# lkp411/cDLRM

Hardware: AMD Instinct MI355X
Metric: training samples/sec, Criteo-Terabyte-shape synthetic (cached data-parallel DLRM step; look-ahead refills that fall into the timed region included: see config.refills_in_timed_region) (higher is better)
Workload: dtype f32

## Files before the change

cdlrm_amd/_lib.py:

```python
from __future__ import annotations

import ctypes as C
import os
from typing import Optional

_HERE = os.path.dirname(os.path.abspath(__file__))
LIB_PATH = os.path.join(_HERE, "csrc", "libcdlrm_hip.so")

c_i32, c_i64, c_u64, c_f32 = C.c_int32, C.c_int64, C.c_uint64, C.c_float
vp = C.c_void_p


class CdlrmLibraryError(RuntimeError):
    pass


class CdlrmError(RuntimeError):
    def __init__(self, rc: int, msg: str):
        super().__init__("libcdlrm_hip: rc=%d: %s" % (rc, msg))
        self.rc = rc


class Geometry(C.Structure):
    _fields_ = [("num_tables", c_i32), ("dim", c_i32), ("num_ways", c_i32), ("aux_rows", c_i32),
                ("table_rows", C.POINTER(c_i64)), ("cache_sets", C.POINTER(c_i64)),
                ("device", c_i32), ("aux_phases", c_i32)]


class Plan(C.Structure):
    _fields_ = [("bitmap", vp), ("uniq", vp), ("uniq_off", vp), ("cap_uniq", c_i64),
                ("prot", vp), ("hit", vp), ("kept", vp), ("kept_off", vp), ("way", vp), ("flags", vp),
                ("winner", vp), ("win_claim", vp), ("win_idx", vp), ("win_row", vp), ("win_tag", vp),
                ("win_off", vp), ("cap_win", c_i64), ("stage", vp), ("ev_tag", vp)]


class Victims(C.Structure):
    _fields_ = [("pos", vp), ("idx", vp), ("off", vp), ("rows", vp), ("cap", c_i64)]


class GemmRoute(C.Structure):
    _fields_ = [("family", c_i32), ("tm", c_i32), ("tn", c_i32), ("mode", c_i32), ("aligned", c_i32), ("splits", c_i32),
                ("vec_a", c_i32), ("vec_b", c_i32), ("fast", c_i32)]


class EmbBwdRoute(C.Structure):
    _fields_ = [("sort_chunk", c_i32), ("sort_e", c_i32), ("sort_chunks", c_i32), ("merge_passes", c_i32), ("seg_meta", c_i32),
                ("keys_in_b", c_i32), ("apply", c_i32), ("arange", c_i32), ("lpr", c_i32), ("reserved", c_i32),
                ("apply_grid_x", c_i64), ("apply_grid_y", c_i64), ("long_grid", c_i64), ("keys_off", c_i64), ("meta_off", c_i64),
                ("once_off", c_i64), ("apply_keys_off", c_i64)]


PROTOTYPES = {
    "cdlrm_abi_version": (C.c_int, []),
    "cdlrm_debug_set": (C.c_int, [c_i32, c_i32]),
    "cdlrm_last_error": (C.c_char_p, []),
    "cdlrm_ctx_create": (C.c_int, [C.POINTER(Geometry), C.POINTER(vp)]),
    "cdlrm_ctx_destroy": (C.c_int, [vp]),
    "cdlrm_ctx_bind_cache": (C.c_int, [vp, vp, vp]),
    "cdlrm_ctx_bind_host_tables": (C.c_int, [vp, C.POINTER(vp)]),
    "cdlrm_host_register": (C.c_int, [vp, c_u64, C.POINTER(vp)]),
    "cdlrm_host_unregister": (C.c_int, [vp]),
    "cdlrm_ctx_check_sync": (C.c_int, [vp, vp]),
    "cdlrm_embbag_probe": (C.c_int, [vp, vp, c_i64, c_i64, vp, vp, vp, c_i32, vp]),
    "cdlrm_window_resolve": (C.c_int, [vp, vp, c_i64, c_i64, c_i64, c_i64, vp, vp, vp]),
    "cdlrm_embbag_take": (C.c_int, [vp, vp, c_i64, c_i64, vp, vp, c_i64, vp, c_i32, vp]),
    "cdlrm_victim_writeback_work_bytes": (c_u64, [c_i32, c_i64]),
    "cdlrm_victim_writeback": (C.c_int, [vp, vp, c_i64, c_i64, vp, vp, c_i64, c_i32, vp, vp]),
    "cdlrm_embbag_fwd": (C.c_int, [vp, vp, vp, c_i64, c_i64, c_i64, vp, c_i64, c_i64, vp]),
    "cdlrm_embbag_bwd_work_bytes": (c_u64, [c_i32, c_i64, c_i32]),
    "cdlrm_embbag_bwd_sgd": (C.c_int, [vp, vp, vp, c_i64, c_i64, c_i64, vp, c_i64, c_i64, c_f32, vp, vp, vp]),
    "cdlrm_embbag_bwd_prepare": (C.c_int, [vp, vp, c_i64, vp, vp]),
    "cdlrm_embbag_bwd_apply": (C.c_int, [vp, vp, c_i64, c_i64, c_i64, vp, c_i64, c_i64, c_f32, vp, vp, vp]),
    "cdlrm_embbag_bwd_apply_rest": (C.c_int, [vp, vp, c_i64, c_i64, c_i64, vp, c_i64, c_i64, c_f32, vp, vp, vp]),
    "cdlrm_embbag_bwd_once_flags": (C.c_int, [vp, vp, c_i64, vp]),
    "cdlrm_embbag_bwd_sorted_bytes": (C.c_uint64, [c_i32, c_i32, c_i64]),
    "cdlrm_embbag_bwd_prepare_window": (C.c_int, [vp, vp, c_i64, c_i64, c_i32, c_i64, c_i32, c_i32, vp, vp]),
    "cdlrm_embbag_bwd_sorted_views": (C.c_int, [vp, vp, c_i32, c_i64, c_i32, vp, vp, vp]),
    "cdlrm_embbag_bwd_apply_sorted": (C.c_int, [vp, c_i64, vp, c_i64, c_i64, c_f32, vp, vp, vp, c_i64, c_i32, c_i32, vp, vp]),
    "cdlrm_embbag_bwd_route": (C.c_int, [c_i32, c_i32, c_i64, c_i32, c_i32, c_i32, c_i32, c_i32, C.POINTER(EmbBwdRoute)]),
    "cdlrm_qr_embbag_fwd": (C.c_int, [vp, vp, c_i64, c_i64, vp, vp, c_i64, c_i32, c_i32, c_i32, vp, vp, vp, vp, vp]),
    "cdlrm_qr_embbag_bwd": (C.c_int, [vp, vp, c_i64, c_i64, vp, vp, vp, c_i64, c_i32, c_i32, c_i32, vp, vp, vp]),
    "cdlrm_bag_fwd": (C.c_int, [vp, vp, c_i64, c_i64, vp, c_i64, c_i32, vp, vp, vp]),
    "cdlrm_bag_bwd": (C.c_int, [vp, vp, c_i64, c_i64, vp, c_i64, c_i32, vp, vp]),
    "cdlrm_window_unique": (C.c_int, [vp, C.POINTER(Plan), vp, c_i64, c_i64, vp]),
    "cdlrm_window_unique_add": (C.c_int, [vp, C.POINTER(Plan), vp, c_i64, c_i64, vp]),
    "cdlrm_window_unique_finish": (C.c_int, [vp, C.POINTER(Plan), vp]),
    "cdlrm_plan_probe": (C.c_int, [vp, C.POINTER(Plan), vp]),
    "cdlrm_plan_offsets_sync": (C.c_int, [vp, C.POINTER(Plan), vp, vp, vp, vp]),
    "cdlrm_plan_assign": (C.c_int, [vp, C.POINTER(Plan), vp, c_u64, vp]),
    "cdlrm_plan_fetch": (C.c_int, [vp, C.POINTER(Plan), C.POINTER(vp), C.c_int, vp]),
    "cdlrm_plan_commit": (C.c_int, [vp, C.POINTER(Plan), vp]),
    "cdlrm_plan_writeback": (C.c_int, [vp, C.POINTER(Plan), C.POINTER(vp), C.c_int, vp]),
    "cdlrm_plan_victims": (C.c_int, [vp, C.POINTER(Plan), C.POINTER(Victims), vp]),
    "cdlrm_plan_victims_list": (C.c_int, [vp, C.POINTER(Plan), C.POINTER(Victims), vp]),
    "cdlrm_host_gather_rows": (C.c_int, [C.POINTER(vp), vp, vp, c_i32, c_i32, vp, c_i32]),
    "cdlrm_ctx_bind_victims": (C.c_int, [vp, C.POINTER(Victims)]),
    "cdlrm_gather_rows": (C.c_int, [vp, vp, c_i64, c_i32, vp, vp]),
    "cdlrm_agg_compact": (C.c_int, [vp, vp, c_i64, vp, c_i64, vp, vp]),
    "cdlrm_agg_gather": (C.c_int, [vp, vp, vp, c_f32, vp, c_i64, c_i64, vp]),
    "cdlrm_agg_scatter": (C.c_int, [vp, vp, vp, vp, c_i64, c_i64, vp]),
    "cdlrm_agg_mark_tier": (C.c_int, [vp, vp, c_i64, c_i64, c_i32, vp, vp]),
    "cdlrm_agg_split": (C.c_int, [vp, vp, c_i64, vp, c_i32, vp, vp, vp]),
    "cdlrm_interact_fwd": (C.c_int, [vp, c_i64, c_i32, c_i32, c_i32, vp, c_i64, vp]),
    "cdlrm_interact_bwd": (C.c_int, [vp, vp, c_i64, c_i64, c_i32, c_i32, c_i32, c_i32, vp, vp]),
    "cdlrm_gather_interact_supported": (C.c_int, [vp]),
    "cdlrm_gather_interact_fwd": (C.c_int, [vp, vp, c_i64, vp, c_i64, c_i64, c_i32, vp, c_i64, vp]),
    "cdlrm_gather_interact_bwd": (C.c_int, [vp, vp, c_i64, vp, c_i64, vp, c_i64, c_i64, c_i32, c_i32, vp, vp]),
    "cdlrm_gather_interact_bwd_sgd": (C.c_int, [vp, vp, c_i64, vp, c_i64, vp, c_i64, c_i64, c_i32, c_i32, vp, vp, c_i64, c_f32, vp]),
    "cdlrm_linear_fwd": (C.c_int, [vp, c_i64, vp, vp, vp, c_i64, c_i64, c_i32, c_i32, c_i32, vp]),
    "cdlrm_linear_bwd_work_bytes": (c_u64, [c_i64, c_i32, c_i32]),
    "cdlrm_linear_bwd": (C.c_int, [vp, c_i64, vp, vp, c_i64, vp, c_i64, vp, c_i64, vp, vp, c_i64, c_i32, c_i32,
                                   c_i32, c_i32, vp, vp]),
    "cdlrm_linear_fwd_route": (C.c_int, [vp, c_i64, vp, vp, vp, c_i64, c_i64, c_i32, c_i32, c_i32, vp, c_i32,
                                         C.POINTER(GemmRoute)]),
    "cdlrm_linear_bwd_route": (C.c_int, [vp, c_i64, vp, vp, c_i64, vp, c_i64, vp, c_i64, vp, vp, c_i64, c_i32, c_i32,
                                         c_i32, c_i32, vp, vp, c_i32, C.POINTER(GemmRoute)]),
    "cdlrm_mlp_wgrad_work_bytes": (c_u64, [c_i32, c_i64, vp, vp]),
    "cdlrm_mlp_wgrad": (C.c_int, [c_i32, vp, vp, vp, vp, vp, vp, c_i64, vp, vp, vp, vp]),
    "cdlrm_mlp_wgrad_sgd": (C.c_int, [c_i32, vp, vp, vp, vp, vp, vp, vp, vp, c_f32, c_i64, vp, vp, vp, vp]),
    "cdlrm_mlp_wgrad_work_bytes_ex": (c_u64, [c_i32, c_i64, vp, vp, c_i32]),
    "cdlrm_mlp_wgrad_ex": (C.c_int, [c_i32, vp, vp, vp, vp, vp, vp, c_i64, vp, vp, c_i32, vp, vp]),
    "cdlrm_mlp_wgrad_sgd_ex": (C.c_int, [c_i32, vp, vp, vp, vp, vp, vp, vp, vp, c_f32, c_i64, vp, vp, c_i32, vp, vp]),
    "cdlrm_mlp_wgrad_route": (C.c_int, [c_i32, vp, vp, vp, vp, vp, vp, c_i64, vp, vp, c_i32, c_i32, C.POINTER(GemmRoute)]),
    "cdlrm_bce_fwd_bwd": (C.c_int, [vp, vp, c_i64, vp, vp, c_i32, vp]),
    "cdlrm_loss_fwd_bwd": (C.c_int, [vp, vp, c_i64, c_i32, C.c_float, C.c_float, C.c_float, vp, vp, vp, c_i32, vp]),
    "cdlrm_head_scratch_floats": (c_i64, []),
    "cdlrm_head_fwd_bwd": (C.c_int, [vp, c_i64, vp, vp, vp, c_i64, c_i32, c_i32, C.c_float, C.c_float, C.c_float, c_i32,
                                     vp, vp, vp, vp, c_i64, vp, vp, c_i32, vp]),
    "cdlrm_head_finish": (C.c_int, [vp, c_i64, vp, vp, vp]),
    "cdlrm_sgd_step2": (C.c_int, [vp, vp, c_i64, c_i64, c_i64, c_i64, C.c_float, vp]),
    "cdlrm_act_bwd": (C.c_int, [vp, c_i64, vp, c_i64, c_i64, c_i32, c_i32, vp]),
    "cdlrm_sgd_step": (C.c_int, [vp, vp, c_i64, c_f32, vp]),
    "cdlrm_scale_div": (C.c_int, [vp, c_i64, c_f32, vp]),
    "cdlrm_scatter_rows": (C.c_int, [vp, vp, vp, c_i64, c_i32, C.c_int, vp]),
    "cdlrm_blend_rows": (C.c_int, [vp, vp, vp, c_i64, c_i32, vp, vp]),
    "cdlrm_mark_rows": (C.c_int, [vp, vp, c_i64, vp, vp]),
    "cdlrm_synth_indices": (C.c_int, [vp, c_i64, c_i64, c_i64, C.c_double, c_u64, vp]),
    "cdlrm_bags_window": (C.c_int, [vp, c_i64, vp, c_i32, c_i32, c_i64, vp, vp]),
    "cdlrm_bags_rank_slice": (C.c_int, [vp, c_i64, vp, c_i32, c_i32, c_i32, vp, c_i64, c_i64, c_i64, c_i64, vp, vp, vp]),
    "cdlrm_dayfile_window": (C.c_int, [vp, vp, vp, c_i64, c_i32, c_i32, c_i64, vp, vp, c_i64, c_i64, vp, vp]),
    "cdlrm_dayfile_tile": (C.c_int, []),
    "cdlrm_tape_create": (vp, [c_i32]),
    "cdlrm_tape_destroy": (None, [vp]),
    "cdlrm_tape_add": (C.c_int, [vp, vp, c_i32, vp, vp, c_i32, vp]),
    "cdlrm_tape_cells": (vp, [vp]),
    "cdlrm_tape_length": (c_i64, [vp]),
    "cdlrm_tape_stream_arg": (c_i32, [vp]),
    "cdlrm_tape_op_info": (C.c_char_p, [vp, c_i64, vp]),
    "cdlrm_tape_probe": (C.c_int, [c_f32, c_i64, c_f32, c_i32, vp, c_i64, c_f32, c_i32, c_i64, c_i64, vp, c_i32, c_f32, c_i64]),
    "cdlrm_tape_probe_log": (C.c_int, [c_i64, c_i64]),
    "cdlrm_tape_probe_log_take": (c_i64, [vp, c_i64]),
    "cdlrm_tape_replay": (C.c_int, [vp]),
    "cdlrm_tape_set_lanes": (C.c_int, [vp, vp, vp, c_i64]),
    "cdlrm_tape_selftest": (C.c_int, []),
    "cdlrm_event_record": (C.c_int, [vp, vp]),
    "cdlrm_stream_wait_event": (C.c_int, [vp, vp]),
    "cdlrm_event_attach_next": (C.c_int, [vp, vp]),
    "cdlrm_stream_create": (vp, [c_i32]),
    "cdlrm_stream_destroy": (C.c_int, [vp]),
    "cdlrm_event_create": (vp, [c_i32]),
    "cdlrm_event_destroy": (C.c_int, [vp]),
    "cdlrm_event_elapsed_us": (C.c_int, [vp, vp, vp]),
    "cdlrm_ctx_time_next_gather": (C.c_int, [vp, vp, vp]),
}

_lib: Optional[C.CDLL] = None
_proxy = None
import threading as _threading

_rec = _threading.local()


class _Recording:

    def __init__(self, cdll):
        self._cdll = cdll

    def __getattr__(self, name):
        fn = getattr(self._cdll, name)
        is_call = fn.restype is C.c_int

        def call(*args):
            tape = getattr(_rec, "tape", None)
            if tape is not None and is_call:
                tape.append((fn, args))
            return fn(*args)

        call.__name__ = name
        self.__dict__[name] = call
        return call


def start_recording(tape: list) -> None:
    _rec.tape = tape


def stop_recording() -> None:
    _rec.tape = None


def record(fn, *args):
    tape = getattr(_rec, "tape", None)
    if tape is not None:
        tape.append((fn, args))
    return fn(*args)


def raw():
    lib()
    return _lib


def lib():
    global _lib, _proxy
    if _lib is None:
        if not os.path.exists(LIB_PATH):
            raise CdlrmLibraryError(
                "%s not found: build it with `make -C cdlrm_amd/csrc` (or __graft_entry__.build()). "
                "cdlrm_amd has no CPU fallback for the cached training path." % LIB_PATH)
        import torch
        l = C.CDLL(LIB_PATH)
        for name, (res, args) in PROTOTYPES.items():
            fn = getattr(l, name)
            fn.restype = res
            fn.argtypes = args
        if l.cdlrm_abi_version() != 1:
            raise CdlrmLibraryError("ABI version mismatch")
        _lib = l
        _proxy = _Recording(l)
    return _proxy


def require_gpu(what: str = "cdlrm_amd") -> None:
    import torch
    if not torch.cuda.is_available():
        raise CdlrmLibraryError(
            "%s needs a HIP device (MI355X / gfx950) and found none: cdlrm_amd has no CPU fallback for the cached training "
            "path -- every compute entry point is a hand-written HIP kernel behind csrc/libcdlrm_hip.so" % what)


HW_QUEUES_PINNED = 2
HIP_DEFAULT_HW_QUEUES = 4


def hw_queues() -> int:
    try:
        return int(os.environ.get("GPU_MAX_HW_QUEUES", str(HIP_DEFAULT_HW_QUEUES)))
    except ValueError:
        return -1


_warned_queues = False


def warn_hw_queues() -> None:
    global _warned_queues
    if not _warned_queues and hw_queues() != HW_QUEUES_PINNED:
        _warned_queues = True
        import warnings
        warnings.warn("GPU_MAX_HW_QUEUES=%s: cdlrm_amd's entry points run with %d hardware queues per process (set "
                      "GPU_MAX_HW_QUEUES=%d before the first HIP call)"
                      % (os.environ.get("GPU_MAX_HW_QUEUES"), HW_QUEUES_PINNED, HW_QUEUES_PINNED), RuntimeWarning, stacklevel=3)


class TapeUnsupported(Exception):
# ... 188 lines not shown
```

cdlrm_amd/csrc/ctx.hip:

```cpp
#include <stdarg.h>
#include <sys/resource.h>
#include <sys/syscall.h>
#include <unistd.h>

#include <algorithm>
#include <thread>

#include "common.h"

static thread_local char g_err[512] = "";

void cdlrm_set_error(const char* fmt, ...) {
    va_list ap;
    va_start(ap, fmt);
    vsnprintf(g_err, sizeof(g_err), fmt, ap);
    va_end(ap);
}

int g_cdlrm_debug[8] = {0, 0, 0, 0, 0, 0, 0, 0};
extern "C" int cdlrm_debug_set(int32_t key, int32_t value) {
    CDLRM_REQUIRE(key >= 0 && key < 8, "key: 0 .. 7");
#ifndef CDLRM_DEV
    CDLRM_REQUIRE(!(key == 6 && (value & 3)), "work-skipping switches (key 6, bits 1 and 2) exist in -DCDLRM_DEV builds only");
#endif
    g_cdlrm_debug[key] = value;
    return 0;
}
extern "C" int cdlrm_abi_version(void) { return CDLRM_ABI_VERSION; }
extern "C" const char* cdlrm_last_error(void) { return g_err; }

extern "C" int cdlrm_ctx_create(const cdlrm_geometry* geo, cdlrm_ctx** out) {
    CDLRM_REQUIRE(geo && out, "null argument");
    CDLRM_REQUIRE(geo->num_tables >= 1 && geo->num_tables <= 1024, "1..1024 tables");
    CDLRM_REQUIRE(geo->dim >= 4 && geo->dim % 4 == 0, "dim must be a positive multiple of 4");
    CDLRM_REQUIRE(geo->num_ways >= 1 && geo->num_ways <= 64, "1..64 ways");
    CDLRM_REQUIRE(geo->aux_rows >= 0, "aux_rows >= 0");
    CDLRM_REQUIRE(geo->aux_phases >= 0 && geo->aux_phases <= 2, "aux_phases 0..2");
    CDLRM_HIP_CHECK(hipSetDevice(geo->device));
    cdlrm_ctx* c = new cdlrm_ctx();
    c->T = geo->num_tables; c->D = geo->dim; c->ways = geo->num_ways; c->aux = geo->aux_rows;
    c->device = geo->device;
    c->aux_phases = geo->aux_phases < 1 ? 1 : geo->aux_phases;
    int64_t tag = 0, row = 0, set = 0, bm = 0;
    for (int k = 0; k < c->T; ++k) {
        TableDesc d;
        d.n_rows = geo->table_rows[k];
        d.P = geo->cache_sets[k];
        if (d.n_rows < 1 || d.P < 1 || d.P > d.n_rows ||
            d.P * (int64_t)c->ways + (int64_t)c->aux * c->aux_phases >= ((int64_t)1 << 31)) {
            delete c;
            cdlrm_set_error("cdlrm_ctx_create: table %d has unsupported geometry (n=%lld P=%lld)", k,
                            (long long)geo->table_rows[k], (long long)geo->cache_sets[k]);
            return CDLRM_EINVAL;
        }
        d.tag_base = tag; d.row_base = row; d.set_base = set; d.bm_base = bm;
        d.bm_words = ((d.n_rows + 63) / 64 + BM_WPB - 1) / BM_WPB * BM_WPB;
        d.rows = d.P * c->ways + (int64_t)c->aux * c->aux_phases;
        tag += d.P * c->ways; row += d.rows; set += d.P; bm += d.bm_words;
        c->h_tab.push_back(d);
    }
    c->total_tags = tag; c->total_rows = row; c->total_sets = set; c->total_bm_words = bm;
    c->h_host_rows.assign(c->T, nullptr);
    CDLRM_HIP_CHECK(hipMalloc(&c->d_tab, sizeof(TableDesc) * c->T));
    CDLRM_HIP_CHECK(hipMemcpy(c->d_tab, c->h_tab.data(), sizeof(TableDesc) * c->T, hipMemcpyHostToDevice));
    CDLRM_HIP_CHECK(hipMalloc(&c->d_host_rows, sizeof(float*) * c->T));
    CDLRM_HIP_CHECK(hipMemset(c->d_host_rows, 0, sizeof(float*) * c->T));
    CDLRM_HIP_CHECK(hipMalloc(&c->d_ptr_fetch, sizeof(float*) * c->T));
    CDLRM_HIP_CHECK(hipMalloc(&c->d_ptr_wb, sizeof(float*) * c->T));
    CDLRM_HIP_CHECK(hipMalloc(&c->d_err, sizeof(int)));
    CDLRM_HIP_CHECK(hipMemset(c->d_err, 0, sizeof(int)));
    CDLRM_HIP_CHECK(hipMalloc(&c->d_small, sizeof(int64_t) * 256));
    CDLRM_HIP_CHECK(hipMemset(c->d_small, 0, sizeof(int64_t) * 256));
    CDLRM_HIP_CHECK(hipHostMalloc((void**)&c->h_pinned, sizeof(int64_t) * 4096, hipHostMallocDefault));
    int rc = cdlrm_scan_reserve(c, 1 << 16);
    if (rc) { delete c; return rc; }
    *out = c;
    return 0;
}

extern "C" int cdlrm_ctx_destroy(cdlrm_ctx* c) {
    if (!c) return 0;
    try {
        (void)hipDeviceSynchronize();
        if (c->d_tab) (void)hipFree(c->d_tab);
        if (c->d_host_rows) (void)hipFree(c->d_host_rows);
        if (c->d_ptr_fetch) (void)hipFree(c->d_ptr_fetch);
        if (c->d_ptr_wb) (void)hipFree(c->d_ptr_wb);
        if (c->d_err) (void)hipFree(c->d_err);
        if (c->d_small) (void)hipFree(c->d_small);
        if (c->d_scan) (void)hipFree(c->d_scan);
        if (c->d_scan_agg) (void)hipFree(c->d_scan_agg);
        if (c->h_pinned) (void)hipHostFree(c->h_pinned);
        (void)hipGetLastError();
    } catch (...) {
    }
    delete c;
    return 0;
}

extern "C" int cdlrm_ctx_bind_cache(cdlrm_ctx* c, int64_t* tags, float* weight) {
    CDLRM_REQUIRE(c && tags && weight, "null argument");
    CDLRM_REQUIRE(((uintptr_t)weight & 15) == 0 && ((uintptr_t)tags & 15) == 0, "16-byte aligned buffers");
    c->tags = tags;
    c->weight = weight;
    return 0;
}

extern "C" int cdlrm_ctx_bind_host_tables(cdlrm_ctx* c, float* const* host_rows) {
    CDLRM_REQUIRE(c && host_rows, "null argument");
    for (int k = 0; k < c->T; ++k) {
        CDLRM_REQUIRE(host_rows[k] != nullptr && ((uintptr_t)host_rows[k] & 15) == 0, "16-byte aligned host tables");
        c->h_host_rows[k] = host_rows[k];
    }
    CDLRM_HIP_CHECK(hipMemcpy(c->d_host_rows, c->h_host_rows.data(), sizeof(float*) * c->T, hipMemcpyHostToDevice));
    return 0;
}

extern "C" int cdlrm_host_register(void* host_ptr, uint64_t bytes, void** device_alias) {
    CDLRM_REQUIRE(host_ptr && bytes && device_alias, "null argument");
    CDLRM_HIP_CHECK(hipHostRegister(host_ptr, bytes, hipHostRegisterMapped | hipHostRegisterPortable));
    CDLRM_HIP_CHECK(hipHostGetDevicePointer(device_alias, host_ptr, 0));
    return 0;
}

extern "C" int cdlrm_host_unregister(void* host_ptr) {
    CDLRM_REQUIRE(host_ptr, "null argument");
    CDLRM_HIP_CHECK(hipHostUnregister(host_ptr));
    return 0;
}

static void host_gather_range(const float* const* tables, const int64_t* idx, const int64_t* off, int T, int D, float* dst,
                              int64_t a, int64_t b, int background) {
    if (background) (void)setpriority(PRIO_PROCESS, (id_t)syscall(SYS_gettid), 19);
    int t = 0;
    const size_t row_bytes = (size_t)D * sizeof(float);
    constexpr int AHEAD = 16;
    int ta = 0;
    for (int64_t j = a; j < b; ++j) {
        const int64_t jp = j + AHEAD;
        if (jp < b) {
            while (ta < T - 1 && jp >= off[ta + 1]) ++ta;
            const char* p = (const char*)(tables[ta] + idx[jp] * D);
            for (size_t o = 0; o < row_bytes; o += 64) __builtin_prefetch(p + o, 0, 0);
        }
        while (t < T - 1 && j >= off[t + 1]) ++t;
        memcpy(dst + j * D, tables[t] + idx[j] * D, row_bytes);
    }
}

extern "C" int cdlrm_host_gather_rows(const float* const* tables, const int64_t* idx, const int64_t* off, int32_t T,
                                      int32_t D, float* dst, int32_t nthreads) {
    CDLRM_REQUIRE(tables && idx && off && dst && T >= 1 && D >= 1, "bad argument");
    const int64_t n = off[T];
    if (n <= 0) return 0;
    for (int k = 0; k < T; ++k) CDLRM_REQUIRE(off[k] <= off[k + 1] && (off[k] == off[k + 1] || tables[k]), "bad offsets / table");
    int nt = nthreads < 1 ? 1 : nthreads;
    if ((int64_t)nt > (n + 4095) / 4096) nt = (int)((n + 4095) / 4096);
    if (nt <= 1) {
        host_gather_range(tables, idx, off, T, D, dst, 0, n, 0);
        return 0;
    }
    std::vector<std::thread> th;
    const int64_t per = (n + nt - 1) / nt;
    for (int i = 0; i < nt; ++i) {
        const int64_t a = i * per, b = std::min<int64_t>(n, a + per);
        if (a >= b) break;
        th.emplace_back(host_gather_range, tables, idx, off, (int)T, (int)D, dst, a, b, 1);
    }
    for (auto& x : th) x.join();
    return 0;
}

extern "C" int cdlrm_ctx_check_sync(cdlrm_ctx* c, void* stream) {
    CDLRM_REQUIRE(c, "null ctx");
    hipStream_t s = (hipStream_t)stream;
    int* h = (int*)(c->h_pinned + 4000);
// ... 11 lines not shown
```

cdlrm_amd/csrc/dense.hip:

```cpp
#include "gemm_wide.h"
#include "gemm_bf16.h"


#define SK_KMAX 32
__global__ void __launch_bounds__(256) k_linear_smallk(const float* __restrict__ X, int64_t ld_x, const float* __restrict__ W,
                                                       const float* __restrict__ bias, float* __restrict__ Y, int64_t ld_y,
                                                       int64_t M, int N, int K, int act) {
    __shared__ float Xs[32][SK_KMAX + 1];
    __shared__ __attribute__((aligned(16))) float Wt[SK_KMAX][128 + 4];
    const int64_t m0 = (int64_t)blockIdx.y * 32;
    const int n0 = blockIdx.x * 128;
    for (int e = threadIdx.x; e < 32 * K; e += 256) {
        const int r = e / K, k = e % K;
        Xs[r][k] = X[min(m0 + r, M - 1) * ld_x + k];
    }
    for (int e = threadIdx.x; e < 128 * K; e += 256) {
        const int n = e / K, k = e % K;
        Wt[k][n] = W[(int64_t)min(n0 + n, N - 1) * K + k];
    }
    __syncthreads();
    const int cg = threadIdx.x & 31, rg = threadIdx.x >> 5;
    float acc[4][4];
#pragma unroll
    for (int i = 0; i < 4; ++i)
// ... 102 lines not shown
        const int64_t blocks = cdiv(M, rpw) * (N >> 8);
        if (blocks <= 0x7fffffff) {
            if (rec) {
                gemm_record(rec, CDLRM_ROUTE_SMALLK_ROWS, 0, 0, 0, 0, 1, 0, 0, 0);
                return 0;
            }
            hipLaunchKernelGGL((k_linear_smallk_rows<13>), dim3((unsigned)blocks), dim3(256), 0, (hipStream_t)stream, X, ld_x, W,
                               bias, Y, ld_y, M, (int)N, rpw, (int)act);
            CDLRM_LAUNCH_CHECK();
            return 0;
        }
    }
    if (K <= SK_KMAX && N % 4 == 0 && ld_y % 4 == 0 && aligned16(Y) && cdiv(M, 32) <= 65535) {
        if (rec) {
            gemm_record(rec, CDLRM_ROUTE_SMALLK, 0, 0, 0, 0, 1, 0, 0, 0);
            return 0;
        }
        dim3 grid((unsigned)cdiv(N, 128), (unsigned)cdiv(M, 32));
        hipLaunchKernelGGL(k_linear_smallk, grid, dim3(256), 0, (hipStream_t)stream, X, ld_x, W, bias, Y, ld_y, M, (int)N,
                           (int)K, (int)act);
        CDLRM_LAUNCH_CHECK();
        return 0;
    }
    GemmArgs g = gemm_args();
    g.A = X; g.lda = ld_x; g.B = W; g.ldb = K; g.C = Y; g.ldc = ld_y; g.slab = 0;
    g.M = M; g.N = N; g.K = K; g.kchunk = K; g.bias = bias; g.act = act;
    g.vecA = aligned16(X) && ld_x % 4 == 0 && K % 4 == 0;
    g.vecB = aligned16(W) && K % 4 == 0;
    g.alone = alone;
    return launch_gemm<true, true>(g, 1, (hipStream_t)stream, rec);
}

extern "C" int cdlrm_linear_fwd(const float* X, int64_t ld_x, const float* W, const float* bias, float* Y, int64_t ld_y,
                                int64_t M, int32_t N, int32_t K, int32_t act, void* stream) {
    return linear_fwd(X, ld_x, W, bias, Y, ld_y, M, N, K, act, stream, nullptr);
}

extern "C" int cdlrm_linear_fwd_route(const float* X, int64_t ld_x, const float* W, const float* bias, float* Y, int64_t ld_y,
                                      int64_t M, int32_t N, int32_t K, int32_t act, void* stream, int32_t n_cu,
                                      cdlrm_gemm_route* out) {
    CDLRM_REQUIRE(out && n_cu >= 1, "bad argument");
    memset(out, 0, sizeof(*out));
    const GemmRec rec = {out, n_cu};
    return linear_fwd(X, ld_x, W, bias, Y, ld_y, M, N, K, act, stream, &rec);
}

__global__ void __launch_bounds__(256) k_act_grad(const float* __restrict__ Y, int64_t ld_y, float* __restrict__ dY,
                                                  int64_t ld_dy, int64_t M, int N, int act) {
    const int64_t total = M * N;
    for (int64_t e = (int64_t)blockIdx.x * blockDim.x + threadIdx.x; e < total; e += (int64_t)gridDim.x * blockDim.x) {
        const int64_t m = e / N;
        const int n = (int)(e % N);
        const float y = Y[m * ld_y + n];
        float d = dY[m * ld_dy + n];
        if (act == 1) d = y > 0.f ? d : 0.f;
        else if (act == 2) d = d * ((1.0f - y) * y);
        dY[m * ld_dy + n] = d;
    }
}

__device__ __forceinline__ void reduce_slabs_body(int bid, const float* __restrict__ partA, int64_t countA, int splitsA,
                                                  float* __restrict__ outA, int gxa, const float* __restrict__ partB,
                                                  int64_t countB, int splitsB, float* __restrict__ outB,
                                                  float (*red)[64], float* __restrict__ pA = nullptr,
                                                  float* __restrict__ pB = nullptr, float lr = 0.f, int novec = 0) {
    if (bid >= gxa) {
        const int c = threadIdx.x & 63, sub = threadIdx.x >> 6;
        const int64_t e = (int64_t)(bid - gxa) * 64 + c;
        float s = 0.f;
        if (e < countB)
            for (int z = sub; z < splitsB; z += 4) s += partB[(int64_t)z * countB + e];
        red[sub][c] = s;
        __syncthreads();
        if (sub == 0 && e < countB) {
            const float g = ((red[0][c] + red[1][c]) + red[2][c]) + red[3][c];
            outB[e] = g;
            if (pB) pB[e] = fmaf(-lr, g, pB[e]);
        }
        return;
    }
    if (!novec && (countA & 3) == 0 && ((((uintptr_t)partA | (uintptr_t)outA | (uintptr_t)pA) & 15) == 0)) {
        const int64_t n4 = countA >> 2;
        const float4* __restrict__ p4 = reinterpret_cast<const float4*>(partA);
        for (int64_t e = (int64_t)bid * blockDim.x + threadIdx.x; e < n4; e += (int64_t)gxa * blockDim.x) {
            float4 s = make_float4(0.f, 0.f, 0.f, 0.f);
            float4 q = make_float4(0.f, 0.f, 0.f, 0.f);
            if (pA) q = reinterpret_cast<const float4*>(pA)[e];
            __builtin_amdgcn_sched_barrier(0);
            int z = 0;
            for (; z + 8 <= splitsA; z += 8) {
                float4 v[8];
#pragma unroll
                for (int u = 0; u < 8; ++u) v[u] = p4[(int64_t)(z + u) * n4 + e];
#pragma unroll
                for (int u = 0; u < 8; ++u) { s.x += v[u].x; s.y += v[u].y; s.z += v[u].z; s.w += v[u].w; }
            }
            for (; z < splitsA; ++z) {
                const float4 v = p4[(int64_t)z * n4 + e];
                s.x += v.x; s.y += v.y; s.z += v.z; s.w += v.w;
            }
            reinterpret_cast<float4*>(outA)[e] = s;
            if (pA) {
                q.x = fmaf(-lr, s.x, q.x); q.y = fmaf(-lr, s.y, q.y); q.z = fmaf(-lr, s.z, q.z); q.w = fmaf(-lr, s.w, q.w);
                reinterpret_cast<float4*>(pA)[e] = q;
            }
        }
        return;
    }
    for (int64_t e = (int64_t)bid * blockDim.x + threadIdx.x; e < countA; e += (int64_t)gxa * blockDim.x) {
        float s = 0.f;
        int z = 0;
        for (; z + 4 <= splitsA; z += 4) {
            const float v0 = partA[(int64_t)z * countA + e], v1 = partA[(int64_t)(z + 1) * countA + e];
            const float v2 = partA[(int64_t)(z + 2) * countA + e], v3 = partA[(int64_t)(z + 3) * countA + e];
            s += v0; s += v1; s += v2; s += v3;
        }
        for (; z < splitsA; ++z) s += partA[(int64_t)z * countA + e];
        outA[e] = s;
        if (pA) pA[e] = fmaf(-lr, s, pA[e]);
    }
}

__global__ void __launch_bounds__(256) k_reduce_slabs(const float* __restrict__ partA, int64_t countA, int splitsA,
                                                      float* __restrict__ outA, int gxa,
                                                      const float* __restrict__ partB, int64_t countB, int splitsB,
                                                      float* __restrict__ outB) {
    __shared__ float red[4][64];
    reduce_slabs_body((int)blockIdx.x, partA, countA, splitsA, outA, gxa, partB, countB, splitsB, outB, red);
}

struct ReduceJob {
    const float* partA; int64_t countA; float* outA; int gxa;
    const float* partB; int64_t countB; float* outB;
    int splits;
    float* pA; float* pB; float lr;
    int novec;
};
struct ReduceGroup {
    int n;
    unsigned first[GEMM_GROUP_MAX + 1];
    ReduceJob j[GEMM_GROUP_MAX];
};
__global__ void __launch_bounds__(256) k_reduce_group(ReduceGroup grp) {
    __shared__ float red[4][64];
    int p = 0;
#pragma unroll
    for (int q = 1; q < GEMM_GROUP_MAX; ++q)
        if (q < grp.n && blockIdx.x >= grp.first[q]) p = q;
    const ReduceJob& r = grp.j[p];
    reduce_slabs_body((int)(blockIdx.x - grp.first[p]), r.partA, r.countA, r.splits, r.outA, r.gxa, r.partB, r.countB,
                      r.splits, r.outB, red, r.pA, r.pB, r.lr, r.novec);
}

#define WGRAD_DIRECT_MAX_M 2048
static int wgrad_splits(int64_t M, int N, int K) {
    if (M <= WGRAD_DIRECT_MAX_M) return 1;
    const int64_t tiles = cdiv(N, 64) * cdiv(K, 64);
    const int64_t target = 1024;
    int64_t s = cdiv(target, tiles);
    const int64_t smax = cdiv(M, 8 * GBK);
    if (s > smax) s = smax;
    if (s < 1) s = 1;
    return (int)s;
}

extern "C" uint64_t cdlrm_linear_bwd_work_bytes(int64_t M, int32_t N, int32_t K) {
    const uint64_t splits = (uint64_t)wgrad_splits(M, N, K);
    const uint64_t slabs = splits * N * K * 4;
    const uint64_t cs = splits * N * 4;
    return ((slabs + 255) & ~(uint64_t)255) + ((cs + 255) & ~(uint64_t)255) + 256;
}

extern "C" uint64_t cdlrm_mlp_wgrad_work_bytes(int32_t n_layers, int64_t M, const int32_t* N, const int32_t* K) {
    uint64_t total = 256, largest = 0;
    if (!N || !K) return 0;
    if (M <= WGRAD_DIRECT_MAX_M) {
        const uint64_t zs = (uint64_t)cdiv(M, 4 * GBK) + 1;
        for (int i = 0; i < n_layers; ++i)
            total += ((zs * N[i] * K[i] * 4 + 255) & ~(uint64_t)255) + ((zs * N[i] * 4 + 255) & ~(uint64_t)255);
        return total;
    }
    (void)largest;
    for (int i = 0; i < n_layers; ++i) total += cdlrm_linear_bwd_work_bytes(M, N[i], K[i]);
    return total;
}

static int linear_bwd(const float* X, int64_t ld_x, const float* W, const float* Y, int64_t ld_y, float* dY, int64_t ld_dy,
                      float* dX, int64_t ld_dx, float* dW, float* db, int64_t M, int32_t N, int32_t K, int32_t act,
                      int32_t x_act, void* work, void* stream, const GemmRec* rec) {
    const int alone = (act & CDLRM_GEMM_ALONE) != 0;
    const int bf16 = (act & CDLRM_GEMM_BF16) != 0 && bf16_layer_ok(N, K);
    act &= ~(CDLRM_GEMM_ALONE | CDLRM_GEMM_BF16);
    CDLRM_REQUIRE(X && W && dY && work && M >= 1 && N >= 1 && K >= 1, "bad argument");
    CDLRM_REQUIRE(dW || !db, "db without dW (the bias gradient is a by-product of the weight-gradient GEMM)");
    CDLRM_REQUIRE(act == 0 || Y, "activation backward needs Y");
    CDLRM_REQUIRE(act >= 0 && act <= 2 && x_act >= 0 && x_act <= 2, "bad activation code");
    CDLRM_REQUIRE(((uintptr_t)work & 255) == 0, "work must be 256-byte aligned");
    hipStream_t s = (hipStream_t)stream;
    const int splits = wgrad_splits(M, N, K);
    float* slabs = (float*)work;
    float* cs = (float*)((char*)work + ((((uint64_t)splits * N * K * 4) + 255) & ~(uint64_t)255));
    if (act != 0 && !rec) {
        const int64_t nb = cdiv(M * N, 256), blocks = nb < 2048 ? nb : 2048;
        hipLaunchKernelGGL(k_act_grad, dim3((unsigned)blocks), dim3(256), 0, s, Y, ld_y, dY, ld_dy, M, N, act);
    }
    if (dX) {
        GemmArgs g = gemm_args();
        g.A = dY; g.lda = ld_dy; g.B = W; g.ldb = K; g.C = dX; g.ldc = ld_dx; g.slab = 0;
        g.M = M; g.N = K; g.K = N; g.kchunk = N; g.bias = nullptr; g.act = 0;
        g.vecA = aligned16(dY) && ld_dy % 4 == 0 && N % 4 == 0;
        g.vecB = aligned16(W) && K % 4 == 0;
        g.mask = X; g.ldmask = ld_x; g.mask_act = x_act;
        g.alone = alone;
        int rc = bf16 ? launch_gemm_bf16<true, false>(g, s, rec) : launch_gemm<true, false>(g, 1, s, rec);
        if (rc) return rc;
    }
    if (dW && bf16) {
        GemmArgs g = gemm_args();
        g.A = dY; g.lda = ld_dy; g.B = X; g.ldb = ld_x; g.ldc = K;
        g.slab = (int64_t)N * K;
        g.M = N; g.N = K; g.K = M; g.kchunk = bf16_wgrad_kchunk(M, cdiv(N, 64) * cdiv(K, 64), splits);
        const int va = bf16_vec<false>(dY, ld_dy, N, M), vb = bf16_vec<false>(X, ld_x, K, M);
        g.vecA = va; g.vecB = vb;
        const int zs = (int)cdiv(M, g.kchunk);
        g.C = zs > 1 ? slabs : dW;
        g.colsum = db ? (zs > 1 ? cs : db) : nullptr;
        if (rec) {
            gemm_record(rec + 1, CDLRM_ROUTE_BF16, 1, 1, 0, 0, zs, va, vb, 0);
            return 0;
        }
        int rc = launch_wgrad_bf16(&g, 1, va, vb, s);
        if (rc) return rc;
        if (zs > 1) {
            int64_t gxa = cdiv((int64_t)N * K, 256);
            if (gxa > 2048) gxa = 2048;
            const int64_t gxb = db ? cdiv(N, 64) : 0;
            hipLaunchKernelGGL(k_reduce_slabs, dim3((unsigned)(gxa + gxb)), dim3(256), 0, s, slabs, (int64_t)N * K, zs, dW,
                               (int)gxa, cs, (int64_t)N, zs, db);
        }
    } else if (dW) {
        GemmArgs g = gemm_args();
        g.A = dY; g.lda = ld_dy; g.B = X; g.ldb = ld_x; g.ldc = K;
        g.slab = (int64_t)N * K;
        g.M = N; g.N = K; g.K = M; g.kchunk = cdiv(cdiv(M, splits), GBK) * GBK; g.bias = nullptr; g.act = 0;
        g.vecA = aligned16(dY) && ld_dy % 4 == 0 && N % 4 == 0;
        g.vecB = aligned16(X) && ld_x % 4 == 0 && K % 4 == 0;
        const int zs = (int)cdiv(M, g.kchunk);
        g.C = zs > 1 ? slabs : dW;
        g.colsum = db ? (zs > 1 ? cs : db) : nullptr;
        int rc = launch_gemm<false, false>(g, zs, s, rec ? rec + 1 : nullptr);
        if (rc) return rc;
        if (zs > 1 && !rec) {
            int64_t gxa = cdiv((int64_t)N * K, 256);
            if (gxa > 2048) gxa = 2048;
            const int64_t gxb = db ? cdiv(N, 64) : 0;
            hipLaunchKernelGGL(k_reduce_slabs, dim3((unsigned)(gxa + gxb)), dim3(256), 0, s, slabs, (int64_t)N * K, zs, dW,
                               (int)gxa, cs, (int64_t)N, zs, db);
        }
    }
    if (!rec) CDLRM_LAUNCH_CHECK();
    return 0;
}

extern "C" int cdlrm_linear_bwd(const float* X, int64_t ld_x, const float* W, const float* Y, int64_t ld_y, float* dY,
                                int64_t ld_dy, float* dX, int64_t ld_dx, float* dW, float* db, int64_t M, int32_t N,
                                int32_t K, int32_t act, int32_t x_act, void* work, void* stream) {
    CdlrmStopScope stop_scope;
    if ((act & ~(CDLRM_GEMM_ALONE | CDLRM_GEMM_BF16)) != 0 || dW || !dX) stop_scope.hold((hipStream_t)stream);
    return linear_bwd(X, ld_x, W, Y, ld_y, dY, ld_dy, dX, ld_dx, dW, db, M, N, K, act, x_act, work, stream, nullptr);
}

extern "C" int cdlrm_linear_bwd_route(const float* X, int64_t ld_x, const float* W, const float* Y, int64_t ld_y, float* dY,
                                      int64_t ld_dy, float* dX, int64_t ld_dx, float* dW, float* db, int64_t M, int32_t N,
                                      int32_t K, int32_t act, int32_t x_act, void* work, void* stream, int32_t n_cu,
                                      cdlrm_gemm_route* out) {
    CDLRM_REQUIRE(out && n_cu >= 1, "bad argument");
    memset(out, 0, 2 * sizeof(*out));
    const GemmRec rec[2] = {{out, n_cu}, {out + 1, n_cu}};
    return linear_bwd(X, ld_x, W, Y, ld_y, dY, ld_dy, dX, ld_dx, dW, db, M, N, K, act, x_act, work, stream, rec);
}

__global__ void __launch_bounds__(256) k_sgd(float* __restrict__ p, const float* __restrict__ g, int64_t n, float lr);

static void launch_reduce_jobs(const std::vector<ReduceJob>& jobs, hipStream_t s) {
    for (size_t q0 = 0; q0 < jobs.size(); q0 += GEMM_GROUP_MAX) {
        ReduceGroup red;
        memset(&red, 0, sizeof(red));
        unsigned rblocks = 0;
        for (size_t q = q0; q < jobs.size() && q < q0 + GEMM_GROUP_MAX; ++q) {
            red.first[red.n] = rblocks;
            red.j[red.n] = jobs[q];
            rblocks += (unsigned)(jobs[q].gxa + cdiv(jobs[q].countB, 64));
            red.n++;
        }
        red.first[red.n] = rblocks;
        hipLaunchKernelGGL(k_reduce_group, dim3(rblocks), dim3(256), 0, s, red);
    }
}

static int sgd_layers(const std::vector<int>& layers, float* const* dW, float* const* db, float* const* P_w, float* const* P_b,
                      const int32_t* N, const int32_t* K, float lr, hipStream_t s) {
    for (int i : layers) {
        const int64_t cnt = (int64_t)N[i] * K[i];
        int64_t gx = cdiv(cnt, 256);
        if (gx > 2048) gx = 2048;
        hipLaunchKernelGGL(k_sgd, dim3((unsigned)gx), dim3(256), 0, s, P_w[i], (const float*)dW[i], cnt, lr);
        if (db[i] && P_b && P_b[i])
            hipLaunchKernelGGL(k_sgd, dim3((unsigned)cdiv(N[i], 256)), dim3(256), 0, s, P_b[i], (const float*)db[i], (int64_t)N[i], lr);
    }
    CDLRM_LAUNCH_CHECK();
    return 0;
}

static inline void route_set(cdlrm_gemm_route* out, int family, int tm, int tn, int mode, int aligned, int splits, int va, int vb,
                             int fast) {
    const GemmRec rec = {out, 0};
    gemm_record(&rec, family, tm, tn, mode, aligned, splits, va, vb, fast);
}

static int mlp_wgrad_impl(int32_t n_layers, const float* const* X, const int64_t* ld_x, const float* const* dZ,
                          const int64_t* ld_dz, float* const* dW, float* const* db, int64_t M, const int32_t* N,
                          const int32_t* K, void* work, void* stream, float* const* P_w, float* const* P_b, float lr,
                          cdlrm_gemm_route* rout = nullptr, int n_cu = 0, int64_t extra_tiles = 0) {
    CDLRM_REQUIRE(n_layers >= 0 && (n_layers == 0 || (X && ld_x && dZ && ld_dz && dW && db && N && K)) && M >= 1,
                  "bad argument");
    hipStream_t s = (hipStream_t)stream;
    std::vector<char> stepped((size_t)(n_layers > 0 ? n_layers : 0), 0);
    auto step_rest = [&]() -> int {
        if (!P_w) return 0;
        std::vector<int> rest;
        for (int i = 0; i < n_layers; ++i)
            if (!stepped[i]) rest.push_back(i);
        return sgd_layers(rest, dW, db, P_w, P_b, N, K, lr, s);
    };
    if (M <= WGRAD_DIRECT_MAX_M) {
        const int use_tiled = 1;
        std::vector<GemmArgs> direct, tiled;
        std::vector<int> direct_layer, tiled_layer;
        int64_t tiles = 0;
        for (int i = 0; i < n_layers; ++i) {
            CDLRM_REQUIRE(X[i] && dZ[i] && dW[i] && N[i] >= 1 && K[i] >= 1 && ld_x[i] >= K[i] && ld_dz[i] >= N[i],
                          "bad layer argument");
            GemmArgs g = gemm_args();
            g.A = dZ[i]; g.lda = ld_dz[i]; g.B = X[i]; g.ldb = ld_x[i]; g.C = dW[i]; g.ldc = K[i];
            g.M = N[i]; g.N = K[i]; g.K = M; g.kchunk = M; g.colsum = db[i];
            g.vecA = aligned16(dZ[i]) && ld_dz[i] % 4 == 0 && N[i] % 4 == 0;
            g.vecB = aligned16(X[i]) && ld_x[i] % 4 == 0 && K[i] % 4 == 0;
            if (use_tiled && g.vecA && g.vecB && M >= 256) {
                tiled.push_back(g);
                tiled_layer.push_back(i);
                tiles += cdiv(N[i], 64) * cdiv(K[i], 64);
            } else {
                direct.push_back(g);
                direct_layer.push_back(i);
            }
        }
        int64_t kchunk = M;
        int zs = 1;
        tiles += extra_tiles;
        if (tiles > 0) {
            const int64_t target_wgs = M <= 1024 ? 768 : 640;
            int64_t splits = cdiv(target_wgs, tiles);
            const int64_t smax = cdiv(M, 4 * GBK);
            if (splits > smax) splits = smax;
            if (splits < 1) splits = 1;
            kchunk = cdiv(cdiv(M, splits), GBK) * GBK;
            zs = (int)cdiv(M, kchunk);
        }
        if (rout) {
            for (size_t q = 0; q < tiled.size(); ++q)
                route_set(&rout[tiled_layer[q]], CDLRM_ROUTE_GEMM, 1, 1, 0, 0, zs, 1, 1, 0);
            for (size_t q = 0; q < direct.size(); ++q)
                route_set(&rout[direct_layer[q]], CDLRM_ROUTE_DIRECT, 0, 0, 0, 0, zs, direct[q].vecA, direct[q].vecB, 0);
            return 0;
        }
        CDLRM_REQUIRE(zs == 1 || (work && ((uintptr_t)work & 255) == 0), "work must be 256-byte aligned");
        char* wp = (char*)work;
        std::vector<ReduceJob> jobs;
        auto slabbed = [&](GemmArgs& g, int li) {
            const int64_t cnt = (int64_t)N[li] * K[li];
            g.kchunk = kchunk;
            g.slab = cnt;
            if (zs == 1) return;
            float* slabs = (float*)wp;
            wp += (((uint64_t)zs * cnt * 4) + 255) & ~(uint64_t)255;
            float* cs = (float*)wp;
            wp += (((uint64_t)zs * N[li] * 4) + 255) & ~(uint64_t)255;
            g.C = slabs;
            g.colsum = db[li] ? cs : nullptr;
            ReduceJob r;
            r.partA = slabs; r.countA = cnt; r.outA = dW[li];
            int64_t gxa = cdiv(cnt, 1024);
            if (gxa > 256) gxa = 256;
            r.gxa = (int)gxa;
            r.partB = cs; r.countB = db[li] ? N[li] : 0; r.outB = db[li];
            r.splits = zs;
            r.novec = g_cdlrm_debug[2];
            r.pA = P_w ? P_w[li] : nullptr; r.pB = (P_w && P_b && db[li]) ? P_b[li] : nullptr; r.lr = lr;
            if (P_w) stepped[li] = 1;
            jobs.push_back(r);
        };
        for (size_t q = 0; q < direct.size(); ++q) slabbed(direct[q], direct_layer[q]);
        for (size_t q = 0; q < tiled.size(); ++q) slabbed(tiled[q], tiled_layer[q]);
        bool direct_done = direct.empty();
        for (size_t q0 = 0; q0 < tiled.size(); q0 += GEMM_GROUP_MAX) {
            GemmGroup grp;
            memset(&grp, 0, sizeof(grp));
            unsigned blocks = 0;
            for (size_t q = q0; q < tiled.size() && q < q0 + GEMM_GROUP_MAX; ++q) {
                grp.first[grp.n] = blocks;
                grp.g[grp.n] = tiled[q];
                blocks += (unsigned)(cdiv(tiled[q].M, 64) * cdiv(tiled[q].N, 64) * zs);
                grp.n++;
            }
            grp.first[grp.n] = blocks;
            if (!direct_done && launch_wgrad_mixed(direct.data(), (int)direct.size(), grp, blocks, s)) {
                direct_done = true;
                continue;
            }
            hipLaunchKernelGGL((k_gemm_group<false, false, true, true>), dim3(blocks), dim3(256), 0, s, grp);
        }
        if (!direct_done) {
            int rc = launch_wgrad_group(direct.data(), (int)direct.size(), s);
            if (rc) return rc;
        }
        launch_reduce_jobs(jobs, s);
        CDLRM_LAUNCH_CHECK();
        return step_rest();
    }
    CDLRM_REQUIRE(rout || (work && ((uintptr_t)work & 255) == 0), "work must be 256-byte aligned");
    char* wp = (char*)work;
    std::vector<ReduceJob> jobs;
    for (int i = 0; i < n_layers; ++i) {
        CDLRM_REQUIRE(X[i] && dZ[i] && dW[i] && N[i] >= 1 && K[i] >= 1 && ld_x[i] >= K[i] && ld_dz[i] >= N[i],
                      "bad layer argument");
        const int splits = wgrad_splits(M, N[i], K[i]);
        const int64_t cnt = (int64_t)N[i] * K[i];
        GemmArgs g = gemm_args();
        g.A = dZ[i]; g.lda = ld_dz[i]; g.B = X[i]; g.ldb = ld_x[i]; g.ldc = K[i];
        g.slab = cnt;
        g.M = N[i]; g.N = K[i]; g.K = M; g.kchunk = cdiv(cdiv(M, splits), GBK) * GBK;
        g.vecA = aligned16(dZ[i]) && ld_dz[i] % 4 == 0 && N[i] % 4 == 0;
        g.vecB = aligned16(X[i]) && ld_x[i] % 4 == 0 && K[i] % 4 == 0;
        const int zs = (int)cdiv(M, g.kchunk);
        g.C = dW[i];
        g.colsum = db[i];
        if (rout) {
            const GemmRec rec = {&rout[i], n_cu};
            (void)launch_gemm<false, false>(g, zs, s, &rec);
            continue;
        }
        if (zs > 1) {
            float* slabs = (float*)wp;
            wp += (((uint64_t)zs * cnt * 4) + 255) & ~(uint64_t)255;
            float* cs = (float*)wp;
            wp += (((uint64_t)zs * N[i] * 4) + 255) & ~(uint64_t)255;
            g.C = slabs;
            g.colsum = db[i] ? cs : nullptr;
            ReduceJob r;
            r.partA = slabs; r.countA = cnt; r.outA = dW[i];
            int64_t gxa = cdiv(cnt, 256);
            if (gxa > 1024) gxa = 1024;
            r.gxa = (int)gxa;
            r.partB = cs; r.countB = db[i] ? N[i] : 0; r.outB = db[i];
            r.splits = zs;
            r.novec = g_cdlrm_debug[2];
            r.pA = P_w ? P_w[i] : nullptr; r.pB = (P_w && P_b && db[i]) ? P_b[i] : nullptr; r.lr = lr;
            if (P_w) stepped[i] = 1;
            jobs.push_back(r);
        }
        int rc = launch_gemm<false, false>(g, zs, s);
        if (rc) return rc;
    }
    if (rout) return 0;
    launch_reduce_jobs(jobs, s);
    CDLRM_LAUNCH_CHECK();
    return step_rest();
}

extern "C" int cdlrm_mlp_wgrad(int32_t n_layers, const float* const* X, const int64_t* ld_x, const float* const* dZ,
                               const int64_t* ld_dz, float* const* dW, float* const* db, int64_t M, const int32_t* N,
                               const int32_t* K, void* work, void* stream) {
    return mlp_wgrad_impl(n_layers, X, ld_x, dZ, ld_dz, dW, db, M, N, K, work, stream, nullptr, nullptr, 0.f);
}

extern "C" int cdlrm_mlp_wgrad_sgd(int32_t n_layers, const float* const* X, const int64_t* ld_x, const float* const* dZ,
                                   const int64_t* ld_dz, float* const* dW, float* const* db, float* const* W,
                                   float* const* b, float lr, int64_t M, const int32_t* N, const int32_t* K, void* work,
                                   void* stream) {
    CDLRM_REQUIRE(n_layers == 0 || (W && b), "parameters missing");
    return mlp_wgrad_impl(n_layers, X, ld_x, dZ, ld_dz, dW, db, M, N, K, work, stream, W, b, lr);
}

struct Bf16Wgrad {
    std::vector<int> fp, bf;
    int64_t kchunk = 0;
    int zs = 1;
    uint64_t fp_bytes = 0;
};

static void bf16_wgrad_plan(int32_t n_layers, int64_t M, const int32_t* N, const int32_t* K, Bf16Wgrad& p) {
    int64_t tiles = 0;
    for (int i = 0; i < n_layers; ++i) {
        if (bf16_layer_ok(N[i], K[i])) {
            p.bf.push_back(i);
            tiles += cdiv(N[i], 64) * cdiv(K[i], 64);
        } else {
            p.fp.push_back(i);
        }
    }
    p.kchunk = bf16_wgrad_kchunk(M, tiles, INT64_MAX);
    p.zs = (int)cdiv(M, p.kchunk);
    if (!p.fp.empty()) {
        std::vector<int32_t> n, k;
        for (int i : p.fp) { n.push_back(N[i]); k.push_back(K[i]); }
        p.fp_bytes = cdlrm_mlp_wgrad_work_bytes((int32_t)p.fp.size(), M, n.data(), k.data());
    }
}

extern "C" uint64_t cdlrm_mlp_wgrad_work_bytes_ex(int32_t n_layers, int64_t M, const int32_t* N, const int32_t* K,
                                                  int32_t flags) {
    if (!(flags & CDLRM_GEMM_BF16)) return cdlrm_mlp_wgrad_work_bytes(n_layers, M, N, K);
    if (!N || !K) return 0;
    Bf16Wgrad p;
    bf16_wgrad_plan(n_layers, M, N, K, p);
    uint64_t total = p.fp_bytes + 256;
    if (p.zs > 1)
        for (int i : p.bf)
            total += (((uint64_t)p.zs * N[i] * K[i] * 4 + 255) & ~(uint64_t)255) + (((uint64_t)p.zs * N[i] * 4 + 255) & ~(uint64_t)255);
    return total;
}

static int mlp_wgrad_ex_impl(int32_t n_layers, const float* const* X, const int64_t* ld_x, const float* const* dZ,
                             const int64_t* ld_dz, float* const* dW, float* const* db, int64_t M, const int32_t* N,
                             const int32_t* K, int32_t flags, void* work, void* stream, float* const* P_w, float* const* P_b,
                             float lr, cdlrm_gemm_route* rout, int n_cu) {
    CDLRM_REQUIRE((flags & ~CDLRM_GEMM_BF16) == 0, "bad flags");
    if (!(flags & CDLRM_GEMM_BF16))
        return mlp_wgrad_impl(n_layers, X, ld_x, dZ, ld_dz, dW, db, M, N, K, work, stream, P_w, P_b, lr, rout, n_cu);
    CDLRM_REQUIRE(n_layers >= 0 && (n_layers == 0 || (X && ld_x && dZ && ld_dz && dW && db && N && K)) && M >= 1,
                  "bad argument");
    CDLRM_REQUIRE(rout || (work && ((uintptr_t)work & 255) == 0), "work must be 256-byte aligned");
    for (int i = 0; i < n_layers; ++i)
        CDLRM_REQUIRE(X[i] && dZ[i] && dW[i] && N[i] >= 1 && K[i] >= 1 && ld_x[i] >= K[i] && ld_dz[i] >= N[i],
                      "bad layer argument");
    hipStream_t s = (hipStream_t)stream;
    Bf16Wgrad p;
    bf16_wgrad_plan(n_layers, M, N, K, p);
    if (!p.fp.empty()) {
        int64_t extra_tiles = 0;
        for (int i : p.bf) {
            const bool va = aligned16(dZ[i]) && ld_dz[i] % 4 == 0 && N[i] % 4 == 0;
            const bool vb = aligned16(X[i]) && ld_x[i] % 4 == 0 && K[i] % 4 == 0;
            if (va && vb && M >= 256) extra_tiles += cdiv(N[i], 64) * cdiv(K[i], 64);
        }
        const size_t nf = p.fp.size();
        std::vector<const float*> fx(nf), fdz(nf);
        std::vector<float*> fdw(nf), fdb(nf), fpw(nf), fpb(nf);
        std::vector<int64_t> fldx(nf), flddz(nf);
        std::vector<int32_t> fn(nf), fk(nf);
        std::vector<cdlrm_gemm_route> fr(nf);
        for (size_t q = 0; q < nf; ++q) {
            const int i = p.fp[q];
            fx[q] = X[i]; fdz[q] = dZ[i]; fdw[q] = dW[i]; fdb[q] = db[i]; fldx[q] = ld_x[i]; flddz[q] = ld_dz[i];
            fn[q] = N[i]; fk[q] = K[i];
            fpw[q] = P_w ? P_w[i] : nullptr; fpb[q] = (P_w && P_b) ? P_b[i] : nullptr;
        }
        memset(fr.data(), 0, nf * sizeof(cdlrm_gemm_route));
        int rc = mlp_wgrad_impl((int32_t)nf, fx.data(), fldx.data(), fdz.data(), flddz.data(), fdw.data(), fdb.data(), M, fn.data(),
                                fk.data(), work, stream, P_w ? fpw.data() : nullptr, P_w ? fpb.data() : nullptr, lr,
                                rout ? fr.data() : nullptr, n_cu, extra_tiles);
        if (rc) return rc;
        if (rout)
            for (size_t q = 0; q < nf; ++q) rout[p.fp[q]] = fr[q];
    }
    if (p.bf.empty()) return 0;
    std::vector<GemmArgs> probs;
    std::vector<ReduceJob> jobs;
    char* wp = (char*)work + p.fp_bytes;
    int va = 1, vb = 1;
    for (int i : p.bf) {
        const int64_t cnt = (int64_t)N[i] * K[i];
        GemmArgs g = gemm_args();
        g.A = dZ[i]; g.lda = ld_dz[i]; g.B = X[i]; g.ldb = ld_x[i]; g.ldc = K[i];
        g.slab = cnt;
        g.M = N[i]; g.N = K[i]; g.K = M; g.kchunk = p.kchunk;
        g.vecA = bf16_vec<false>(dZ[i], ld_dz[i], N[i], M);
        g.vecB = bf16_vec<false>(X[i], ld_x[i], K[i], M);
// ... 1413 lines not shown
```

cdlrm_amd/csrc/gemm_glds.h:

```cpp
#pragma once
#include "gemm.h"

#define G2_BK 32
#ifndef G2_PRIO
#define G2_PRIO 0
#endif
#ifndef G2_ABL
#define G2_ABL 0
#endif

typedef __attribute__((address_space(3))) void* g2_lds_ptr;

__device__ __forceinline__ void g2_dma16(const float* src, unsigned lds_wave_base) {
    unsigned keep;
    asm volatile("s_mov_b32 %0, m0\n\ts_mov_b32 m0, %2\n\ts_nop 0\n\tglobal_load_lds_dwordx4 %1, off\n\ts_mov_b32 m0, %0"
                 : "=&s"(keep)
                 : "v"(src), "s"(lds_wave_base)
                 : "memory");
}
__device__ __forceinline__ void g2_dma_wait() { asm volatile("s_waitcnt vmcnt(0)" ::: "memory"); }
__device__ __forceinline__ unsigned g2_lds_addr(const float* p) {
    return (unsigned)(uintptr_t)(g2_lds_ptr)(p);
}

template <bool KC, int ROWS>
struct G2Stage {
    static constexpr int NP = ROWS / 32;
    const float* src[NP];
    int64_t step;
    __device__ __forceinline__ void init(const float* P, int64_t ld, int64_t r0, int64_t rmax, int64_t kbeg) {
        const int tid = threadIdx.x;
#pragma unroll
        for (int i = 0; i < NP; ++i) {
            if (KC) {
                const int row = i * 32 + (tid >> 3);
                const int c = (tid & 7) ^ ((row >> 1) & 7);
                src[i] = P + min(r0 + row, rmax - 1) * ld + kbeg + 4 * c;
            } else {
                constexpr int CPR = ROWS / 4;
                const int q = i * 256 + tid;
                const int kk = q / CPR, rc = (q % CPR) * 4;
                src[i] = P + (kbeg + kk) * ld + min(r0 + rc, rmax - 4);
            }
        }
        step = KC ? G2_BK : G2_BK * ld;
    }
    __device__ __forceinline__ void piece(int i, unsigned base) {
        g2_dma16(src[i], base + i * 4096u);
        src[i] += step;
    }
};

template <bool A_KC, bool B_KC, int TM, int TN>
__device__ __forceinline__ void g2_frags(const float* Ab, const float* Bb, int kg, int ra, int rb, int lk, int sw,
                                         float4 (&a)[TM], float4 (&b)[TN]) {
    constexpr int BM = 64 * TM, BN = 64 * TN;
#pragma unroll
    for (int i = 0; i < TM; ++i) {
        const int r = ra + i * 32;
        if (A_KC) {
            a[i] = *reinterpret_cast<const float4*>(Ab + r * G2_BK + 4 * ((kg * 2 + lk) ^ sw));
        } else {
            const float* q = Ab + (kg * 8 + 4 * lk) * BM + r;
            a[i] = make_float4(q[0], q[BM], q[2 * BM], q[3 * BM]);
        }
    }
#pragma unroll
    for (int j = 0; j < TN; ++j) {
        const int c = rb + j * 32;
        if (B_KC) {
            b[j] = *reinterpret_cast<const float4*>(Bb + c * G2_BK + 4 * ((kg * 2 + lk) ^ sw));
        } else {
            const float* q = Bb + (kg * 8 + 4 * lk) * BN + c;
            b[j] = make_float4(q[0], q[BN], q[2 * BN], q[3 * BN]);
        }
    }
}

template <int TM, int TN>
__device__ __forceinline__ void g2_epilogue(const GemmArgs& g, f32x16 (&acc)[TM][TN], int64_t m0, int64_t n0, unsigned bz,
                                            int wm, int wn, int lane) {
    float* C = g.C + (int64_t)bz * g.slab;
    const bool vbias = g.bias != nullptr && (((uintptr_t)g.bias) & 15) == 0;
    const bool vmask = g.mask_act != 0 && (((uintptr_t)g.mask) & 15) == 0 && (g.ldmask & 3) == 0;
#pragma unroll
    for (int i = 0; i < TM; ++i) {
        const int64_t row = m0 + wm * (32 * TM) + i * 32 + (lane & 31);
#pragma unroll
        for (int j = 0; j < TN; ++j) {
#pragma unroll
            for (int q = 0; q < 4; ++q) {
                const int64_t col = n0 + wn * (32 * TN) + j * 32 + 8 * q + 4 * (lane >> 5);
                if (row >= g.M || col >= g.N) continue;
                float4 v = make_float4(acc[i][j][4 * q], acc[i][j][4 * q + 1], acc[i][j][4 * q + 2], acc[i][j][4 * q + 3]);
                if (g.bias) {
                    float4 bv;
                    if (vbias) bv = *reinterpret_cast<const float4*>(g.bias + col);
                    else bv = make_float4(g.bias[col], g.bias[col + 1], g.bias[col + 2], g.bias[col + 3]);
                    v.x += bv.x; v.y += bv.y; v.z += bv.z; v.w += bv.w;
                }
                if (g.act == 1) {
                    v.x = v.x > 0.f ? v.x : 0.f; v.y = v.y > 0.f ? v.y : 0.f;
                    v.z = v.z > 0.f ? v.z : 0.f; v.w = v.w > 0.f ? v.w : 0.f;
                } else if (g.act == 2) {
                    v.x = 1.0f / (1.0f + expf(-v.x)); v.y = 1.0f / (1.0f + expf(-v.y));
                    v.z = 1.0f / (1.0f + expf(-v.z)); v.w = 1.0f / (1.0f + expf(-v.w));
                }
                if (g.mask_act) {
                    float4 x;
                    const float* mp = g.mask + row * g.ldmask + col;
                    if (vmask) x = *reinterpret_cast<const float4*>(mp);
                    else x = make_float4(mp[0], mp[1], mp[2], mp[3]);
                    if (g.mask_act == 1) {
                        v.x = x.x > 0.f ? v.x : 0.f; v.y = x.y > 0.f ? v.y : 0.f;
                        v.z = x.z > 0.f ? v.z : 0.f; v.w = x.w > 0.f ? v.w : 0.f;
                    } else {
                        v.x *= (1.0f - x.x) * x.x; v.y *= (1.0f - x.y) * x.y;
                        v.z *= (1.0f - x.z) * x.z; v.w *= (1.0f - x.w) * x.w;
                    }
                }
                *reinterpret_cast<float4*>(C + row * g.ldc + col) = v;
            }
        }
    }
}

template <int TM, int TN, bool B_KC, int ACT>
__device__ __forceinline__ void g2_epilogue_full(const GemmArgs& g, f32x16 (&acc)[TM][TN], int64_t m0, int64_t n0, int wm, int wn,
                                                 int lane) {
    float4 bv[TN][4];
    float4 mv[B_KC ? 1 : TM][B_KC ? 1 : TN][4];
    const int64_t row0 = m0 + wm * (32 * TM) + (lane & 31);
    const int64_t col0 = n0 + wn * (32 * TN) + 4 * (lane >> 5);
    if (B_KC) {
        if (g.bias) {
#pragma unroll
            for (int j = 0; j < TN; ++j)
#pragma unroll
                for (int q = 0; q < 4; ++q) bv[j][q] = *reinterpret_cast<const float4*>(g.bias + col0 + j * 32 + 8 * q);
        } else {
#pragma unroll
            for (int j = 0; j < TN; ++j)
#pragma unroll
                for (int q = 0; q < 4; ++q) bv[j][q] = make_float4(0.f, 0.f, 0.f, 0.f);
        }
    } else if (ACT != 0) {
#pragma unroll
        for (int i = 0; i < TM; ++i)
#pragma unroll
            for (int j = 0; j < TN; ++j)
#pragma unroll
                for (int q = 0; q < 4; ++q)
                    mv[i][j][q] = *reinterpret_cast<const float4*>(g.mask + (row0 + i * 32) * g.ldmask + col0 + j * 32 + 8 * q);
    }
    const bool has_bias = g.bias != nullptr;
    __builtin_amdgcn_sched_barrier(0);
#pragma unroll
    for (int i = 0; i < TM; ++i)
#pragma unroll
        for (int j = 0; j < TN; ++j)
#pragma unroll
            for (int q = 0; q < 4; ++q) {
                float4 v = make_float4(acc[i][j][4 * q], acc[i][j][4 * q + 1], acc[i][j][4 * q + 2], acc[i][j][4 * q + 3]);
                if (B_KC) {
                    const float4 b = bv[j][q];
                    if (has_bias) { v.x += b.x; v.y += b.y; v.z += b.z; v.w += b.w; }
                    if (ACT == 1) {
                        v.x = v.x > 0.f ? v.x : 0.f; v.y = v.y > 0.f ? v.y : 0.f;
                        v.z = v.z > 0.f ? v.z : 0.f; v.w = v.w > 0.f ? v.w : 0.f;
                    } else if (ACT == 2) {
                        v.x = 1.0f / (1.0f + expf(-v.x)); v.y = 1.0f / (1.0f + expf(-v.y));
                        v.z = 1.0f / (1.0f + expf(-v.z)); v.w = 1.0f / (1.0f + expf(-v.w));
                    }
                } else if (ACT != 0) {
                    const float4 x = mv[i][j][q];
                    if (ACT == 1) {
                        v.x = x.x > 0.f ? v.x : 0.f; v.y = x.y > 0.f ? v.y : 0.f;
                        v.z = x.z > 0.f ? v.z : 0.f; v.w = x.w > 0.f ? v.w : 0.f;
                    } else if (ACT == 2) {
                        v.x *= (1.0f - x.x) * x.x; v.y *= (1.0f - x.y) * x.y;
                        v.z *= (1.0f - x.z) * x.z; v.w *= (1.0f - x.w) * x.w;
                    }
                }
                *reinterpret_cast<float4*>(g.C + (row0 + i * 32) * g.ldc + col0 + j * 32 + 8 * q) = v;
            }
}

template <bool B_KC>
__host__ __device__ __forceinline__ bool g2_full_ok(const GemmArgs& g) {
    if (!g.fastep) return false;
    if (B_KC) return g.mask_act == 0 && (g.bias == nullptr || (((uintptr_t)g.bias) & 15) == 0);
    return g.bias == nullptr && g.act == 0 && (g.mask_act == 0 || ((((uintptr_t)g.mask) & 15) == 0 && (g.ldmask & 3) == 0));
}

#ifdef GEMM2_STAMP
__device__ unsigned long long g2_stamps[8 * 4096];
#define G2_STAMP(slot)                                                                            \
    if (threadIdx.x == 0 && g2_wg < 4096) {                                                         \
        g2_stamps[g2_wg * 8 + (slot)] = __builtin_amdgcn_s_memtime();                                \
        if ((slot) == 0 || (slot) == 3) g2_stamps[g2_wg * 8 + 4 + ((slot) ? 1 : 0)] = __builtin_amdgcn_s_memrealtime(); \
        if ((slot) == 0) g2_stamps[g2_wg * 8 + 6] = ((unsigned long long)__builtin_amdgcn_s_getreg((31 << 11) | 20) << 32) | \
                                                    (unsigned)__builtin_amdgcn_s_getreg((31 << 11) | 4);               \
    }
#else
#define G2_STAMP(slot)
#endif

template <bool A_KC, bool B_KC, int TM, int TN>
__device__ __forceinline__ void gemm2_tile_body(const GemmArgs& g, unsigned bx, unsigned by, unsigned bz, float* lds) {
#ifdef GEMM2_STAMP
    const unsigned g2_wg = (blockIdx.z * gridDim.y + blockIdx.y) * gridDim.x + blockIdx.x;
#endif
    G2_STAMP(0)
    constexpr int BM = 64 * TM, BN = 64 * TN;
    constexpr int A_ST = BM * G2_BK, B_ST = BN * G2_BK;
    float* As = lds;
    float* Bs = lds + 2 * A_ST;
    const int lane = threadIdx.x & 63, wave = threadIdx.x >> 6;
    const int wm = wave >> 1, wn = wave & 1;
    const int lr = lane & 31, lk = lane >> 5;
    const int64_t m0 = (int64_t)by * BM;
    const int64_t n0 = (int64_t)bx * BN;
    const int64_t kbeg = (int64_t)bz * g.kchunk;
    const int64_t kend = min(g.K, kbeg + g.kchunk);
    const int nt = (int)((kend - kbeg) / G2_BK);
    f32x16 acc[TM][TN];
#pragma unroll
    for (int i = 0; i < TM; ++i)
#pragma unroll
        for (int j = 0; j < TN; ++j)
#pragma unroll
            for (int r = 0; r < 16; ++r) acc[i][j][r] = 0.f;
    const bool do_colsum = !A_KC && g.colsum != nullptr && bx == 0 && wn == 0;
    float csum[TM];
#pragma unroll
    for (int i = 0; i < TM; ++i) csum[i] = 0.f;

    G2Stage<A_KC, BM> sa;
    G2Stage<B_KC, BN> sb;
    constexpr int NPA = G2Stage<A_KC, BM>::NP, NPB = G2Stage<B_KC, BN>::NP, NPIECE = NPA + NPB;
    sa.init(g.A, g.lda, m0, g.M, kbeg);
    sb.init(g.B, g.ldb, n0, g.N, kbeg);
    const unsigned a_dst = __builtin_amdgcn_readfirstlane(g2_lds_addr(As) + wave * 1024u);
    const unsigned b_dst = __builtin_amdgcn_readfirstlane(g2_lds_addr(Bs) + wave * 1024u);
    const int ra = wm * (32 * TM) + lr, rb = wn * (32 * TN) + lr;
    const int sw = (lr >> 1) & 7;

    float4 fa[2][TM], fb[2][TN];
#pragma unroll
    for (int i = 0; i < NPA; ++i) sa.piece(i, a_dst);
#pragma unroll
    for (int i = 0; i < NPB; ++i) sb.piece(i, b_dst);
    g2_dma_wait();
    __syncthreads();
    if (nt > 1) {
#pragma unroll
        for (int i = 0; i < NPA; ++i) sa.piece(i, a_dst + A_ST * 4u);
#pragma unroll
        for (int i = 0; i < NPB; ++i) sb.piece(i, b_dst + B_ST * 4u);
    }
    g2_frags<A_KC, B_KC, TM, TN>(As, Bs, 0, ra, rb, lk, sw, fa[0], fb[0]);
    G2_STAMP(1)

    auto mfma_group = [&](const float4 (&a)[TM], const float4 (&b)[TN]) {
        if (!A_KC && do_colsum) {
#pragma unroll
            for (int i = 0; i < TM; ++i) csum[i] += (a[i].x + a[i].y) + (a[i].z + a[i].w);
        }
#pragma unroll
        for (int i = 0; i < TM; ++i)
#pragma unroll
            for (int j = 0; j < TN; ++j) {
                acc[i][j] = __builtin_amdgcn_mfma_f32_32x32x2f32(b[j].x, a[i].x, acc[i][j], 0, 0, 0);
                acc[i][j] = __builtin_amdgcn_mfma_f32_32x32x2f32(b[j].y, a[i].y, acc[i][j], 0, 0, 0);
                acc[i][j] = __builtin_amdgcn_mfma_f32_32x32x2f32(b[j].z, a[i].z, acc[i][j], 0, 0, 0);
                acc[i][j] = __builtin_amdgcn_mfma_f32_32x32x2f32(b[j].w, a[i].w, acc[i][j], 0, 0, 0);
            }
    };

    for (int t = 0; t < nt; ++t) {
        const int cur = t & 1;
        const float* Ab = As + cur * A_ST;
        const float* Bb = Bs + cur * B_ST;
        g2_frags<A_KC, B_KC, TM, TN>(Ab, Bb, 1, ra, rb, lk, sw, fa[1], fb[1]);
        mfma_group(fa[0], fb[0]);
        __builtin_amdgcn_sched_barrier(0);
        g2_frags<A_KC, B_KC, TM, TN>(Ab, Bb, 2, ra, rb, lk, sw, fa[0], fb[0]);
        mfma_group(fa[1], fb[1]);
        __builtin_amdgcn_sched_barrier(0);
        g2_frags<A_KC, B_KC, TM, TN>(Ab, Bb, 3, ra, rb, lk, sw, fa[1], fb[1]);
        mfma_group(fa[0], fb[0]);
        __builtin_amdgcn_sched_barrier(0);
        const bool more = t + 1 < nt, more2 = t + 2 < nt;
        if (more) {
            g2_dma_wait();
            if (!(G2_ABL & 2))
            __syncthreads();
            g2_frags<A_KC, B_KC, TM, TN>(As + (cur ^ 1) * A_ST, Bs + (cur ^ 1) * B_ST, 0, ra, rb, lk, sw, fa[0], fb[0]);
        }
        __builtin_amdgcn_sched_barrier(0);
        if (!A_KC && do_colsum) {
#pragma unroll
            for (int i = 0; i < TM; ++i) csum[i] += (fa[1][i].x + fa[1][i].y) + (fa[1][i].z + fa[1][i].w);
        }
        const unsigned a_st = a_dst + cur * (A_ST * 4u), b_st = b_dst + cur * (B_ST * 4u);
#pragma unroll
        for (int m = 0; m < 4 * TM * TN; ++m) {
            const int i = (m >> 2) / TN, j = (m >> 2) % TN, comp = m & 3;
            const float av = comp == 0 ? fa[1][i].x : comp == 1 ? fa[1][i].y : comp == 2 ? fa[1][i].z : fa[1][i].w;
            const float bv = comp == 0 ? fb[1][j].x : comp == 1 ? fb[1][j].y : comp == 2 ? fb[1][j].z : fb[1][j].w;
            acc[i][j] = __builtin_amdgcn_mfma_f32_32x32x2f32(bv, av, acc[i][j], 0, 0, 0);
            constexpr int PSTEP = (G2_ABL & 4) ? 2 : 1;
            if (!(G2_ABL & 1) && (m % PSTEP) == 0 && m / PSTEP < NPIECE && more2) {
                if (m / PSTEP < NPA) sa.piece(m / PSTEP, a_st);
                else sb.piece(m / PSTEP - NPA, b_st);
            }
            __builtin_amdgcn_sched_barrier(0);
        }
    }
    G2_STAMP(2)
    if (!A_KC && g.colsum != nullptr && bx == 0) {
        if (wn == 0) {
#pragma unroll
            for (int i = 0; i < TM; ++i) {
                const float other = __shfl_xor(csum[i], 32, 64);
                const float s = lk == 0 ? csum[i] + other : other + csum[i];
                const int64_t row = m0 + wm * (32 * TM) + i * 32 + lr;
                if (lk == 0 && row < g.M) g.colsum[(int64_t)bz * g.M + row] = s;
            }
        }
    }
    bool fast = A_KC && gridDim.z == 1 && m0 + BM <= g.M && n0 + BN <= (int64_t)g.N && g2_full_ok<B_KC>(g);
    if (fast) {
        const int actk = B_KC ? g.act : g.mask_act;
        if (actk == 1) g2_epilogue_full<TM, TN, B_KC, 1>(g, acc, m0, n0, wm, wn, lane);
        else if (actk == 2) g2_epilogue_full<TM, TN, B_KC, 2>(g, acc, m0, n0, wm, wn, lane);
        else g2_epilogue_full<TM, TN, B_KC, 0>(g, acc, m0, n0, wm, wn, lane);
    } else {
        g2_epilogue<TM, TN>(g, acc, m0, n0, bz, wm, wn, lane);
    }
    G2_STAMP(3)
}

template <bool A_KC, bool B_KC, int TM, int TN>
__global__ void __launch_bounds__(256) k_gemm2(GemmArgs g) {
    __shared__ __attribute__((aligned(1024))) float lds[2 * 64 * (TM + TN) * G2_BK];
    const unsigned nwg = gridDim.x * gridDim.y * gridDim.z;
    const unsigned orig = (blockIdx.z * gridDim.y + blockIdx.y) * gridDim.x + blockIdx.x;
    const unsigned wgid = xcd_remap(orig, nwg);
#if G2_PRIO
    if (orig < (nwg >> 1)) __builtin_amdgcn_s_setprio(G2_PRIO);
#endif
    gemm2_tile_body<A_KC, B_KC, TM, TN>(g, wgid % gridDim.x, (wgid / gridDim.x) % gridDim.y,
                                        wgid / (gridDim.x * gridDim.y), lds);
}


template <bool A_KC, bool B_KC>
static inline bool gemm2_applies(const GemmArgs& g) {
    if (!g.vecA || !g.vecB) return false;
    const int64_t kc = g.kchunk < g.K ? g.kchunk : g.K;
    if (g.K < G2_BK || g.K % G2_BK != 0 || kc % G2_BK != 0) return false;
    if (!A_KC && g.M < 4) return false;
    if (!B_KC && g.N < 4) return false;
    if (g.N % 4 != 0 || g.ldc % 4 != 0 || g.slab % 4 != 0 || (((uintptr_t)g.C) & 15) != 0) return false;
    return true;
}

#ifndef G2_EXTRA_LDS
#define G2_EXTRA_LDS(tm, tn) 0
#endif
template <bool A_KC, bool B_KC>
static void launch_gemm2(const GemmArgs& g, int tm, int tn, int splits, hipStream_t s) {
    dim3 grid((unsigned)cdiv(g.N, 64 * tn), (unsigned)cdiv(g.M, 64 * tm), (unsigned)splits);
    const size_t dyn = (size_t)G2_EXTRA_LDS(tm, tn);
    if (tm == 2 && tn == 2) CDLRM_LAUNCH_EV((k_gemm2<A_KC, B_KC, 2, 2>), grid, dim3(256), dyn, s, g);
    else if (tm == 2 && tn == 1) CDLRM_LAUNCH_EV((k_gemm2<A_KC, B_KC, 2, 1>), grid, dim3(256), dyn, s, g);
    else if (tm == 1 && tn == 2) CDLRM_LAUNCH_EV((k_gemm2<A_KC, B_KC, 1, 2>), grid, dim3(256), dyn, s, g);
    else CDLRM_LAUNCH_EV((k_gemm2<A_KC, B_KC, 1, 1>), grid, dim3(256), dyn, s, g);
}

template <bool A_KC, bool B_KC>
static bool gemm3_try(const GemmArgs& g, int splits, hipStream_t s, const GemmRec* rec);

template <bool A_KC, bool B_KC>
static int launch_gemm(GemmArgs g, int splits, hipStream_t s, const GemmRec* rec = nullptr) {
    if (g.K < 4) g.vecA = g.vecB = 0;
    if constexpr (A_KC || !B_KC) {
        if (gemm3_try<A_KC, B_KC>(g, splits, s, rec)) {
            if (!rec) CDLRM_LAUNCH_CHECK();
            return 0;
        }
    }
    const bool long_narrow = (g.M >= 4096 || g.K >= 4096) && cdiv(g.M, 64) * cdiv(g.N, 64) * splits >= 256 &&
                             gemm2_applies<A_KC, B_KC>(g);
    if (gemm_use_direct(g.M, g.N, splits) && !long_narrow) {
        launch_gemm_direct<A_KC, B_KC>(g, splits, s, rec);
        if (!rec) CDLRM_LAUNCH_CHECK();
        return 0;
    }
    if (gemm2_applies<A_KC, B_KC>(g)) {
        int tm2 = 2, tn2 = 1;
        if (g.M <= 64 || cdiv(g.M, 128) * cdiv(g.N, 64) * splits <= 256) tm2 = 1;
        if (splits == 1 && g.K <= 256) tm2 = 1;
        if (!(g_cdlrm_debug[6] & 16) && A_KC && splits == 1 && tm2 == 2 && cdiv(g.M, 128) * cdiv(g.N, 128) >= 1024) tn2 = 2;
        if (rec) {
            gemm_record(rec, CDLRM_ROUTE_GEMM2, tm2, tn2, 0, 0, splits, 1, 1, A_KC && splits == 1 && g2_full_ok<B_KC>(g));
            return 0;
        }
        launch_gemm2<A_KC, B_KC>(g, tm2, tn2, splits, s);
        CDLRM_LAUNCH_CHECK();
        return 0;
    }
    if (g.N <= 32 || g.M <= 32) {
        launch_gemm_direct<A_KC, B_KC>(g, splits, s, rec);
        if (!rec) CDLRM_LAUNCH_CHECK();
        return 0;
    }
    int tm, tn;
    gemm_pick_tile(g.M, g.N, splits, &tm, &tn);
    if (g.N <= 32) tn = 1;
    if (g.M <= 32) tm = 1;
    if (tm == 2 && tn == 1) { tm = 1; tn = g.N <= 64 ? 1 : 2; }
    if (g.K < 4) g.vecA = g.vecB = 0;
    if (!A_KC && g.M < 4) g.vecA = 0;
    if (!B_KC && g.N < 4) g.vecB = 0;
    if (rec) {
        gemm_record(rec, CDLRM_ROUTE_GEMM, tm, tn, 0, 0, splits, g.vecA, g.vecB, 0);
        return 0;
    }
    dim3 grid((unsigned)cdiv(g.N, 64 * tn), (unsigned)cdiv(g.M, 64 * tm), (unsigned)splits);
    if (tm == 2 && tn == 2) launch_gemm_v<A_KC, B_KC, 2, 2>(g, grid, s);
    else if (tm == 1 && tn == 2) launch_gemm_v<A_KC, B_KC, 1, 2>(g, grid, s);
    else launch_gemm_v<A_KC, B_KC, 1, 1>(g, grid, s);
    CDLRM_LAUNCH_CHECK();
    return 0;
}
```

cdlrm_amd/csrc/tape.hip:

```cpp
#include <hip/hip_runtime.h>

#include <atomic>
#include <chrono>
#include <climits>
#include <condition_variable>
#include <mutex>
#include <new>
#include <thread>
#include <tuple>
#include <type_traits>
#include <utility>
#include <vector>

#include "common.h"

#define TAPE_MAX_INT 24
#define TAPE_MAX_FLT 8
#define TAPE_MAX_LANES 4

typedef int (*tape_invoke_fn)(void* fn, const int64_t* ia, const float* fa);

template <typename T>
static inline T tape_take(const int64_t*& ia, const float*& fa) {
    if constexpr (std::is_floating_point<T>::value) {
        return (T)*fa++;
    } else if constexpr (std::is_pointer<T>::value) {
        return reinterpret_cast<T>((intptr_t)*ia++);
    } else {
        static_assert(std::is_integral<T>::value, "tape entry points take pointers, integers and floats only");
        return static_cast<T>(*ia++);
    }
}

template <typename R, typename... A>
static int tape_invoke(void* fn, const int64_t* ia, const float* fa) {
    std::tuple<A...> args{tape_take<A>(ia, fa)...};
    return (int)std::apply(reinterpret_cast<R (*)(A...)>(fn), args);
}

struct TapeEntry {
    void* fn;
    tape_invoke_fn invoke;
    int32_t n_int, n_flt;
    const char* name;
    int32_t stream_arg;
};

template <typename R, typename... A>
static TapeEntry tape_entry(R (*f)(A...), const char* name) {
    static_assert(std::is_same<R, int>::value, "tape entry points return int");
    constexpr int n_flt = (0 + ... + (std::is_floating_point<A>::value ? 1 : 0));
    constexpr int n_int = (int)sizeof...(A) - n_flt;
    static_assert(n_int <= TAPE_MAX_INT && n_flt <= TAPE_MAX_FLT, "too many arguments for a tape call");
    return TapeEntry{reinterpret_cast<void*>(f), &tape_invoke<R, A...>, n_int, n_flt, name, -1};
}
template <typename... A> struct tape_last_is_ptr : std::false_type {};
template <typename A0> struct tape_last_is_ptr<A0> : std::is_same<A0, void*> {};
template <typename A0, typename... A> struct tape_last_is_ptr<A0, A...> : tape_last_is_ptr<A...> {};
template <typename R, typename... A>
static TapeEntry tape_entry_s(R (*f)(A...), const char* name) {
    static_assert(tape_last_is_ptr<A...>::value, "a launching entry point ends on its stream (void*)");
    TapeEntry e = tape_entry(f, name);
    e.stream_arg = (int32_t)sizeof...(A) - 1;
    return e;
}
template <typename R, typename... A>
static TapeEntry tape_entry_at(R (*f)(A...), const char* name, int32_t stream_arg) {
    TapeEntry e = tape_entry(f, name);
    e.stream_arg = stream_arg;
    return e;
}

extern "C" int cdlrm_tape_probe(float f0, int64_t a0, float f1, int32_t a1, void* a2, int64_t a3, float f2, int32_t a4,
                                int64_t a5, int64_t a6, void* a7, int32_t a8, float f3, int64_t a9);
extern "C" int cdlrm_tape_probe_log(int64_t tag, int64_t spin);

#define TAPE_FN(f) tape_entry_s(&f, #f)
#define TAPE_FN_AT(f, pos) tape_entry_at(&f, #f, pos)
static const std::vector<TapeEntry>& tape_registry() {
    static const std::vector<TapeEntry> reg = {
        TAPE_FN(cdlrm_embbag_probe), TAPE_FN(cdlrm_embbag_take), TAPE_FN(cdlrm_embbag_fwd), TAPE_FN(cdlrm_embbag_bwd_sgd),
        TAPE_FN(cdlrm_embbag_bwd_prepare), TAPE_FN(cdlrm_embbag_bwd_apply), TAPE_FN(cdlrm_embbag_bwd_apply_rest),
        TAPE_FN(cdlrm_gather_interact_bwd_sgd), TAPE_FN(cdlrm_embbag_bwd_prepare_window), TAPE_FN(cdlrm_embbag_bwd_apply_sorted),
        TAPE_FN(cdlrm_window_resolve),
        TAPE_FN(cdlrm_mark_rows), TAPE_FN(cdlrm_interact_fwd), TAPE_FN(cdlrm_interact_bwd), TAPE_FN(cdlrm_gather_interact_fwd),
        TAPE_FN(cdlrm_gather_interact_bwd), TAPE_FN(cdlrm_linear_fwd),
        TAPE_FN(cdlrm_linear_bwd), TAPE_FN(cdlrm_mlp_wgrad), TAPE_FN(cdlrm_mlp_wgrad_sgd), TAPE_FN(cdlrm_mlp_wgrad_ex),
        TAPE_FN(cdlrm_mlp_wgrad_sgd_ex), TAPE_FN(cdlrm_bce_fwd_bwd),
        TAPE_FN(cdlrm_loss_fwd_bwd), TAPE_FN(cdlrm_head_fwd_bwd), TAPE_FN(cdlrm_head_finish), TAPE_FN(cdlrm_act_bwd),
        TAPE_FN(cdlrm_sgd_step), TAPE_FN(cdlrm_sgd_step2), TAPE_FN(cdlrm_scale_div),
        TAPE_FN_AT(cdlrm_ctx_time_next_gather, -1),
        TAPE_FN_AT(cdlrm_event_record, 1), TAPE_FN_AT(cdlrm_stream_wait_event, 0), TAPE_FN_AT(cdlrm_event_attach_next, 1),
        TAPE_FN(cdlrm_agg_compact), TAPE_FN(cdlrm_agg_gather), TAPE_FN(cdlrm_agg_scatter),
        TAPE_FN_AT(cdlrm_tape_probe, -1), TAPE_FN_AT(cdlrm_tape_probe_log, -1),
    };
    return reg;
}
#undef TAPE_FN_AT
#undef TAPE_FN

struct TapeOp {
    void* fn;
    tape_invoke_fn invoke;
    int32_t n_int, n_flt;
    int64_t iargs[TAPE_MAX_INT];
    int32_t cell[TAPE_MAX_INT];
    float fargs[TAPE_MAX_FLT];
    int32_t lane = 0;
    int32_t dep = -1;
    const char* name = "";
    int64_t call_ns = 0, wait_ns = 0, calls = 0, max_ns = 0;
};

struct cdlrm_tape {
    std::vector<TapeOp> ops;
    std::vector<int64_t> cells;
    int lanes = 1;
    int device = 0;
    std::atomic<int> done[TAPE_MAX_LANES];
    std::atomic<int> finished[TAPE_MAX_LANES];
    int rc[TAPE_MAX_LANES];
    char err[TAPE_MAX_LANES][256];
};

static inline int tape_call(const TapeOp& o, const int64_t* a) { return o.invoke(o.fn, a, o.fargs); }

extern "C" cdlrm_tape* cdlrm_tape_create(int32_t n_cells) {
    if (n_cells < 0 || n_cells > 64) { cdlrm_set_error("cdlrm_tape_create: 0..64 cells"); return nullptr; }
    cdlrm_tape* t = new (std::nothrow) cdlrm_tape();
    if (!t) { cdlrm_set_error("cdlrm_tape_create: out of memory"); return nullptr; }
    t->cells.assign((size_t)n_cells, 0);
    return t;
}

extern "C" void cdlrm_tape_destroy(cdlrm_tape* t) { delete t; }

extern "C" int cdlrm_tape_add(cdlrm_tape* t, void* fn, int32_t n_int, const int64_t* iargs, const int32_t* cell,
                              int32_t n_flt, const float* fargs) {
    CDLRM_REQUIRE(t && fn, "null argument");
    CDLRM_REQUIRE(n_int >= 0 && n_int <= TAPE_MAX_INT && n_flt >= 0 && n_flt <= TAPE_MAX_FLT, "too many arguments for a tape call");
    const TapeEntry* e = nullptr;
    for (const TapeEntry& r : tape_registry())
        if (r.fn == fn) { e = &r; break; }
    CDLRM_REQUIRE(e, "not a registered tape entry point (csrc/tape.hip: tape_registry)");
    if (e->n_int != n_int || e->n_flt != n_flt) {
        cdlrm_set_error("cdlrm_tape_add: %s takes %d integer-class + %d float arguments, got %d + %d", e->name, e->n_int,
                        e->n_flt, n_int, n_flt);
        return CDLRM_EINVAL;
    }
    TapeOp o;
    o.fn = fn;
    o.invoke = e->invoke;
    o.name = e->name;
    o.n_int = n_int; o.n_flt = n_flt;
    for (int i = 0; i < TAPE_MAX_INT; ++i) {
        o.iargs[i] = i < n_int ? iargs[i] : 0;
        o.cell[i] = i < n_int ? cell[i] : -1;
        CDLRM_REQUIRE(o.cell[i] >= -1 && o.cell[i] < (int)t->cells.size(), "cell index outside the tape's cells");
    }
    for (int i = 0; i < TAPE_MAX_FLT; ++i) o.fargs[i] = i < n_flt ? fargs[i] : 0.f;
    t->ops.push_back(o);
    return 0;
}

extern "C" int64_t* cdlrm_tape_cells(cdlrm_tape* t) { return t ? t->cells.data() : nullptr; }

extern "C" int64_t cdlrm_tape_length(cdlrm_tape* t) { return t ? (int64_t)t->ops.size() : -1; }

extern "C" const char* cdlrm_tape_op_info(cdlrm_tape* t, int64_t k, int64_t* out) {
    if (!t || !out || k < 0 || k >= (int64_t)t->ops.size()) return nullptr;
    const TapeOp& o = t->ops[(size_t)k];
    out[0] = o.lane; out[1] = o.calls; out[2] = o.call_ns; out[3] = o.wait_ns; out[4] = o.max_ns;
    return o.name;
}

extern "C" int32_t cdlrm_tape_stream_arg(void* fn) {
    for (const TapeEntry& e : tape_registry())
        if (e.fn == fn) return e.stream_arg;
    return -2;
}

static inline void tape_pause() { __builtin_ia32_pause(); }

static inline int64_t tape_now_ns() {
    return std::chrono::duration_cast<std::chrono::nanoseconds>(std::chrono::steady_clock::now().time_since_epoch()).count();
}

static int tape_run_lane(cdlrm_tape* t, int lane) {
    const int64_t* cells = t->cells.data();
    const int n = (int)t->ops.size();
    const bool timed = g_cdlrm_debug[3] != 0;
    int rc = 0;
    for (int k = 0; k < n; ++k) {
        TapeOp& o = t->ops[k];
        if (o.lane != lane) continue;
        const int64_t t0 = timed ? tape_now_ns() : 0;
        if (o.dep >= 0) {
            const std::atomic<int>& other = t->done[t->ops[o.dep].lane];
            while (other.load(std::memory_order_acquire) < o.dep) tape_pause();
        }
        const int64_t t1 = timed ? tape_now_ns() : 0;
        int64_t a[TAPE_MAX_INT];
        for (int i = 0; i < TAPE_MAX_INT; ++i) a[i] = o.cell[i] >= 0 ? cells[o.cell[i]] : o.iargs[i];
        rc = tape_call(o, a);
        if (timed) { const int64_t d = tape_now_ns() - t1; o.wait_ns += t1 - t0; o.call_ns += d; ++o.calls; if (d > o.max_ns) o.max_ns = d; }
        if (rc) break;
        t->done[lane].store(k, std::memory_order_release);
    }
    t->done[lane].store(INT_MAX, std::memory_order_release);
    return rc;
}

struct TapeHelper {
    int lane = 1;
    std::atomic<cdlrm_tape*> job{nullptr};
    std::atomic<int> sleeping{0};
    std::mutex m;
    std::condition_variable cv;
    void loop() {
        int idle = 0;
        int device = -1;
        for (;;) {
            cdlrm_tape* t = job.exchange(nullptr, std::memory_order_acquire);
            if (!t) {
                if (++idle < (1 << 16)) { tape_pause(); continue; }
                std::unique_lock<std::mutex> lk(m);
                sleeping.store(1, std::memory_order_seq_cst);
                while (!job.load(std::memory_order_seq_cst)) cv.wait_for(lk, std::chrono::milliseconds(5));
                sleeping.store(0, std::memory_order_seq_cst);
                idle = 0;
                continue;
            }
            idle = 0;
            if (t->device >= 0 && t->device != device) { (void)hipSetDevice(t->device); device = t->device; }
            if (t->device >= 0) (void)hipGetLastError();
            t->rc[lane] = tape_run_lane(t, lane);
            if (t->rc[lane]) snprintf(t->err[lane], sizeof(t->err[lane]), "%s", cdlrm_last_error());
            t->finished[lane].store(1, std::memory_order_release);
        }
    }
// ... 186 lines not shown
```

cdlrm_amd/engine.py:

```python
from __future__ import annotations

import itertools
import math
import os
from typing import List, Optional

import torch
import torch.distributed as dist

from . import _lib
from . import _streams as S
from . import ops
from ._lib import record as rec
from .model_no_ddp import DLRM_Net, Embedding_Table_Cache_Group, Embedding_Table_Group, _linears


_SORT_SERIAL = itertools.count(1)


def square_bags(lS_o, lS_i, device=None, multiple: int = 256):
    if isinstance(lS_i, torch.Tensor) and lS_i.dim() == 2:
        off = lS_o if isinstance(lS_o, torch.Tensor) or lS_o is None else torch.stack(list(lS_o))
        return (None if off is None else off.to(device) if device is not None else off,
                lS_i.to(device) if device is not None else lS_i)
# ... 510 lines not shown
                eng.flush_pending_resolve()
        nchunks = -(-self.nb // self.CH)
        want = min(nchunks, -(-min(int(upto_batch), self.nb) // self.CH))
        while self.done < want and self._armed is None:
            c = self.done
            if c >= self.RING and self.maxj < (c - 2) * self.CH + 1:
                break
            self.done += 1
            pr = self._prepare(c)
            if not urgent and c > 0 and self._started and self._long_batch() and eng._pending_resolve is None:
                eng._pending_resolve, eng.mark_next = pr, True
                self._armed = c
                break
            if hasattr(eng, "_issue_resolve"):
                eng._issue_resolve(pr, lambda fn, *a: fn(*a), S.current_stream(eng.dev), placed=False)
            else:
                ops.window_resolve(self.ctx, pr["cols"], self.lbs, pr["ws"], pr["wsrc"], stream=eng.pref, batch_len=self.B)
        if not urgent:
            self.ensure_sorted(int(upto_batch) - self.CH - 2 + 3)

    def _chunk_nb(self, c: int) -> int:
        return min(self.nb, (c + 1) * self.CH) - c * self.CH

    def ensure_sorted(self, upto_batch: int):
        if not self.sort_chunks:
            return
        eng = self.eng
        upto = min(int(upto_batch), self.nb)
        while self.sorted_upto < upto:
            b0 = self.sorted_upto
            c = b0 // self.CH
            if c >= self.done or c not in self.chunks:
                break
            if self._armed is not None and c >= self._armed and getattr(eng, "_pending_resolve", None) is not None:
                break
            ws, _, ev = self.chunks[c]
            nbc = self._chunk_nb(c)
            j0 = b0 - c * self.CH
            cnt = min(self.SL, nbc - j0)
            if getattr(eng, "sort_chunks", True):
                st = getattr(eng, "sort_st", eng.pref)
                st.wait_event(ev)
                if eng._emb_done is not None:
                    st.wait_event(eng._emb_done)
                if getattr(eng, "sort_delay", 0):
                    with torch.cuda.stream(st):
                        torch.cuda._sleep(int(eng.sort_delay))
                ops.embbag_bwd_prepare_window(self.ctx, ws[:, self.col0:], self.B, nbc, self.width,
                                              self._sorted_ring[c % self.RING], stream=st, j0=j0, count=cnt)
                sev = self._sorted_ev[c % self.RING][j0 // self.SL]
                sev.record(st)
                eng._last_sort_ev = sev
                self._sorted_at[b0] = (cnt, next(_SORT_SERIAL))
            self.sorted_upto = b0 + cnt
            self._sorted_at.pop(b0 - self.RING * self.CH, None)

    def sorted_views(self, j: int):
        if not self.sort_chunks or j >= self.sorted_upto:
            return None
        c = j // self.CH
        nbc = self._chunk_nb(c)
        jl = j - c * self.CH
        at = self._sorted_at.get(j - jl % self.SL)
        if at is None:
            return None
        k, m, o = ops.embbag_bwd_sorted_views(self.ctx, self._sorted_ring[c % self.RING], nbc, self.width, jl)
        return k, m, o, nbc * self.width, self._sorted_ev[c % self.RING][jl // self.SL], at[1]

    def batch(self, j: int):
        c = j // self.CH
        self.maxj = max(self.maxj, j)
        self.ensure(j + 1, urgent=True)
        ws, wsrc, ev = self.chunks[c]
        col = (j - c * self.CH) * self.B + self.col0
        if c >= 2 and (c - 2) in self.chunks:
            del self.chunks[c - 2]
        return ws[:, col:col + self.width], wsrc[:, col:col + self.width], ev, (self, j)

    def lookahead(self, j: int, kmax: int):
        out = []
        eng = self.eng
        for k in range(1, int(kmax) + 1):
            b = j + k
            if b >= self.nb:
                break
            c = b // self.CH
            if c >= self.done or c not in self.chunks:
                break
            if self._armed is not None and c >= self._armed and getattr(eng, "_pending_resolve", None) is not None:
                break
            ws, _, ev = self.chunks[c]
            col = (b - c * self.CH) * self.B
            out.append((k, ws[:, col:col + self.B], ev))
        return out


class TrainEngine:
    def __init__(self, cache_group: Embedding_Table_Cache_Group, dlrm: DLRM_Net, host_tables: Embedding_Table_Group,
                 *, lr: float, lr_embeds: float, world_size: int = 1, rank: int = 0, table_agg_freq: int = 1,
                 table_agg_op: str = "mean", process_group=None, loss: str = "bce", loss_weights=(1.0, 1.0),
                 defer_top_update: bool = False, force_collectives: bool = False, matmul_precision: str = "fp32"):
        self.cg, self.dlrm, self.host = cache_group, dlrm, host_tables
        self.ctx = cache_group.ctx
        self.dev = cache_group.weight.device
        self.lr, self.lr_embeds = float(lr), float(lr_embeds)
        self.world, self.rank = int(world_size), int(rank)
        self.multi = self.world > 1 or bool(force_collectives)
        self.agg_freq, self.agg_op = int(table_agg_freq), table_agg_op
        self.pg = process_group
        self.T, self.D = self.ctx.T, self.ctx.D
        self.F = self.T + 1
        self.itself = bool(dlrm.arch_interaction_itself)
        assert dlrm.arch_interaction_op in ("dot", "cat"), "--arch-interaction-op: dot or cat (model_no_ddp.py:272-304)"
        self.cat = dlrm.arch_interaction_op == "cat"
        self.loss_kind = ops.LOSS[loss]
        self.loss_weights = (float(loss_weights[0]), float(loss_weights[1]))
        thr = float(getattr(dlrm, "loss_threshold", 0.0) or 0.0)
        self.loss_threshold = thr if 0.0 < thr < 1.0 else 0.0
        self.defer_top = bool(defer_top_update)
        self.matmul_precision = matmul_precision
        self.bot = dlrm._acts(dlrm.bot_l, dlrm.sigmoid_bot)
        self.top = dlrm._acts(dlrm.top_l, dlrm.sigmoid_top)
        self._flatten_params()
        self.ctx.bind_host_tables(host_tables.device_pointers())
        self._bufs = {}
        self.iter = 0
        self.comm = S.new_stream(self.dev) if self.multi else None
        self.side = S.new_stream(self.dev)
        self.pref = S.new_stream(self.dev)
        self.agg_rows = None
        self.agg_chunk_rows = 1 << 16
        self.lazy_merge = True
        self.merge_budget_rows = 1 << 16
        self.merge_budget_auto = True
        self._pump = None
        self._pref = None
        self._phase = 0
        self._emb_done = None
        ne = lambda: S.new_event(self.dev)
        self._events = dict(probed={k: ne() for k in range(4)}, probed_inline=ne(), gathered=ne(), interacted=ne(),
                            emb_done=ne(), wgrad_done=ne(), top_dz=ne(), top_updated=ne(), fwd_mark=ne(), res_slot=ne(),
                            tier_marked=ne())
        if S.is_hip(self.dev):
            cur = S.current_stream(self.dev)
            for e in list(self._events["probed"].values()) + [v for k, v in self._events.items() if k != "probed"]:
                e.record(cur)
        self._head_scratch = ops.head_scratch(self.dev)
        self.stat_acc = torch.zeros(2, dtype=torch.float64, device=self.dev)
        self.loss_sync = True
        l_last, a_last = self.top[-1]
        self.fused_head = l_last.out_features == 1 and a_last == 2
        self.wst = self.pref
        self.split_wgrad_min = 2049
        self.gather_alone_min = 16384
        self.wide_gemm = True
        self.fuse_once = True
        self.sort_chunks = True
        self.sort_slice = 2
        self.sort_st = self.pref
        self._cur_sorted = self._next_sorted = None
        self._next_waited = self._cur_waited = 0
        self.slice_wait = True
        self._last_sort_ev = None
        self.evict_victim = False
        self._vwb_work = {}
        self._gslot = None
        self._res = self._next_res = None
        self._tapes = {}
        self.tape_fallbacks = []
        self.use_tape = S.is_hip(self.dev)
        self.native_tape = True
        self.tape_lanes = 3
        self.tape_lanes_below = 4096
        self.attach_events = True
        self.fuse_gather = True
        self.place_resolve_min = 8192
        self.mark_next = False
        self._mark_this = False
        self._fwd_marked = False
        self._pending_resolve = None

    def _flatten_params(self):
        lin = _linears(self.dlrm.bot_l) + _linears(self.dlrm.top_l)
        top0 = _linears(self.dlrm.top_l)[0]
        kp = {l: ((l.in_features + 3) // 4 * 4 if l is top0 else l.in_features) for l in lin}
        nw = sum(l.out_features * kp[l] for l in lin)
        nb = sum(l.bias.numel() for l in lin)
        self.param_flat = torch.zeros(nw + nb, dtype=torch.float32, device=self.dev)
        self.grad_flat = torch.zeros(nw + nb, dtype=torch.float32, device=self.dev)
        self.n_weight = nw
        nbot = len(_linears(self.dlrm.bot_l))
        nw_bot = sum(l.out_features * kp[l] for l in lin[:nbot])
        nb_bot = sum(l.bias.numel() for l in lin[:nbot])
        self.rng_bot = (0, nw_bot, nw, nb_bot)
        self.rng_top = (nw_bot, nw - nw_bot, nw + nb_bot, nb - nb_bot)
        self._grad_views = (self.grad_flat[nw_bot:nw], self.grad_flat[0:nw_bot])
        off_w, off_b = 0, nw
        self.W, self.gW, self.gb = {}, {}, {}
        for l in lin:
            n = l.out_features * kp[l]
            Wp = self.param_flat[off_w:off_w + n].view(l.out_features, kp[l])
            Wp[:, :l.in_features].copy_(l.weight.data)
            self.W[l] = Wp
            l.weight.data = Wp[:, :l.in_features]
            self.gW[l] = self.grad_flat[off_w:off_w + n].view(l.out_features, kp[l])
            l.weight.grad = self.gW[l][:, :l.in_features]
            off_w += n
            m = l.bias.numel()
            self.param_flat[off_b:off_b + m].copy_(l.bias.data)
            l.bias.data = self.param_flat[off_b:off_b + m]
            self.gb[l] = self.grad_flat[off_b:off_b + m]
            l.bias.grad = self.gb[l]
            off_b += m
        self.r_width = kp[top0]

    def _issue_resolve(self, pr, rec, main, placed: bool):
        pst, ev = self.pref, self._events
        if placed:
            if not self._fwd_marked:
                rec(ev["fwd_mark"].record, main)
            rec(pst.wait_event, ev["fwd_mark"])
        elif pr["first"]:
            pst.wait_stream(main)
        rec(ev["res_slot"].record, self.side)
        rec(pst.wait_event, ev["res_slot"])
        if self.multi:
            rec(pst.wait_event, ev["tier_marked"])
        ops.window_resolve(self.ctx, pr["cols"], pr["lbs"], pr["ws"], pr["wsrc"], stream=pst, batch_len=pr["B"])
        if S.is_hip(self.dev):
            ops.event_record(pr["ev"], pst)
        else:
            pr["ev"].record(pst)

    def flush_pending_resolve(self):
        pr, self._pending_resolve = self._pending_resolve, None
        self.mark_next = False
        if pr is not None:
            self._issue_resolve(pr, lambda fn, *a: fn(*a), S.current_stream(self.dev), placed=False)

    def _fused_gather(self, lS_o) -> bool:
        return bool(self.fuse_gather and lS_o is None and not self.cat and S.is_hip(self.dev)
                    and ops.gather_interact_supported(self.ctx))

    def _side_gather(self, B: int) -> bool:
        return B < self.gather_alone_min and not (self.defer_top and self.cat)

    def _chain(self, B: int, next_idx, lS_o) -> bool:
        return not self._side_gather(B) and next_idx is not None and self._next_res is not None and lS_o is None

    def _take(self, idx, res, phase: int, which, st):
        out = self._probe_bufs(idx.shape[1], which)
        if res is None:
            return ops.embbag_probe(self.ctx, idx, stream=st, aux_phase=phase, out=out)
        ops.embbag_take(self.ctx, idx, res[0], res[1], out[0], aux_phase=phase, stream=st)
        return out

    def _wait_slices(self, cur, nxt, B: int, next_idx):
        if not self.slice_wait:
            return
        if nxt is not None and nxt[5] != self._next_waited:
            (self.pref if self.ctx.aux_phases >= 2 and not self._chain(B, next_idx, None) else self.side).wait_event(nxt[4])
            self._next_waited = nxt[5]
        if cur is not None and cur[5] != self._cur_waited:
            self.side.wait_event(cur[4])
            self._cur_waited = cur[5]

    def _reduce_avg(self) -> bool:
        r = getattr(self, "_avg_ok", None)
        if r is None:
            W = self.world
            r = (W & (W - 1)) == 0 and dist.get_backend(self.pg) == "nccl"
            self._avg_ok = r
        return r

    def _mm(self, l) -> dict:
        if self.matmul_precision == "fp32":
            return {}
        assert self.matmul_precision == "bf16", "matmul_precision: 'fp32' or 'bf16', not %r" % (self.matmul_precision,)
        return {"bf16": True} if ops.bf16_eligible(l.out_features, self.W[l].shape[1]) else {}

    def _wplans(self, buf):
        if self.matmul_precision == "fp32":
            return buf["wgrad"], buf["wgrad_split"]
        self._mm(self.bot[0][0])
        if "wgrad_bf16" not in buf:
            xs, dzs, layers, B, dev = buf["wgrad_args"]
            gw = [self.gW[l] for l in layers]
            gb = [self.gb[l] for l in layers]
            wk = lambda ls: ops.mlp_wgrad_work(B, [l.out_features for l in ls], [self.W[l].shape[1] for l in ls], dev,
                                               precision="bf16")
            whole, split = None, None
            if buf["wgrad_split"] is None:
                whole = ops.WgradPlan(xs, dzs, gw, gb, wk(layers), precision="bf16")
            else:
                nb = len(self.bot)
                split = (ops.WgradPlan(xs[:nb], dzs[:nb], gw[:nb], gb[:nb], wk(layers[:nb]), precision="bf16"),
                         ops.WgradPlan(xs[nb:], dzs[nb:], gw[nb:], gb[nb:], wk(layers[nb:]), precision="bf16"))
                split[0].set_params([self.W[l] for l in layers[:nb]], [l.bias.data for l in layers[:nb]])
                split[1].set_params([self.W[l] for l in layers[nb:]], [l.bias.data for l in layers[nb:]])
            buf["wgrad_bf16"] = (whole, split)
        return buf["wgrad_bf16"]

    def _buffers(self, B):
        if B in self._bufs:
            return self._bufs[B]
        dev, D, F = self.dev, self.D, self.F
        f32 = torch.float32
        npairs = F * (F + 1) // 2 if self.itself else F * (F - 1) // 2
        b = dict()
        if self.cat:
            assert self.r_width >= F * D
            b["R"] = torch.zeros(B + 1, self.r_width, dtype=f32, device=dev)[:B]
            b["dR"] = torch.zeros(B + 1, self.r_width, dtype=f32, device=dev)[:B]
            b["feat"] = b["R"].as_strided((B, F, D), (self.r_width, D, 1))
            b["dfeat"] = b["dR"].as_strided((B, F, D), (self.r_width, D, 1))
        else:
            b["feat"] = torch.zeros(B + 1, F, D, dtype=f32, device=dev)[:B]
            b["dfeat"] = torch.zeros(B + 1, F, D, dtype=f32, device=dev)[:B]
            assert self.r_width >= D + npairs
            b["R"] = torch.zeros(B, self.r_width, dtype=f32, device=dev)
            b["dR"] = torch.zeros(B, self.r_width, dtype=f32, device=dev)
        b["Zc"] = torch.empty(B, 1, dtype=f32, device=dev) if self.loss_threshold > 0.0 else None
        b["bot_y"] = [torch.empty(B, l.out_features, dtype=f32, device=dev) for l, _ in self.bot[:-1]]
        b["bot_dy"] = [torch.empty(B, l.out_features, dtype=f32, device=dev) for l, _ in self.bot[:-1]]
        b["top_y"] = [torch.empty(B, l.out_features, dtype=f32, device=dev) for l, _ in self.top]
        b["top_dy"] = [torch.empty(B, l.out_features, dtype=f32, device=dev) for l, _ in self.top]
        b["loss"] = torch.zeros(65, dtype=f32, device=dev)
        work = 0
        for l, _ in self.bot + self.top:
            work = max(work, ops.linear_bwd_work(B, l.out_features, self.W[l].shape[1], dev).numel())
        work = max(work, ops.mlp_wgrad_work(B, [l.out_features for l, _ in self.bot + self.top],
                                            [self.W[l].shape[1] for l, _ in self.bot + self.top], dev).numel())
        b["lin_work"] = torch.empty(work, dtype=torch.uint8, device=dev)
        layers = [l for l, _ in self.bot + self.top]
        x0 = torch.empty(B, self.W[layers[0]].shape[1], dtype=f32, device=dev)
        xs = [x0] + b["bot_y"] + [b["R"]] + b["top_y"][:-1]
        dzs = b["bot_dy"] + [b["dfeat"][:, 0, :]] + b["top_dy"]
        b["wgrad"] = ops.WgradPlan(xs, dzs, [self.gW[l] for l in layers], [self.gb[l] for l in layers], b["lin_work"])
        b["wgrad_args"] = (xs, dzs, layers, B, dev)
        b["wgrad_split"] = None
        if self.defer_top or (S.is_hip(dev) and B >= self.split_wgrad_min):
            nb = len(self.bot)
            gw = [self.gW[l] for l in layers]
            gb = [self.gb[l] for l in layers]
            wk = lambda ls: ops.mlp_wgrad_work(B, [l.out_features for l in ls], [self.W[l].shape[1] for l in ls], dev)
            b["wgrad_split"] = (ops.WgradPlan(xs[:nb], dzs[:nb], gw[:nb], gb[:nb], wk(layers[:nb])),
                                ops.WgradPlan(xs[nb:], dzs[nb:], gw[nb:], gb[nb:], wk(layers[nb:])))
            b["wgrad_split"][0].set_params([self.W[l] for l in layers[:nb]], [l.bias.data for l in layers[:nb]])
            b["wgrad_split"][1].set_params([self.W[l] for l in layers[nb:]], [l.bias.data for l in layers[nb:]])
        self._bufs[B] = b
        return b

    def _probe_bufs(self, n, which):
        key = ("probe", n, which)
        if key not in self._bufs:
            i32 = torch.int32
            self._bufs[key] = (torch.empty(self.T, n, dtype=i32, device=self.dev),
                               torch.empty(self.T, n, dtype=i32, device=self.dev),
                               torch.empty(self.T, dtype=i32, device=self.dev))
        return self._bufs[key]

    def _emb_work(self, n):
        key = ("emb", n)
        if key not in self._bufs:
            self._bufs[key] = ops.embbag_bwd_work(self.ctx, n, self.dev)
        return self._bufs[key]

    def sync_touched_to_rank0(self):
        if not self.multi:
            return
        ctx = self.ctx
        self._pump_finish()
        self._agg_alloc()
        self._agg_flags.copy_(self.cg.touched)
        dist.all_reduce(self._agg_flags, op=dist.ReduceOp.MAX, group=self.pg)
        U = self._agg_list(self._agg_flags)
        if U == 0:
            return
        buf = self._agg_buffer(U)
        ops.agg_gather(ctx, self.agg_rows, self.agg_count, 1.0, buf, U)
        dist.broadcast(buf, src=0, group=self.pg)
        ops.agg_scatter(ctx, self.agg_rows, self.agg_count, buf, U)

    def _agg_alloc(self):
        if self.agg_rows is None:
            self.agg_rows = torch.empty(self.ctx.total_rows, dtype=torch.int64, device=self.dev)
            self.agg_count = torch.zeros(1, dtype=torch.int64, device=self.dev)
            self.agg_count_host = S.pinned(torch.zeros(1, dtype=torch.int64), self.dev)
            self._agg_flags = torch.zeros(self.ctx.total_rows, dtype=torch.uint8, device=self.dev)
            self._agg_counted = S.new_event(self.dev)
            self._agg_buf = None

    def _agg_list(self, flags) -> int:
        ops.agg_compact(self.ctx, flags, self.agg_rows, self.agg_count)
        self.agg_count_host.copy_(self.agg_count, non_blocking=True)
        self._agg_counted.record(S.current_stream(self.dev))
        self._agg_counted.synchronize()
        return int(self.agg_count_host[0])

    def _agg_buffer(self, U: int) -> torch.Tensor:
        if self._agg_buf is None or self._agg_buf.shape[0] < U:
            cap = 1 << max(12, (U - 1).bit_length())
            self._agg_buf = torch.empty(min(cap, self.ctx.total_rows), self.D, dtype=torch.float32, device=self.dev)
        return self._agg_buf[:U]

    def step(self, X: torch.Tensor, lS_i: torch.Tensor, T: torch.Tensor, lS_o: Optional[torch.Tensor] = None,
             j: Optional[int] = None, gather_events: Optional[list] = None, next_idx: Optional[torch.Tensor] = None,
             res=None, next_res=None, loss_sync: bool = True):
        B, n = X.shape[0], lS_i.shape[1]
        if self.evict_victim:
            assert not self.multi, "--evict-victim-cache is defined for one rank (every rank would write its own misses' rows)"
            next_idx = next_res = None
        self.loss_sync = bool(loss_sync) or not self.fused_head
        self._mark_this = bool(self.mark_next and self._pending_resolve is not None and lS_o is None)
        self.mark_next = False
        self._res, self._next_res = res, (next_res if next_idx is not None else None)
        if lS_o is not None:
            assert lS_o.shape[1] in (B, B + 1)
        if j is None:
            j = self.iter
        sgd_done = False
        if gather_events is None:
            self._gslot = None
        elif isinstance(gather_events, tuple):
            self._gslot = gather_events
        else:
            self._gslot = (ops.TimingEvent(), ops.TimingEvent())
            gather_events.append(self._gslot)
        if self._pump is not None:
            p, pos = self._pump, (res[3] if (res is not None and len(res) > 3) else None)
            if pos is None or pos[0] is not p["rs"] or pos[1] != p["j0"] + (self.iter - p["step0"]):
                self._pump_finish()
        if self._pump is not None:
            self._pump_wait()
        self._cur_sorted = self._next_sorted = None
        if lS_o is None and not self.evict_victim:
            if res is not None and len(res) > 3:
                self._cur_sorted = res[3][0].sorted_views(res[3][1])
            if self._next_res is not None and len(next_res) > 3:
                self._next_sorted = next_res[3][0].sorted_views(next_res[3][1])
            pf = self._pref
            if (self._cur_sorted is not None and pf is not None and pf["ptr"] == lS_i.data_ptr()
                    and pf["shape"] == tuple(lS_i.shape) and not pf.get("sorted_ok")):
                self._cur_sorted = None
            self._wait_slices(self._cur_sorted, self._next_sorted, B, next_idx)
        if res is not None:
            self.side.wait_event(res[2])
        if self._next_res is not None and next_res[2] is not (res[2] if res is not None else None):
            self.side.wait_event(next_res[2])
        if self.use_tape and lS_o is None and not self.evict_victim:
            sgd_done = self._step_taped(X, lS_i, T, next_idx)
        else:
            sgd_done = self._fwd_bwd(X, lS_i, T, lS_o, gather_events, next_idx)
        if self.evict_victim:
            if n not in self._vwb_work:
                self._vwb_work[n] = ops.victim_writeback_work(self.ctx, n)
            ops.victim_writeback(self.ctx, lS_i, self._last_slots, res[1] if (res is not None and lS_o is None) else None,
                                 self._last_phase, self._vwb_work[n], stream=self.side)
        if self._mark_this:
            self._pending_resolve = None
        if self.multi and self.defer_top:
            wst, W = self.wst, float(self.world)
            gt, gb = self._grad_views
            avg = self._reduce_avg()
            with S.on_stream(wst):
                if avg:
                    dist.all_reduce(gt, op=dist.ReduceOp.AVG, group=self.pg)
                else:
                    ops.scale_div(gt, W, stream=wst)
                    dist.all_reduce(gt, op=dist.ReduceOp.SUM, group=self.pg)
                ops.sgd_step2(self.param_flat, self.grad_flat, *self.rng_top, self.lr, stream=wst)
                self._events["top_updated"].record(wst)
            if avg:
                dist.all_reduce(gb, op=dist.ReduceOp.AVG, group=self.pg)
            else:
                ops.scale_div(gb, W)
                dist.all_reduce(gb, op=dist.ReduceOp.SUM, group=self.pg)
            if next_idx is None or not (self._side_gather(B) and self.ctx.aux_phases >= 2):
                S.current_stream(self.dev).wait_event(self._events["emb_done"])
            ops.sgd_step2(self.param_flat, self.grad_flat, *self.rng_bot, self.lr)
            sgd_done = True
        elif self.multi:
            gw = self.grad_flat[:self.n_weight]
            if self._reduce_avg():
                dist.all_reduce(gw, op=dist.ReduceOp.AVG, group=self.pg)
            else:
                ops.scale_div(gw, float(self.world))
                dist.all_reduce(gw, op=dist.ReduceOp.SUM, group=self.pg)
            S.current_stream(self.dev).wait_event(self._events["emb_done"])
        if not sgd_done:
            ops.sgd_step(self.param_flat, self.grad_flat, self.lr)
        if j is None:
            j = self.iter
        if self.multi and j > 0 and j % self.agg_freq == 0:
            if self._emb_done is not None:
                S.current_stream(self.dev).wait_event(self._emb_done)
            self.table_aggregate()
            self.side.wait_stream(S.current_stream(self.dev))
        elif self._pump is not None:
            self._pump_advance()
        self.iter += 1
        return self._buffers(B)["loss"]
# ... 37 lines not shown
            if self._gslot is not None:
                ops.time_next_gather(ctx, self._gslot[0], self._gslot[1])
            ops.embbag_fwd(ctx, slots, lS_o, feat[:, 1:, :], feat.stride(0), D, n_bags=n_bags, stream=st)

        side_gather = self._side_gather(B)
        if side_gather:
            rec(side.wait_event, probed)
            if self.defer_top and not self.cat and not top_waited:
                rec(side.wait_event, ev["top_updated"])
                top_waited = True
            gather(side)
            rec(ev["gathered"].record, side)
        cur = X
        bot_acts = [X]
        for i, (l, act) in enumerate(self.bot):
            y = feat[:, 0, :] if i == len(self.bot) - 1 else buf["bot_y"][i]
            ops.linear_fwd(cur, self.W[l], l.bias.data, y, act, alone=self.wide_gemm, **self._mm(l))
            bot_acts.append(y)
            cur = y
        if side_gather:
            rec(main.wait_event, ev["gathered"])
        else:
            rec(main.wait_event, probed)
            gather(main)
        if next_idx is not None and two_phase:
            pst = self.pref
            if B >= self.gather_alone_min:
                ev_g = ev["gathered"]
                rec(ev_g.record, main)
                rec(pst.wait_event, ev_g)
            if self._emb_done is not None:
                rec(pst.wait_event, self._emb_done)
            ph = 1 - self._phase
            res = self._take(next_idx, self._next_res, ph, ph, pst)
            evp = ev["probed"][ph]
            rec(evp.record, pst)
            self._pref = dict(ptr=next_idx.data_ptr(), shape=tuple(next_idx.shape), phase=ph,
                              res=(res[0], res[1], res[2], evp), sorted_ok=self._next_sorted is not None)
        emb_work = self._emb_work(n)
        if not side_gather:
            rec(side.wait_event, probed)
        attach = self.attach_events and S.is_hip(self.dev)
        sv = self._cur_sorted if (lS_o is None and n == B) else None
        once = bool(self.fuse_once and fused and sv is not None)
        if sv is None and not prepared:
            ops.embbag_bwd_prepare(ctx, slots, emb_work, stream=side)
        if self.defer_top and not self.cat and not top_waited:
            rec(main.wait_event, ev["top_updated"])
        self._fwd_marked = False
        if fused:
            if self._gslot is not None:
                ops.time_next_gather(ctx, self._gslot[0], self._gslot[1])
            if attach and self._mark_this:
                ops.event_attach_next(ev["fwd_mark"], main)
                self._fwd_marked = True
            ops.gather_interact_fwd(ctx, slots, feat[:, 0, :], self.itself, R)
        elif not self.cat:
            ops.interact_fwd(feat, self.itself, R)
        if self._mark_this:
            self._issue_resolve(self._pending_resolve, rec, main, placed=True)
        cur = R
        top_acts = [R]
        fused_head = self.fused_head
        for i, (l, act) in enumerate(self.top):
            y = buf["top_y"][i]
            if not (fused_head and i == len(self.top) - 1):
                ops.linear_fwd(cur, self.W[l], l.bias.data, y, act, alone=self.wide_gemm, **self._mm(l))
            top_acts.append(y)
            cur = y
        Z = cur
        last_act = self.top[-1][1]
        whole_plan, split = self._wplans(buf)
        wst = self.wst
        sgd_in_wgrad = self.defer_top and not self.multi

        n_top = len(self.top)
        if fused_head:
            l = self.top[-1][0]
            dX = dR if n_top == 1 else buf["top_dy"][-2]
            ops.head_fwd_bwd(top_acts[-2][:, :l.in_features], self.W[l], l.bias.data, T, Z, buf["top_dy"][-1],
                             dX[:, :l.in_features], buf["loss"], self._head_scratch,
                             x_act=(self.top[-2][1] if n_top > 1 else 0), kind=self.loss_kind,
                             weights=self.loss_weights, threshold=self.loss_threshold, Zc=buf["Zc"], finish=False)
            if self.loss_sync:
                ops.head_finish(self._head_scratch, B, buf["loss"], acc=self.stat_acc)
            dY = dX
        else:
            ops.loss_fwd_bwd(Z, T, buf["loss"], buf["top_dy"][-1], kind=self.loss_kind, weights=self.loss_weights,
                             threshold=self.loss_threshold, Zc=buf["Zc"], sigmoid_bwd=(last_act == 2))
            rec(self.stat_acc.add_, buf["loss"][1:3])
            dY = buf["top_dy"][-1]
        for i in reversed(range(n_top - 1 if fused_head else n_top)):
            l, act = self.top[i]
            if i == len(self.top) - 1 and act == 2:
                act = 0
            elif i < len(self.top) - 1:
                act = 0
            dX = dR if i == 0 else buf["top_dy"][i - 1]
            if i == 0 and attach and split is not None:
                ops.event_attach_next(ev["top_dz"], main)
            ops.linear_bwd(top_acts[i], self.W[l], top_acts[i + 1], dY, dX, None, None, act,
                           buf["lin_work"], x_act=(self.top[i - 1][1] if i > 0 else 0), alone=self.wide_gemm, **self._mm(l))
            dY = dX
        if split is not None:
            if not (attach and n_top - (1 if fused_head else 0) > 0):
                rec(ev["top_dz"].record, main)
            rec(wst.wait_event, ev["top_dz"])
            ops.mlp_wgrad(split[1], stream=wst, lr=self.lr if sgd_in_wgrad else None)
            if not self.defer_top:
                rec(ev["wgrad_done"].record, wst)
            elif not self.multi:
                rec(ev["top_updated"].record, wst)
        if self.cat:
            ops.act_bwd(dfeat[:, 0, :], feat[:, 0, :], self.bot[-1][1])
        else:
            if attach:
                ops.event_attach_next(ev["interacted"], main)
            if once:
                ops.gather_interact_bwd_sgd(ctx, slots, feat[:, 0, :], dR, self.itself, dfeat, sv[2], sv[3], self.lr_embeds,
                                            x_act=self.bot[-1][1])
            elif fused:
                ops.gather_interact_bwd(ctx, slots, feat[:, 0, :], dR, self.itself, dfeat, x_act=self.bot[-1][1])
            else:
                ops.interact_bwd(feat, dR, self.itself, dfeat, x_act=self.bot[-1][1])
        if not attach or self.cat:
            rec(ev["interacted"].record, main)
        rec(side.wait_event, ev["interacted"])
        if fused_head and not self.loss_sync:
            ops.head_finish(self._head_scratch, B, buf["loss"], stream=side, acc=self.stat_acc)
        if sv is not None:
            ops.embbag_bwd_apply_sorted(ctx, n, dfeat[:, 1:, :], dfeat.stride(0), D, self.lr_embeds, emb_work, sv[0], sv[1], sv[3],
                                        self._phase, once, cg.touched if self.multi else None, stream=side)
        else:
            ops.embbag_bwd_apply(ctx, n, lS_o, dfeat[:, 1:, :], dfeat.stride(0), D, self.lr_embeds, emb_work,
                                 cg.touched if self.multi else None, stream=side)
        emb_done = ev["emb_done"]
        rec(emb_done.record, side)
        self._emb_done = emb_done
        if next_idx is not None and not two_phase:
            which = 2 + (self.iter & 1)
            res = self._take(next_idx, self._next_res, 0, which, side)
            chain_sort = chain and self._next_sorted is None
            if chain_sort:
                ops.embbag_bwd_prepare(ctx, res[0], emb_work, stream=side)
            chained_top = chain and sgd_in_wgrad and split is not None
            if chained_top:
                rec(side.wait_event, ev["top_updated"])
            evp = ev["probed"][which]
            rec(evp.record, side)
            self._pref = dict(ptr=next_idx.data_ptr(), shape=tuple(next_idx.shape), phase=0,
                              res=(res[0], res[1], res[2], evp), chained_top=chained_top, prepared=chain_sort,
                              sorted_ok=self._next_sorted is not None)
        dY = dfeat[:, 0, :]
        for i in reversed(range(1, len(self.bot))):
            l, act = self.bot[i]
            dX = buf["bot_dy"][i - 1]
            ops.linear_bwd(bot_acts[i], self.W[l], bot_acts[i + 1], dY, dX, None, None, 0,
                           buf["lin_work"], x_act=self.bot[i - 1][1], **self._mm(l))
            dY = dX
        if split is not None:
            split[0].set_x(0, X)
            ops.mlp_wgrad(split[0], lr=self.lr if sgd_in_wgrad else None)
            if not self.defer_top:
                rec(main.wait_event, ev["wgrad_done"])
        else:
            plan = whole_plan
            plan.set_x(0, X)
            ops.mlp_wgrad(plan)
        if self.multi:
            return False
        if next_idx is None:
            rec(main.wait_stream, side)
        elif chain:
            pass
        elif not (side_gather and two_phase):
            rec(main.wait_event, emb_done)
        return split is not None and sgd_in_wgrad

    def evaluate(self, X: torch.Tensor, lS_i: torch.Tensor, lS_o: Optional[torch.Tensor] = None) -> torch.Tensor:
        ctx = self.ctx
        B, n = X.shape[0], lS_i.shape[1]
        assert n <= ctx.aux, "test batch larger than the aux table (test_mini_batch_size <= aux_table_size)"
        if self._pump is not None:
            raise RuntimeError("evaluate(): a row merge is still draining; every rank has to call drain_merge() first")
        self.finish()
        pend = self._pref
        if pend is not None and pend["phase"] == self._phase:
            S.current_stream(self.dev).wait_event(pend["res"][3])
            self._pref = None
        buf = self._buffers(B)
        feat, R = buf["feat"], buf["R"]
        F, D = self.F, self.D
        slots, _, _ = ops.embbag_probe(ctx, lS_i, aux_phase=self._phase, out=self._probe_bufs(n, "eval"))
        cur = X
        for i, (l, act) in enumerate(self.bot):
            y = feat[:, 0, :] if i == len(self.bot) - 1 else buf["bot_y"][i]
            ops.linear_fwd(cur, self.W[l], l.bias.data, y, act, **self._mm(l))
            cur = y
        if self._fused_gather(lS_o):
            ops.gather_interact_fwd(ctx, slots, feat[:, 0, :], self.itself, R)
        else:
            ops.embbag_fwd(ctx, slots, lS_o, feat[:, 1:, :], feat.stride(0), D, n_bags=(B if lS_o is None else lS_o.shape[1]))
            if not self.cat:
                ops.interact_fwd(feat, self.itself, R)
        cur = R
        for i, (l, act) in enumerate(self.top):
            y = buf["top_y"][i]
            ops.linear_fwd(cur, self.W[l], l.bias.data, y, act, alone=self.wide_gemm, **self._mm(l))
            cur = y
        if self.loss_threshold > 0.0:
            cur = torch.clamp(cur, min=self.loss_threshold, max=1.0 - self.loss_threshold)
        return cur

    def drain_merge(self):
        self._pump_finish()

    def finish(self):
        if self.defer_top:
            S.current_stream(self.dev).wait_event(self._events["top_updated"])
        if self._emb_done is not None:
            S.current_stream(self.dev).wait_event(self._emb_done)
        self._pump_finish()

    def prediction(self, B: int) -> torch.Tensor:
        buf = self._buffers(B)
        return buf["Zc"] if buf["Zc"] is not None else buf["top_y"][-1]

    def _step_taped(self, X, lS_i, T, next_idx):
        import ctypes as C
        B, n = X.shape[0], lS_i.shape[1]
        main = S.current_stream(self.dev)
        pref = self._pref
        hit = pref is not None and pref["ptr"] == lS_i.data_ptr() and pref["shape"] == tuple(lS_i.shape)
        phase = pref["phase"] if hit else self._phase
        nxt = next_idx is not None
        key = (B, n, main.cuda_stream, hit, phase, nxt, self._emb_done is not None, X.stride(0), lS_i.stride(0),
               next_idx.stride(0) if nxt else 0,
               (self.iter & 1) if (self.ctx.aux_phases < 2 or self._chain(B, next_idx, None)) else 0,
               bool(hit and pref.get("chained_top")), bool(hit and pref.get("prepared")),
               self._gslot is not None, self.loss_sync,
               (int(self._pending_resolve["cols"].shape[1]), self._pending_resolve["cols"].stride(0)) if self._mark_this else None,
               self.tape_lanes, self.tape_lanes_below, self.attach_events, self.fuse_gather, self.wide_gemm, self.fuse_once,
               self.matmul_precision,
               None if self._cur_sorted is None else self._cur_sorted[3], self._next_sorted is not None,
               self._res[0].stride(0) if (self._res is not None and not hit) else 0,
               self._next_res[0].stride(0) if self._next_res is not None else 0)
        tape = self._tapes.get(key)
        if tape is None:
            calls = []
            _lib.start_recording(calls)
            try:
                included = self._fwd_bwd(X, lS_i, T, None, None, next_idx)
                if not self.multi and not included:
                    ops.sgd_step(self.param_flat, self.grad_flat, self.lr)
            finally:
                _lib.stop_recording()
            cells = {k: C.c_void_p(v) for k, v in self._tape_ptrs(X, T, lS_i, next_idx, hit).items()}
            by_value = {c.value: c for c in cells.values()}
            if len(by_value) != len(cells):
                return not self.multi
            prog = []
            for fn, args in calls:
                if getattr(fn, "argtypes", None) is not None:
                    args = tuple(by_value.get(a, a) if isinstance(a, int) and not isinstance(a, bool) else a for a in args)
                    prog.append((fn, args, True))
                else:
                    prog.append((fn, args, False))
            post = self._pref
            native = None
            if self.native_tape and _lib.native_tape_ok():
                try:
                    lanes = self.tape_lanes if B < self.tape_lanes_below else 1
                    native = _lib.NativeTape(prog, cells, main_stream=main.cuda_stream if lanes > 1 else None, max_lanes=lanes)
                except _lib.TapeUnsupported as e:
                    native = None
                    self.tape_fallbacks.append(str(e))
            self._tapes[key] = dict(prog=prog, cells=cells, phase=self._phase, native=native,
                                    pref=None if post is None else (post["phase"], post["res"], post.get("chained_top", False),
                                                                    post.get("prepared", False)))
            return not self.multi
        cells = tape["cells"]
        for k, v in self._tape_ptrs(X, T, lS_i, next_idx, hit).items():
            cells[k].value = v
        bufs = self._buffers(B)
        whole_plan, split = self._wplans(bufs)
        (split[0] if split is not None else whole_plan).set_x(0, X)
        if tape["native"] is not None:
            rc = tape["native"].replay()
            if rc:
                _lib.check(rc)
        else:
            for fn, args, is_lib in tape["prog"]:
                rc = fn(*args)
                if is_lib and rc:
                    _lib.check(rc)
        self._phase = tape["phase"]
        self._emb_done = self._events["emb_done"]
        self._pref = None
        if tape["pref"] is not None:
            self._pref = dict(ptr=next_idx.data_ptr(), shape=tuple(next_idx.shape), phase=tape["pref"][0], res=tape["pref"][1],
                              chained_top=tape["pref"][2], prepared=tape["pref"][3], sorted_ok=self._next_sorted is not None)
        return not self.multi

    def _tape_ptrs(self, X, T, lS_i, next_idx, hit: bool) -> dict:
        p = {"X": X.data_ptr(), "T": T.data_ptr(), "idx": lS_i.data_ptr()}
        if next_idx is not None:
            p["next"] = next_idx.data_ptr()
        if self._res is not None and not hit:
            p["ws"], p["wsrc"] = self._res[0].data_ptr(), self._res[1].data_ptr()
        if self._next_res is not None:
            p["nws"], p["nwsrc"] = self._next_res[0].data_ptr(), self._next_res[1].data_ptr()
        if self._cur_sorted is not None:
            p["skeys"], p["smeta"], p["sonce"] = self._cur_sorted[:3]
        if self._gslot is not None:
            p["g0"], p["g1"] = self._gslot[0].handle, self._gslot[1].handle
        if self._mark_this:
            pr = self._pending_resolve
            p["rcols"], p["rws"] = pr["cols"].data_ptr(), pr["ws"].data_ptr()
            p["rwsrc"], p["rev"] = pr["wsrc"].data_ptr(), int(pr["ev"].cuda_event)
        return p

    MERGE_CLASS_FIRST = (1, 2, 3, 5, 9, 17, 33)
    MERGE_LOOKAHEAD = 64

    def _pump_start(self, U, buf, scale, rop) -> bool:
        pos = self._res[3] if (self._res is not None and len(self._res) > 3) else None
        if pos is None:
            return False
        rs, j = pos
        la = rs.lookahead(j, self.MERGE_LOOKAHEAD)
        if not la:
            return False
        ctx, main = self.ctx, S.current_stream(self.dev)
        first = self.MERGE_CLASS_FIRST
        C = len(first) + 1
        K = la[-1][0]
        if ("agg_tier",) not in self._bufs:
            self._bufs[("agg_tier",)] = (torch.empty(ctx.total_rows, dtype=torch.uint8, device=self.dev),
                                         torch.empty(ctx.total_rows, dtype=torch.int64, device=self.dev),
                                         torch.zeros(C + 1, dtype=torch.int64, device=self.dev),
                                         S.pinned(torch.zeros(C + 1, dtype=torch.int64), self.dev))
        tier, rows_sorted, off_dev, off_host = self._bufs[("agg_tier",)]
        tier.fill_(C - 1)
        seen = set()
        for k, ws, ev in la:
            if id(ev) not in seen:
                main.wait_event(ev)
                seen.add(id(ev))
        for c in reversed(range(C - 1)):
            hi = first[c + 1] if c + 1 < len(first) else self.MERGE_LOOKAHEAD + 1
            for k, ws, ev in la:
                if first[c] <= k < hi:
                    ops.agg_mark_tier(ctx, ws, c, tier)
        ops.agg_split(ctx, self.agg_rows, U, tier, C, rows_sorted, off_dev)
        self._events["tier_marked"].record(main)
        off_host.copy_(off_dev, non_blocking=True)
        self._agg_counted.record(main)
        self._agg_counted.synchronize()
        off = [int(x) for x in off_host.tolist()]
        ready = S.new_event(self.dev)
        ready.record(main)
        budget = int(self.merge_budget_rows)
        if self.merge_budget_auto:
            budget = max(budget, int(rs.lbs) * self.T)
        self._pump = dict(rows=rows_sorted, U=U, buf=buf, scale=scale, rop=rop, off=off, K=K, step0=self.iter, issued=0,
                          waited=0, chunks=[], ready=ready, budget=budget, rs=rs, j0=j)
        self._pump_advance()
        return True

    def _pump_need(self, d: int) -> int:
        p = self._pump
        if d > p["K"]:
            return p["U"]
        need = 0
        for c, f in enumerate(self.MERGE_CLASS_FIRST):
            if f <= d:
                need = p["off"][c + 1]
        return need

    def _pump_issue(self, lo: int, hi: int):
        p, ctx, comm = self._pump, self.ctx, self.comm
        with S.on_stream(comm):
            if not p["chunks"]:
                comm.wait_event(p["ready"])
            ops.agg_gather(ctx, p["rows"][lo:], self.agg_count, p["scale"], p["buf"][lo:hi], hi - lo, first=lo)
            dist.all_reduce(p["buf"][lo:hi], op=p["rop"], group=self.pg)
            ops.agg_scatter(ctx, p["rows"][lo:], self.agg_count, p["buf"][lo:hi], hi - lo, first=lo)
            ev = S.new_event(self.dev)
            ev.record(comm)
        p["chunks"].append((hi, ev))
        p["issued"] = hi

    def _pump_advance(self, everything: bool = False):
        p = self._pump
        if p is None:
            return
# ... 87 lines not shown
```

cdlrm_amd/ops.py:

```python
from __future__ import annotations

import ctypes as C
from typing import List, Optional, Sequence

import torch

from . import _lib
from ._lib import Geometry, Plan, check, ptr, stream_ptr
from ._lib import Victims as _VictimsStruct


def _require_cuda(t: torch.Tensor, name: str):
    if not t.is_cuda:
        raise RuntimeError("cdlrm_amd: %s must live on the MI355X (got %s); there is no CPU path" % (name, t.device))


class CacheCtx:

    def __init__(self, table_rows: Sequence[int], cache_sets: Sequence[int], dim: int, num_ways: int,
                 aux_rows: int, device: torch.device, aux_phases: int = 1):
        self.T = len(table_rows)
        self.D, self.ways, self.aux = int(dim), int(num_ways), int(aux_rows)
        self.aux_phases = max(1, int(aux_phases))
        self.table_rows = [int(x) for x in table_rows]
# ... 341 lines not shown
    def writeback(self, dst_ptrs: Sequence[int], average: bool, stream=None):
        arr = (C.c_void_p * self.ctx.T)(*[int(p) for p in dst_ptrs])
        check(_lib.lib().cdlrm_plan_writeback(self.ctx.handle, C.byref(self.c), arr, 1 if average else 0,
                                              stream_ptr(stream)))


class Victims:

    def __init__(self, ctx: CacheCtx, cap: int):
        dev = ctx.device
        self.cap = max(1, int(cap))
        self.pos = torch.empty(self.cap, dtype=torch.int32, device=dev)
        self.idx = torch.zeros(self.cap, dtype=torch.int64, device=dev)
        self.off = torch.zeros(ctx.T + 2, dtype=torch.int64, device=dev)
        self.rows = torch.empty((self.cap, ctx.D), dtype=torch.float32, device=dev)
        self.c = _VictimsStruct(self.pos.data_ptr(), self.idx.data_ptr(), self.off.data_ptr(), self.rows.data_ptr(),
                                self.cap)


def host_gather_rows(table_ptrs: Sequence[int], idx: torch.Tensor, off: Sequence[int], dim: int, dst: torch.Tensor,
                     threads: int = 16):
    T = len(table_ptrs)
    assert idx.device.type == "cpu" and idx.dtype == torch.int64 and idx.is_contiguous()
    assert dst.device.type == "cpu" and dst.dtype == torch.float32 and dst.is_contiguous() and dst.shape[1] == dim
    assert len(off) == T + 1 and off[-1] <= idx.numel() and off[-1] <= dst.shape[0]
    tp = (C.c_void_p * T)(*[int(p) for p in table_ptrs])
    oa = (C.c_int64 * (T + 1))(*[int(o) for o in off])
    check(_lib.lib().cdlrm_host_gather_rows(tp, idx.data_ptr(), oa, T, int(dim), dst.data_ptr(), int(threads)))


def gather_rows(src_ptr: int, index: torch.Tensor, dim: int, stream=None) -> torch.Tensor:
    _require_cuda(index, "index")
    out = torch.empty((index.numel(), dim), dtype=torch.float32, device=index.device)
    check(_lib.lib().cdlrm_gather_rows(int(src_ptr), index.data_ptr(), index.numel(), dim, out.data_ptr(),
                                       stream_ptr(stream)))
    return out



def agg_compact(ctx: CacheCtx, touched: torch.Tensor, rows_out: torch.Tensor, count_out: torch.Tensor, stream=None):
    check(_lib.lib().cdlrm_agg_compact(ctx.handle, touched.data_ptr(), touched.numel(), rows_out.data_ptr(),
                                       rows_out.numel(), count_out.data_ptr(), stream_ptr(stream)))


def agg_gather(ctx: CacheCtx, rows: torch.Tensor, count: torch.Tensor, scale: float, buf: torch.Tensor, cap: int,
               stream=None, first: int = 0):
    check(_lib.lib().cdlrm_agg_gather(ctx.handle, rows.data_ptr(), count.data_ptr(), float(scale), buf.data_ptr(),
                                      int(cap), int(first), stream_ptr(stream)))


def agg_scatter(ctx: CacheCtx, rows: torch.Tensor, count: torch.Tensor, buf: torch.Tensor, cap: int, stream=None,
                first: int = 0):
    check(_lib.lib().cdlrm_agg_scatter(ctx.handle, rows.data_ptr(), count.data_ptr(), buf.data_ptr(), int(cap),
                                       int(first), stream_ptr(stream)))


def agg_mark_tier(ctx: CacheCtx, slots: torch.Tensor, value: int, tier: torch.Tensor, stream=None):
    assert slots.dtype == torch.int32 and slots.dim() == 2 and slots.shape[0] == ctx.T and slots.stride(1) == 1
    assert tier.dtype == torch.uint8 and tier.numel() == ctx.total_rows
    check(_lib.lib().cdlrm_agg_mark_tier(ctx.handle, slots.data_ptr(), slots.shape[1], slots.stride(0), int(value),
                                         tier.data_ptr(), stream_ptr(stream)))


def agg_split(ctx: CacheCtx, rows: torch.Tensor, count: int, tier: torch.Tensor, n_classes: int, rows_out: torch.Tensor,
              class_off: torch.Tensor, stream=None):
    assert rows.dtype == torch.int64 and rows_out.dtype == torch.int64 and rows_out.numel() >= count
    assert class_off.dtype == torch.int64 and class_off.numel() >= n_classes + 1
    check(_lib.lib().cdlrm_agg_split(ctx.handle, rows.data_ptr(), int(count), tier.data_ptr(), int(n_classes), rows_out.data_ptr(),
                                     class_off.data_ptr(), stream_ptr(stream)))



def interact_fwd(feat: torch.Tensor, itself: bool, R: torch.Tensor, stream=None):
    B, F, D = feat.shape
    check(_lib.lib().cdlrm_interact_fwd(feat.data_ptr(), B, F, D, int(bool(itself)), R.data_ptr(), R.stride(0),
                                        stream_ptr(stream)))


def interact_bwd(feat: torch.Tensor, dR: torch.Tensor, itself: bool, dfeat: torch.Tensor, stream=None, x_act: int = 0):
    B, F, D = feat.shape
    check(_lib.lib().cdlrm_interact_bwd(feat.data_ptr(), dR.data_ptr(), dR.stride(0), B, F, D, int(bool(itself)),
                                        int(x_act), dfeat.data_ptr(), stream_ptr(stream)))


def gather_interact_supported(ctx: CacheCtx) -> bool:
    return bool(_lib.raw().cdlrm_gather_interact_supported(ctx.handle))


def gather_interact_fwd(ctx: CacheCtx, slots: torch.Tensor, x: torch.Tensor, itself: bool, R: torch.Tensor, stream=None):
    B = x.shape[0]
    assert slots.dtype == torch.int32 and slots.stride(1) == 1 and x.stride(1) == 1
    check(_lib.lib().cdlrm_gather_interact_fwd(ctx.handle, slots.data_ptr(), slots.stride(0), x.data_ptr(), x.stride(0), B,
                                               int(bool(itself)), R.data_ptr(), R.stride(0), stream_ptr(stream)))


def gather_interact_bwd(ctx: CacheCtx, slots: torch.Tensor, x: torch.Tensor, dR: torch.Tensor, itself: bool,
                        dfeat: torch.Tensor, stream=None, x_act: int = 0):
    B = x.shape[0]
    assert slots.dtype == torch.int32 and slots.stride(1) == 1 and x.stride(1) == 1 and dfeat.is_contiguous()
    check(_lib.lib().cdlrm_gather_interact_bwd(ctx.handle, slots.data_ptr(), slots.stride(0), x.data_ptr(), x.stride(0),
                                               dR.data_ptr(), dR.stride(0), B, int(bool(itself)), int(x_act),
                                               dfeat.data_ptr(), stream_ptr(stream)))


def gather_interact_bwd_sgd(ctx: CacheCtx, slots: torch.Tensor, x: torch.Tensor, dR: torch.Tensor, itself: bool,
                            dfeat: torch.Tensor, once: int, ld_once: int, lr: float, stream=None, x_act: int = 0):
    B = x.shape[0]
    assert slots.dtype == torch.int32 and slots.stride(1) == 1 and x.stride(1) == 1 and dfeat.is_contiguous()
    check(_lib.lib().cdlrm_gather_interact_bwd_sgd(ctx.handle, slots.data_ptr(), slots.stride(0), x.data_ptr(), x.stride(0),
                                                   dR.data_ptr(), dR.stride(0), B, int(bool(itself)), int(x_act),
                                                   dfeat.data_ptr(), int(once), int(ld_once), float(lr), stream_ptr(stream)))


ACT = {"none": 0, "relu": 1, "sigmoid": 2}


GEMM_ALONE = 0x100
GEMM_BF16 = 0x200
PRECISIONS = {"fp32": 0, "bf16": GEMM_BF16}


def bf16_eligible(N: int, K: int) -> bool:
    return int(N) >= 32 and int(K) >= 32


def _flags(alone: bool = False, bf16: bool = False) -> int:
    return (GEMM_ALONE if alone else 0) | (GEMM_BF16 if bf16 else 0)


def linear_fwd(X: torch.Tensor, W: torch.Tensor, b: Optional[torch.Tensor], Y: torch.Tensor, act: int, stream=None,
               alone: bool = False, bf16: bool = False):
    M, K = X.shape
    N = W.shape[0]
    assert W.shape[1] == K and W.is_contiguous() and X.stride(1) == 1 and Y.stride(1) == 1
    check(_lib.lib().cdlrm_linear_fwd(X.data_ptr(), X.stride(0), W.data_ptr(), ptr(b), Y.data_ptr(), Y.stride(0), M, N,
                                      K, act | _flags(alone, bf16), stream_ptr(stream)))


def linear_bwd_work(M: int, N: int, K: int, device) -> torch.Tensor:
    nbytes = int(_lib.lib().cdlrm_linear_bwd_work_bytes(M, N, K))
    return torch.empty((nbytes + 255) // 256 * 256, dtype=torch.uint8, device=device)


def linear_bwd(X, W, Y, dY, dX, dW, db, act: int, work: torch.Tensor, stream=None, x_act: int = 0, alone: bool = False,
               bf16: bool = False):
    M, K = X.shape
    N = W.shape[0]
    check(_lib.lib().cdlrm_linear_bwd(X.data_ptr(), X.stride(0), W.data_ptr(), ptr(Y), 0 if Y is None else Y.stride(0),
                                      dY.data_ptr(), dY.stride(0), ptr(dX), 0 if dX is None else dX.stride(0),
                                      ptr(dW), ptr(db), M, N, K, act | _flags(alone, bf16), int(x_act), work.data_ptr(),
                                      stream_ptr(stream)))


ROUTE_FAMILIES = {0: None, 1: "smallk_rows", 2: "smallk", 3: "direct", 4: "staged", 5: "gemm2", 6: "gemm3", 7: "gemm",
                  8: "bf16"}


def _route(r: _lib.GemmRoute) -> Optional[dict]:
    fam = ROUTE_FAMILIES[r.family]
    if fam is None:
        return None
    return dict(family=fam, tm=r.tm, tn=r.tn, mode=r.mode, aligned=r.aligned, splits=r.splits, vec_a=r.vec_a, vec_b=r.vec_b,
                fast=r.fast)


def linear_fwd_route(X, W, b, Y, act: int, alone: bool = False, n_cu: int = 256, bf16: bool = False) -> dict:
    M, K = X.shape
    N = W.shape[0]
    out = _lib.GemmRoute()
    check(_lib.raw().cdlrm_linear_fwd_route(X.data_ptr(), X.stride(0), W.data_ptr(), ptr(b), Y.data_ptr(), Y.stride(0), M, N, K,
                                            act | _flags(alone, bf16), None, int(n_cu), C.byref(out)))
    return _route(out)


def linear_bwd_route(X, W, Y, dY, dX, dW, db, act: int, x_act: int = 0, alone: bool = False, n_cu: int = 256,
                     bf16: bool = False):
    M, K = X.shape
    N = W.shape[0]
    out = (_lib.GemmRoute * 2)()
    check(_lib.raw().cdlrm_linear_bwd_route(X.data_ptr(), X.stride(0), W.data_ptr(), ptr(Y), 0 if Y is None else Y.stride(0),
                                            dY.data_ptr(), dY.stride(0), ptr(dX), 0 if dX is None else dX.stride(0), ptr(dW),
                                            ptr(db), M, N, K, act | _flags(alone, bf16), int(x_act), 256, None,
                                            int(n_cu), out))
    return _route(out[0]), _route(out[1])


def _wgrad_work_bytes(M: int, Ns, Ks, precision: str) -> int:
    n = len(Ns)
    NA = C.c_int32 * n
    N, K = NA(*[int(x) for x in Ns]), NA(*[int(x) for x in Ks])
    if precision == "fp32":
        return int(_lib.lib().cdlrm_mlp_wgrad_work_bytes(n, int(M), N, K))
    return int(_lib.lib().cdlrm_mlp_wgrad_work_bytes_ex(n, int(M), N, K, PRECISIONS[precision]))


def mlp_wgrad_work(M: int, Ns: Sequence[int], Ks: Sequence[int], device, precision: str = "fp32") -> torch.Tensor:
    nbytes = _wgrad_work_bytes(M, Ns, Ks, precision)
    return torch.empty((nbytes + 255) // 256 * 256, dtype=torch.uint8, device=device)


class WgradPlan:

    def __init__(self, Xs, dZs, dWs, dbs, work: torch.Tensor, precision: str = "fp32"):
        import ctypes as C
        assert precision in PRECISIONS, precision
        self.precision = precision
        n = len(Xs)
        assert len(dZs) == n and len(dWs) == n and len(dbs) == n
        self.n = n
        self.M = int(dZs[0].shape[0])
        self._keep = (list(Xs), list(dZs), list(dWs), list(dbs), work)
        PA, IA, NA = C.c_void_p * n, C.c_int64 * n, C.c_int32 * n
        self.X = PA(*[x.data_ptr() for x in Xs])
        self.ld_x = IA(*[x.stride(0) for x in Xs])
        self.dZ = PA(*[d.data_ptr() for d in dZs])
        self.ld_dz = IA(*[d.stride(0) for d in dZs])
        self.dW = PA(*[w.data_ptr() for w in dWs])
        self.db = PA(*[ptr(b) for b in dbs])
        self.N = NA(*[int(w.shape[0]) for w in dWs])
        self.K = NA(*[int(w.shape[1]) for w in dWs])
        for x, d, w in zip(Xs, dZs, dWs):
            assert x.shape[0] == self.M and d.shape[0] == self.M and x.stride(1) == 1 and d.stride(1) == 1
            assert w.is_contiguous() and d.shape[1] == w.shape[0] and x.shape[1] <= w.shape[1] <= x.stride(0)
        need = _wgrad_work_bytes(self.M, list(self.N), list(self.K), precision)
        assert work.numel() * work.element_size() >= need and work.data_ptr() % 256 == 0, "work too small: ops.mlp_wgrad_work"
        self.work = work

    def set_x(self, i: int, x: torch.Tensor):
        assert x.shape[0] == self.M and x.stride(1) == 1
        self.X[i] = x.data_ptr()
        self.ld_x[i] = x.stride(0)
        self._keep[0][i] = x

    def set_params(self, Ws, bs):
        import ctypes as C
        assert len(Ws) == self.n and len(bs) == self.n
        for i, w in enumerate(Ws):
            assert w.is_contiguous() and tuple(w.shape) == (int(self.N[i]), int(self.K[i]))
        PA = C.c_void_p * self.n
        self.P_w = PA(*[w.data_ptr() for w in Ws])
        self.P_b = PA(*[ptr(b) for b in bs])
        self._params = (list(Ws), list(bs))


def mlp_wgrad(plan: WgradPlan, stream=None, lr: Optional[float] = None):
    if plan.precision != "fp32":
        flags = PRECISIONS[plan.precision]
        if lr is None:
            check(_lib.lib().cdlrm_mlp_wgrad_ex(plan.n, plan.X, plan.ld_x, plan.dZ, plan.ld_dz, plan.dW, plan.db, plan.M, plan.N,
                                                plan.K, flags, plan.work.data_ptr(), stream_ptr(stream)))
        else:
            check(_lib.lib().cdlrm_mlp_wgrad_sgd_ex(plan.n, plan.X, plan.ld_x, plan.dZ, plan.ld_dz, plan.dW, plan.db, plan.P_w,
                                                    plan.P_b, float(lr), plan.M, plan.N, plan.K, flags, plan.work.data_ptr(),
                                                    stream_ptr(stream)))
        return
    if lr is None:
        check(_lib.lib().cdlrm_mlp_wgrad(plan.n, plan.X, plan.ld_x, plan.dZ, plan.ld_dz, plan.dW, plan.db, plan.M, plan.N,
                                         plan.K, plan.work.data_ptr(), stream_ptr(stream)))
    else:
        check(_lib.lib().cdlrm_mlp_wgrad_sgd(plan.n, plan.X, plan.ld_x, plan.dZ, plan.ld_dz, plan.dW, plan.db, plan.P_w,
                                             plan.P_b, float(lr), plan.M, plan.N, plan.K, plan.work.data_ptr(),
                                             stream_ptr(stream)))


def mlp_wgrad_route(plan: WgradPlan, n_cu: int = 256, precision: Optional[str] = None) -> list:
    out = (_lib.GemmRoute * max(plan.n, 1))()
    flags = PRECISIONS[precision or plan.precision]
    check(_lib.raw().cdlrm_mlp_wgrad_route(plan.n, plan.X, plan.ld_x, plan.dZ, plan.ld_dz, plan.dW, plan.db, plan.M, plan.N,
                                           plan.K, flags, int(n_cu), out))
    return [_route(out[i]) for i in range(plan.n)]


def bce_fwd_bwd(Z: torch.Tensor, target: torch.Tensor, loss_buf: torch.Tensor, dZ: Optional[torch.Tensor], stream=None,
                sigmoid_bwd: bool = False):
    assert loss_buf.numel() >= 65
    check(_lib.lib().cdlrm_bce_fwd_bwd(Z.data_ptr(), target.data_ptr(), Z.numel(), loss_buf.data_ptr(), ptr(dZ),
                                       1 if sigmoid_bwd else 0, stream_ptr(stream)))


LOSS = {"bce": 0, "mse": 1, "wbce": 2}


def loss_fwd_bwd(Z: torch.Tensor, target: torch.Tensor, loss_buf: torch.Tensor, dZ: Optional[torch.Tensor], *,
                 kind: int = 0, weights=(1.0, 1.0), threshold: float = 0.0, Zc: Optional[torch.Tensor] = None,
                 sigmoid_bwd: bool = False, stream=None):
    check(_lib.lib().cdlrm_loss_fwd_bwd(Z.data_ptr(), target.data_ptr(), Z.numel(), int(kind), float(weights[0]),
                                        float(weights[1]), float(threshold), loss_buf.data_ptr(), ptr(dZ), ptr(Zc),
                                        1 if sigmoid_bwd else 0, stream_ptr(stream)))


def head_scratch(device) -> torch.Tensor:
    return torch.zeros(int(_lib.lib().cdlrm_head_scratch_floats()), dtype=torch.float32, device=device)


def head_fwd_bwd(Y: torch.Tensor, w: torch.Tensor, bias: Optional[torch.Tensor], target: torch.Tensor, Z: torch.Tensor,
                 dZ: torch.Tensor, dY: Optional[torch.Tensor], loss_buf: torch.Tensor, scratch: torch.Tensor, *,
                 x_act: int = 0, kind: int = 0, weights=(1.0, 1.0), threshold: float = 0.0,
                 Zc: Optional[torch.Tensor] = None, finish: bool = True, stream=None):
    B, K = Y.shape
    assert Y.stride(1) == 1 and w.numel() >= K and Z.numel() == B and dZ.numel() == B and target.numel() == B
    assert dY is None or (dY.shape == Y.shape and dY.stride(1) == 1)
    check(_lib.lib().cdlrm_head_fwd_bwd(Y.data_ptr(), Y.stride(0), w.data_ptr(), ptr(bias), target.data_ptr(), B, K,
                                        int(kind), float(weights[0]), float(weights[1]), float(threshold), int(x_act),
                                        Z.data_ptr(), ptr(Zc), dZ.data_ptr(), ptr(dY), 0 if dY is None else dY.stride(0),
                                        loss_buf.data_ptr(), scratch.data_ptr(), 1 if finish else 0, stream_ptr(stream)))


def head_finish(scratch: torch.Tensor, B: int, loss_buf: torch.Tensor, stream=None, acc: Optional[torch.Tensor] = None):
# ... 118 lines not shown
```

include/cdlrm_hip.h:

```cpp
#ifndef CDLRM_HIP_H
#define CDLRM_HIP_H

#include <stdint.h>

#ifdef __cplusplus
extern "C" {
#endif

#define CDLRM_ABI_VERSION 1

#define CDLRM_EINVAL (-22)
#define CDLRM_ERANGE (-34)
#define CDLRM_ENOMEM (-12)

typedef struct cdlrm_ctx cdlrm_ctx;

typedef struct {
    int32_t num_tables;
    int32_t dim;
    int32_t num_ways;
    int32_t aux_rows;
    const int64_t* table_rows;
    const int64_t* cache_sets;
    int32_t device;
// ... 73 lines not shown
    int32_t arange;
    int32_t lpr;
    int32_t reserved;
    int64_t apply_grid_x, apply_grid_y;
    int64_t long_grid;
    int64_t keys_off, meta_off, once_off;
    int64_t apply_keys_off;
} cdlrm_emb_bwd_route;
int cdlrm_embbag_bwd_route(int32_t num_tables, int32_t dim, int64_t n, int32_t has_offsets, int32_t entry, int32_t nb,
                           int32_t j0, int32_t count, cdlrm_emb_bwd_route* out);


typedef struct {
    uint64_t* bitmap;
    int64_t*  uniq;
    int64_t*  uniq_off;
    int64_t   cap_uniq;
    uint64_t* prot;
    uint8_t*  hit;
    int32_t*  kept;
    int64_t*  kept_off;
    uint8_t*  way;
    uint8_t*  flags;
    int32_t*  winner;
    int32_t*  win_claim;
    int64_t*  win_idx;
    int64_t*  win_row;
    int64_t*  win_tag;
    int64_t*  win_off;
    int64_t   cap_win;
    float*    stage;
    int64_t*  ev_tag;
} cdlrm_plan;

int cdlrm_window_unique(cdlrm_ctx* ctx, const cdlrm_plan* plan, const int64_t* idx, int64_t n,
                        int64_t ld_idx, void* stream);
int cdlrm_window_unique_add(cdlrm_ctx* ctx, const cdlrm_plan* plan, const int64_t* idx, int64_t n,
                            int64_t ld_idx, void* stream);
int cdlrm_window_unique_finish(cdlrm_ctx* ctx, const cdlrm_plan* plan, void* stream);

int cdlrm_plan_probe(cdlrm_ctx* ctx, const cdlrm_plan* plan, void* stream);

int cdlrm_plan_offsets_sync(cdlrm_ctx* ctx, const cdlrm_plan* plan, int64_t* uniq_off,
                            int64_t* kept_off, int64_t* win_off, void* stream);

int cdlrm_plan_assign(cdlrm_ctx* ctx, const cdlrm_plan* plan, const float* q, uint64_t seed,
                      void* stream);

int cdlrm_plan_fetch(cdlrm_ctx* ctx, const cdlrm_plan* plan, const float* const* src_rows,
                     int by_position, void* stream);

int cdlrm_plan_commit(cdlrm_ctx* ctx, const cdlrm_plan* plan, void* stream);

int cdlrm_plan_writeback(cdlrm_ctx* ctx, const cdlrm_plan* plan, float* const* dst_rows,
                         int average, void* stream);

typedef struct {
    int32_t* pos;
    int64_t* idx;
    int64_t* off;
    float*   rows;
    int64_t  cap;
} cdlrm_victims;
int cdlrm_plan_victims(cdlrm_ctx* ctx, const cdlrm_plan* plan, const cdlrm_victims* victims, void* stream);
int cdlrm_plan_victims_list(cdlrm_ctx* ctx, const cdlrm_plan* plan, const cdlrm_victims* victims, void* stream);

int cdlrm_host_gather_rows(const float* const* tables, const int64_t* idx, const int64_t* off, int32_t T,
                           int32_t D, float* dst, int32_t nthreads);
int cdlrm_ctx_bind_victims(cdlrm_ctx* ctx, const cdlrm_victims* victims);

int cdlrm_gather_rows(const float* src, const int64_t* index, int64_t count, int32_t dim,
                      float* out, void* stream);

int cdlrm_scatter_rows(float* dst, const int64_t* index, const float* rows, int64_t count,
                       int32_t dim, int average, void* stream);
int cdlrm_blend_rows(const float* dst, const int64_t* index, const float* rows, int64_t count,
                     int32_t dim, float* out, void* stream);

int cdlrm_qr_embbag_fwd(const int64_t* idx, const int64_t* offsets, int64_t n, int64_t n_bags,
                        const float* Wq, const float* Wr, int64_t rows_q, int32_t collisions, int32_t dim,
                        int32_t op, float* out, float* eq_out, float* er_out, int32_t* err_word, void* stream);
int cdlrm_qr_embbag_bwd(const int64_t* idx, const int64_t* offsets, int64_t n, int64_t n_bags,
                        const float* eq, const float* er, const float* grad_out, int64_t rows_q,
                        int32_t collisions, int32_t dim, int32_t op, float* gWq, float* gWr, void* stream);

int cdlrm_bag_fwd(const int64_t* idx, const int64_t* offsets, int64_t n, int64_t n_bags, const float* W, int64_t rows,
                  int32_t dim, float* out, int32_t* err_word, void* stream);
int cdlrm_bag_bwd(const int64_t* idx, const int64_t* offsets, int64_t n, int64_t n_bags, const float* grad_out,
                  int64_t rows, int32_t dim, float* gW, void* stream);


int cdlrm_mark_rows(cdlrm_ctx* ctx, const int32_t* slots, int64_t n, uint8_t* touched, void* stream);

int cdlrm_agg_compact(cdlrm_ctx* ctx, uint8_t* touched, int64_t total_rows, int64_t* rows_out,
                      int64_t cap, int64_t* count_out, void* stream);
int cdlrm_agg_gather(cdlrm_ctx* ctx, const int64_t* rows, const int64_t* count, float scale,
                     float* buf, int64_t cap, int64_t first, void* stream);
int cdlrm_agg_scatter(cdlrm_ctx* ctx, const int64_t* rows, const int64_t* count, const float* buf,
                      int64_t cap, int64_t first, void* stream);
int cdlrm_agg_mark_tier(cdlrm_ctx* ctx, const int32_t* slots, int64_t n, int64_t ld, int32_t value, uint8_t* tier, void* stream);
int cdlrm_agg_split(cdlrm_ctx* ctx, const int64_t* rows, int64_t count, const uint8_t* tier, int32_t n_classes,
                    int64_t* rows_out, int64_t* class_off, void* stream);


int cdlrm_interact_fwd(const float* feat, int64_t B, int32_t F, int32_t D, int32_t itself,
                       float* R, int64_t ld_r, void* stream);
int cdlrm_interact_bwd(const float* feat, const float* dR, int64_t ld_r, int64_t B, int32_t F,
                       int32_t D, int32_t itself, int32_t x_act, float* dfeat, void* stream);
int cdlrm_gather_interact_supported(cdlrm_ctx* ctx);
int cdlrm_gather_interact_fwd(cdlrm_ctx* ctx, const int32_t* slots, int64_t n, const float* x, int64_t ld_x, int64_t B,
                              int32_t itself, float* R, int64_t ld_r, void* stream);
int cdlrm_gather_interact_bwd(cdlrm_ctx* ctx, const int32_t* slots, int64_t n, const float* x, int64_t ld_x,
                              const float* dR, int64_t ld_r, int64_t B, int32_t itself, int32_t x_act, float* dfeat,
                              void* stream);
int cdlrm_gather_interact_bwd_sgd(cdlrm_ctx* ctx, const int32_t* slots, int64_t n, const float* x, int64_t ld_x,
                                  const float* dR, int64_t ld_r, int64_t B, int32_t itself, int32_t x_act, float* dfeat,
                                  const uint8_t* once, int64_t ld_once, float lr, void* stream);
#define CDLRM_GEMM_ALONE 0x100
#define CDLRM_GEMM_BF16 0x200
int cdlrm_linear_fwd(const float* X, int64_t ld_x, const float* W, const float* bias, float* Y,
                     int64_t ld_y, int64_t M, int32_t N, int32_t K, int32_t act, void* stream);
uint64_t cdlrm_linear_bwd_work_bytes(int64_t M, int32_t N, int32_t K);
int cdlrm_linear_bwd(const float* X, int64_t ld_x, const float* W, const float* Y, int64_t ld_y,
                     float* dY, int64_t ld_dy, float* dX, int64_t ld_dx, float* dW, float* db,
                     int64_t M, int32_t N, int32_t K, int32_t act, int32_t x_act, void* work,
                     void* stream);

#define CDLRM_ROUTE_NONE 0
#define CDLRM_ROUTE_SMALLK_ROWS 1
#define CDLRM_ROUTE_SMALLK 2
#define CDLRM_ROUTE_DIRECT 3
#define CDLRM_ROUTE_STAGED 4
#define CDLRM_ROUTE_GEMM2 5
#define CDLRM_ROUTE_GEMM3 6
#define CDLRM_ROUTE_GEMM 7
#define CDLRM_ROUTE_BF16 8
typedef struct cdlrm_gemm_route {
    int32_t family;
    int32_t tm, tn;
    int32_t mode;
    int32_t aligned;
    int32_t splits;
    int32_t vec_a, vec_b;
    int32_t fast;
} cdlrm_gemm_route;
int cdlrm_linear_fwd_route(const float* X, int64_t ld_x, const float* W, const float* bias, float* Y,
                           int64_t ld_y, int64_t M, int32_t N, int32_t K, int32_t act, void* stream, int32_t n_cu,
                           cdlrm_gemm_route* out);
int cdlrm_linear_bwd_route(const float* X, int64_t ld_x, const float* W, const float* Y, int64_t ld_y,
                           float* dY, int64_t ld_dy, float* dX, int64_t ld_dx, float* dW, float* db,
                           int64_t M, int32_t N, int32_t K, int32_t act, int32_t x_act, void* work,
                           void* stream, int32_t n_cu, cdlrm_gemm_route* out);

uint64_t cdlrm_mlp_wgrad_work_bytes(int32_t n_layers, int64_t M, const int32_t* N, const int32_t* K);
int cdlrm_mlp_wgrad(int32_t n_layers, const float* const* X, const int64_t* ld_x, const float* const* dZ,
                    const int64_t* ld_dz, float* const* dW, float* const* db, int64_t M, const int32_t* N,
                    const int32_t* K, void* work, void* stream);
int cdlrm_mlp_wgrad_sgd(int32_t n_layers, const float* const* X, const int64_t* ld_x, const float* const* dZ,
                        const int64_t* ld_dz, float* const* dW, float* const* db, float* const* W, float* const* b,
                        float lr, int64_t M, const int32_t* N, const int32_t* K, void* work, void* stream);

uint64_t cdlrm_mlp_wgrad_work_bytes_ex(int32_t n_layers, int64_t M, const int32_t* N, const int32_t* K, int32_t flags);
int cdlrm_mlp_wgrad_ex(int32_t n_layers, const float* const* X, const int64_t* ld_x, const float* const* dZ,
                       const int64_t* ld_dz, float* const* dW, float* const* db, int64_t M, const int32_t* N,
                       const int32_t* K, int32_t flags, void* work, void* stream);
int cdlrm_mlp_wgrad_sgd_ex(int32_t n_layers, const float* const* X, const int64_t* ld_x, const float* const* dZ,
                           const int64_t* ld_dz, float* const* dW, float* const* db, float* const* W, float* const* b,
                           float lr, int64_t M, const int32_t* N, const int32_t* K, int32_t flags, void* work, void* stream);
int cdlrm_mlp_wgrad_route(int32_t n_layers, const float* const* X, const int64_t* ld_x, const float* const* dZ,
                          const int64_t* ld_dz, float* const* dW, float* const* db, int64_t M, const int32_t* N,
                          const int32_t* K, int32_t flags, int32_t n_cu, cdlrm_gemm_route* out);

int cdlrm_bce_fwd_bwd(const float* Z, const float* target, int64_t n, float* loss_out, float* dZ,
                      int32_t sigmoid_bwd, void* stream);

int cdlrm_loss_fwd_bwd(const float* Z, const float* target, int64_t n, int32_t kind, float w0, float w1,
                       float threshold, float* loss_out, float* dZ, float* Zc, int32_t sigmoid_bwd, void* stream);

int64_t cdlrm_head_scratch_floats(void);
int cdlrm_head_fwd_bwd(const float* Y, int64_t ldy, const float* w, const float* bias, const float* target,
                       int64_t B, int32_t K, int32_t kind, float w0, float w1, float threshold, int32_t x_act,
                       float* Z, float* Zc, float* dZ, float* dY, int64_t lddy, float* loss_out, float* scratch,
                       int32_t finish, void* stream);
int cdlrm_head_finish(const float* scratch, int64_t B, float* loss_out, double* acc, void* stream);

int cdlrm_sgd_step(float* param, const float* grad, int64_t n, float lr, void* stream);

int cdlrm_act_bwd(float* dX, int64_t lddx, const float* X, int64_t ldx, int64_t M, int32_t N, int32_t act, void* stream);

int cdlrm_sgd_step2(float* param, const float* grad, int64_t off0, int64_t n0, int64_t off1, int64_t n1, float lr,
                    void* stream);

int cdlrm_scale_div(float* x, int64_t n, float divisor, void* stream);

int cdlrm_synth_indices(int64_t* out, int64_t count, int64_t first, int64_t n_rows, double alpha, uint64_t key, void* stream);

int cdlrm_bags_window(const int64_t* buf, int64_t total, const int64_t* bpos, int32_t L, int32_t T, int64_t n_win,
                      int64_t* out, void* stream);
int cdlrm_bags_rank_slice(const int64_t* buf, int64_t total, const int64_t* bpos, int32_t L, int32_t b, int32_t T,
                          const int64_t* off, int64_t nbag, int64_t s0, int64_t s1, int64_t n, int64_t* idx, int64_t* off_out,
                          void* stream);

int cdlrm_dayfile_window(const int32_t* x_int, const int32_t* x_cat, const int32_t* y, int64_t n, int32_t n_dense, int32_t n_cat,
                         int64_t max_ind_range, float* X, int64_t* lS_i, int64_t lS_i_pitch, int64_t col0, float* T,
                         void* stream);
int cdlrm_dayfile_tile(void);

typedef struct cdlrm_tape cdlrm_tape;
cdlrm_tape* cdlrm_tape_create(int32_t n_cells);
void cdlrm_tape_destroy(cdlrm_tape* t);
int cdlrm_tape_add(cdlrm_tape* t, void* fn, int32_t n_int, const int64_t* iargs, const int32_t* cell, int32_t n_flt,
                   const float* fargs);
int64_t* cdlrm_tape_cells(cdlrm_tape* t);
int64_t cdlrm_tape_length(cdlrm_tape* t);
int32_t cdlrm_tape_stream_arg(void* fn);
const char* cdlrm_tape_op_info(cdlrm_tape* t, int64_t k, int64_t* out);
int cdlrm_tape_replay(cdlrm_tape* t);
int cdlrm_tape_set_lanes(cdlrm_tape* t, const int32_t* lane, const int32_t* dep, int64_t n);
int cdlrm_tape_selftest(void);
int cdlrm_tape_probe(float f0, int64_t a0, float f1, int32_t a1, void* a2, int64_t a3, float f2, int32_t a4, int64_t a5,
                     int64_t a6, void* a7, int32_t a8, float f3, int64_t a9);
int cdlrm_tape_probe_log(int64_t tag, int64_t spin);
int64_t cdlrm_tape_probe_log_take(int64_t* out, int64_t cap);
int cdlrm_event_record(void* event, void* stream);
int cdlrm_stream_wait_event(void* stream, void* event);
int cdlrm_event_attach_next(void* event, void* stream);
void* cdlrm_stream_create(int32_t priority);
int cdlrm_stream_destroy(void* stream);
void* cdlrm_event_create(int32_t timing);
int cdlrm_event_destroy(void* event);
int cdlrm_event_elapsed_us(void* start, void* stop, float* us);
int cdlrm_ctx_time_next_gather(cdlrm_ctx* ctx, void* start_event, void* stop_event);

#ifdef __cplusplus
}
#endif
#endif
```

Measured before the change: 15.26 million.

## Fold thin first-layer bottom-MLP weight gradient into the layer-1 dgrad GEMM epilogue

When the first bottom-MLP layer has 16 or fewer inputs, the dgrad GEMM of layer 1 now parks each output tile in LDS. It then computes per-tile partial weight and bias gradients for layer 0 directly from those tiles and the raw inputs. A small reduce kernel sums the per-tile partials and can optionally apply the SGD update. This removes a separate wgrad pass that would re-read the full dZ for layer 0, at the cost of extra LDS traffic, a sync in the GEMM epilogue, and a per-tile partial buffer.

```diff
diff --git a/cdlrm_amd/_lib.py b/cdlrm_amd/_lib.py
--- a/cdlrm_amd/_lib.py
+++ b/cdlrm_amd/_lib.py
@@ -111,6 +111,11 @@
     "cdlrm_linear_bwd_work_bytes": (c_u64, [c_i64, c_i32, c_i32]),
     "cdlrm_linear_bwd": (C.c_int, [vp, c_i64, vp, vp, c_i64, vp, c_i64, vp, c_i64, vp, vp, c_i64, c_i32, c_i32,
                                    c_i32, c_i32, vp, vp]),
+    "cdlrm_linear_bwd_fold_work_bytes": (c_u64, [c_i64, c_i32, c_i32]),
+    "cdlrm_linear_bwd_ex": (C.c_int, [vp, c_i64, vp, vp, c_i64, vp, c_i64, vp, c_i64, vp, vp, c_i64, c_i32, c_i32,
+                                      c_i32, c_i32, vp, vp, c_i64, c_i32, vp, vp, vp, vp, c_f32, vp, vp]),
+    "cdlrm_linear_bwd_ex_route": (C.c_int, [vp, c_i64, vp, vp, c_i64, vp, c_i64, vp, c_i64, vp, vp, c_i64, c_i32, c_i32,
+                                            c_i32, c_i32, vp, vp, c_i64, c_i32, vp, vp, c_i32, C.POINTER(GemmRoute)]),
     "cdlrm_linear_fwd_route": (C.c_int, [vp, c_i64, vp, vp, vp, c_i64, c_i64, c_i32, c_i32, c_i32, vp, c_i32,
                                          C.POINTER(GemmRoute)]),
     "cdlrm_linear_bwd_route": (C.c_int, [vp, c_i64, vp, vp, c_i64, vp, c_i64, vp, c_i64, vp, vp, c_i64, c_i32, c_i32,
diff --git a/cdlrm_amd/csrc/ctx.hip b/cdlrm_amd/csrc/ctx.hip
--- a/cdlrm_amd/csrc/ctx.hip
+++ b/cdlrm_amd/csrc/ctx.hip
@@ -21,7 +21,7 @@
 extern "C" int cdlrm_debug_set(int32_t key, int32_t value) {
     CDLRM_REQUIRE(key >= 0 && key < 8, "key: 0 .. 7");
 #ifndef CDLRM_DEV
-    CDLRM_REQUIRE(!(key == 6 && (value & 3)), "work-skipping switches (key 6, bits 1 and 2) exist in -DCDLRM_DEV builds only");
+    CDLRM_REQUIRE(!(key == 6 && (value & 7)), "work-skipping switches (key 6, bits 1, 2 and 4) exist in -DCDLRM_DEV builds only");
 #endif
     g_cdlrm_debug[key] = value;
     return 0;
diff --git a/cdlrm_amd/csrc/dense.hip b/cdlrm_amd/csrc/dense.hip
--- a/cdlrm_amd/csrc/dense.hip
+++ b/cdlrm_amd/csrc/dense.hip
@@ -278,6 +278,40 @@
                       r.splits, r.outB, red, r.pA, r.pB, r.lr, r.novec);
 }
 
+__global__ void __launch_bounds__(256) k_reduce_fold(const float* __restrict__ partA, int64_t countA, float* __restrict__ outA,
+                                                     float* __restrict__ pA, int gxa, const float* __restrict__ partB,
+                                                     int64_t countB, float* __restrict__ outB, float* __restrict__ pB, int slabs,
+                                                     float lr) {
+    __shared__ float4 red[16][16];
+    const int el = threadIdx.x & 15, sub = threadIdx.x >> 4;
+    const bool isb = (int)blockIdx.x >= gxa;
+    const float4* __restrict__ part = reinterpret_cast<const float4*>(isb ? partB : partA);
+    const int64_t n4 = (isb ? countB : countA) >> 2;
+    float* __restrict__ out = isb ? outB : outA;
+    float* __restrict__ p = isb ? pB : pA;
+    const int64_t e = (int64_t)((int)blockIdx.x - (isb ? gxa : 0)) * 16 + el;
+    float4 s = make_float4(0.f, 0.f, 0.f, 0.f);
+    if (e < n4) {
+#pragma unroll 8
+        for (int z = sub; z < slabs; z += 16) {
+            const float4 v = part[(int64_t)z * n4 + e];
+            s.x += v.x; s.y += v.y; s.z += v.z; s.w += v.w;
+        }
+    }
+    red[sub][el] = s;
+    __syncthreads();
+    if (sub != 0 || e >= n4) return;
+    float4 t = red[0][el];
+#pragma unroll
+    for (int u = 1; u < 16; ++u) { const float4 v = red[u][el]; t.x += v.x; t.y += v.y; t.z += v.z; t.w += v.w; }
+    const float g[4] = {t.x, t.y, t.z, t.w};
+#pragma unroll
+    for (int u = 0; u < 4; ++u) {
+        out[4 * e + u] = g[u];
+        if (p) p[4 * e + u] = fmaf(-lr, g[u], p[4 * e + u]);
+    }
+}
+
 #define WGRAD_DIRECT_MAX_M 2048
 static int wgrad_splits(int64_t M, int N, int K) {
     if (M <= WGRAD_DIRECT_MAX_M) return 1;
@@ -311,9 +345,35 @@
     return total;
 }
 
+struct FoldReq {
+    const float* x; int64_t ldx; int k;
+    float* dW; float* db;
+    float* P_w; float* P_b; float lr;
+    void* work;
+    cdlrm_gemm_route* rout;
+};
+
+extern "C" uint64_t cdlrm_linear_bwd_fold_work_bytes(int64_t M, int32_t K, int32_t k_below) {
+    if (M < 1 || K < 1 || k_below < 1) return 0;
+    const uint64_t tiles = (uint64_t)cdiv(M, 64);
+    return ((tiles * K * k_below * 4 + 255) & ~(uint64_t)255) + ((tiles * K * 4 + 255) & ~(uint64_t)255) + 256;
+}
+
+static bool fold_tile(const GemmArgs& g, int k_below, int n_cu, int* tm, int* tn) {
+    if (g.M <= WGRAD_DIRECT_MAX_M || k_below < 1 || k_below > G2_FOLD_KMAX) return false;
+    cdlrm_gemm_route r;
+    memset(&r, 0, sizeof(r));
+    const GemmRec rec = {&r, n_cu};
+    if (launch_gemm<true, false>(g, 1, nullptr, &rec) != 0) return false;
+    if (r.family != CDLRM_ROUTE_GEMM2 || r.splits != 1 || (r.tm == 2 && r.tn == 2)) return false;
+    *tm = r.tm;
+    *tn = r.tn;
+    return true;
+}
+
 static int linear_bwd(const float* X, int64_t ld_x, const float* W, const float* Y, int64_t ld_y, float* dY, int64_t ld_dy,
                       float* dX, int64_t ld_dx, float* dW, float* db, int64_t M, int32_t N, int32_t K, int32_t act,
-                      int32_t x_act, void* work, void* stream, const GemmRec* rec) {
+                      int32_t x_act, void* work, void* stream, const GemmRec* rec, const FoldReq* fold = nullptr) {
     const int alone = (act & CDLRM_GEMM_ALONE) != 0;
     const int bf16 = (act & CDLRM_GEMM_BF16) != 0 && bf16_layer_ok(N, K);
     act &= ~(CDLRM_GEMM_ALONE | CDLRM_GEMM_BF16);
@@ -338,6 +398,31 @@
         g.vecB = aligned16(W) && K % 4 == 0;
         g.mask = X; g.ldmask = ld_x; g.mask_act = x_act;
         g.alone = alone;
+        int ftm = 0, ftn = 0;
+        const bool folded = fold && !bf16 && fold_tile(g, fold->k, rec ? rec->n_cu : gemm_device_cus(), &ftm, &ftn);
+        if (fold && !rec)
+            CDLRM_REQUIRE(folded, "no fold for this call (fp32 LDS-DMA dgrad at M > 2048 only): ask cdlrm_linear_bwd_ex_route");
+        if (folded) {
+            const int64_t tiles = cdiv(M, 64 * ftm);
+            if (rec) {
+                gemm_record(rec, CDLRM_ROUTE_GEMM2, ftm, ftn, 0, 0, 1, 1, 1, g2_full_ok<false>(g));
+                const GemmRec frec = {fold->rout, rec->n_cu};
+                gemm_record(&frec, CDLRM_ROUTE_FOLD, ftm, ftn, 0, 0, (int)tiles, 1, 1, 0);
+                return 0;
+            }
+            const int64_t cnt = (int64_t)K * fold->k;
+            G2Fold f;
+            f.x = fold->x; f.ldx = fold->ldx; f.k = fold->k;
+            f.dw = (float*)fold->work;
+            f.db = fold->db ? (float*)((char*)fold->work + ((((uint64_t)tiles * cnt * 4) + 255) & ~(uint64_t)255)) : nullptr;
+            launch_gemm2_fold(g, f, ftm, ftn, s);
+            const int gxa = (int)cdiv(cnt >> 2, 16), gxb = fold->db ? (int)cdiv(K >> 2, 16) : 0;
+            hipLaunchKernelGGL(k_reduce_fold, dim3((unsigned)(gxa + gxb)), dim3(256), 0, s, (const float*)f.dw, cnt, fold->dW,
+                               fold->P_w, gxa, (const float*)f.db, (int64_t)K, fold->db, fold->db ? fold->P_b : nullptr, (int)tiles,
+                               fold->lr);
+            CDLRM_LAUNCH_CHECK();
+            return 0;
+        }
         int rc = bf16 ? launch_gemm_bf16<true, false>(g, s, rec) : launch_gemm<true, false>(g, 1, s, rec);
         if (rc) return rc;
     }
@@ -404,6 +489,46 @@
     memset(out, 0, 2 * sizeof(*out));
     const GemmRec rec[2] = {{out, n_cu}, {out + 1, n_cu}};
     return linear_bwd(X, ld_x, W, Y, ld_y, dY, ld_dy, dX, ld_dx, dW, db, M, N, K, act, x_act, work, stream, rec);
+}
+
+static int fold_check(const float* x_below, int64_t ld_x_below, int32_t k_below, float* dW_below, float* db_below, float* P_w,
+                      float* P_b, const void* work_below, bool query, float* dX, float* dW, float* db, int32_t act, int32_t K) {
+    CDLRM_REQUIRE(k_below >= 1 && ld_x_below >= k_below && dW_below, "bad argument for the layer below");
+    CDLRM_REQUIRE(dX && !dW && !db && (act & 0xff) == 0, "the fold rides on a dgrad-only call (dX, no dW / db, act = 0)");
+    CDLRM_REQUIRE(K % 4 == 0, "the layer below needs a multiple of four outputs");
+    CDLRM_REQUIRE(P_w || !P_b, "P_b without P_w");
+    CDLRM_REQUIRE(query || (work_below && ((uintptr_t)work_below & 255) == 0), "work_below must be 256-byte aligned");
+    (void)x_below;
+    return 0;
+}
+
+extern "C" int cdlrm_linear_bwd_ex(const float* X, int64_t ld_x, const float* W, const float* Y, int64_t ld_y, float* dY,
+                                   int64_t ld_dy, float* dX, int64_t ld_dx, float* dW, float* db, int64_t M, int32_t N,
+                                   int32_t K, int32_t act, int32_t x_act, void* work, const float* x_below, int64_t ld_x_below,
+                                   int32_t k_below, float* dW_below, float* db_below, float* P_w, float* P_b, float lr,
+                                   void* work_below, void* stream) {
+    if (!x_below) return cdlrm_linear_bwd(X, ld_x, W, Y, ld_y, dY, ld_dy, dX, ld_dx, dW, db, M, N, K, act, x_act, work, stream);
+    CdlrmStopScope stop_scope;
+    stop_scope.hold((hipStream_t)stream);
+    int rc = fold_check(x_below, ld_x_below, k_below, dW_below, db_below, P_w, P_b, work_below, false, dX, dW, db, act, K);
+    if (rc) return rc;
+    const FoldReq fold = {x_below, ld_x_below, (int)k_below, dW_below, db_below, P_w, P_b, lr, work_below, nullptr};
+    return linear_bwd(X, ld_x, W, Y, ld_y, dY, ld_dy, dX, ld_dx, dW, db, M, N, K, act, x_act, work, stream, nullptr, &fold);
+}
+
+extern "C" int cdlrm_linear_bwd_ex_route(const float* X, int64_t ld_x, const float* W, const float* Y, int64_t ld_y, float* dY,
+                                         int64_t ld_dy, float* dX, int64_t ld_dx, float* dW, float* db, int64_t M, int32_t N,
+                                         int32_t K, int32_t act, int32_t x_act, void* work, const float* x_below,
+                                         int64_t ld_x_below, int32_t k_below, float* dW_below, float* db_below, int32_t n_cu,
+                                         cdlrm_gemm_route* out) {
+    CDLRM_REQUIRE(out && n_cu >= 1, "bad argument");
+    memset(out, 0, 3 * sizeof(*out));
+    const GemmRec rec[2] = {{out, n_cu}, {out + 1, n_cu}};
+    if (!x_below) return linear_bwd(X, ld_x, W, Y, ld_y, dY, ld_dy, dX, ld_dx, dW, db, M, N, K, act, x_act, work, nullptr, rec);
+    int rc = fold_check(x_below, ld_x_below, k_below, dW_below, db_below, nullptr, nullptr, nullptr, true, dX, dW, db, act, K);
+    if (rc) return rc;
+    const FoldReq fold = {x_below, ld_x_below, (int)k_below, dW_below, db_below, nullptr, nullptr, 0.f, nullptr, out + 2};
+    return linear_bwd(X, ld_x, W, Y, ld_y, dY, ld_dy, dX, ld_dx, dW, db, M, N, K, act, x_act, work, nullptr, rec, &fold);
 }
 
 __global__ void __launch_bounds__(256) k_sgd(float* __restrict__ p, const float* __restrict__ g, int64_t n, float lr);
@@ -560,6 +685,12 @@
     for (int i = 0; i < n_layers; ++i) {
         CDLRM_REQUIRE(X[i] && dZ[i] && dW[i] && N[i] >= 1 && K[i] >= 1 && ld_x[i] >= K[i] && ld_dz[i] >= N[i],
                       "bad layer argument");
+#ifdef CDLRM_DEV
+        if ((g_cdlrm_debug[6] & 4) && !rout && (N[i] <= 32 || K[i] <= 32)) {
+            stepped[i] = 1;
+            continue;
+        }
+#endif
         const int splits = wgrad_splits(M, N[i], K[i]);
         const int64_t cnt = (int64_t)N[i] * K[i];
         GemmArgs g = gemm_args();
diff --git a/cdlrm_amd/csrc/gemm_glds.h b/cdlrm_amd/csrc/gemm_glds.h
--- a/cdlrm_amd/csrc/gemm_glds.h
+++ b/cdlrm_amd/csrc/gemm_glds.h
@@ -77,9 +77,21 @@
     }
 }
 
+struct G2Fold {
+    const float* x; int64_t ldx; int k;
+    float* dw;
+    float* db;
+};
+#define G2_FOLD_KMAX 16
 template <int TM, int TN>
+__device__ __forceinline__ void g2_park(float* park, int lrow, int lcol, const float4& v) {
+    float* p = park + lrow * (64 * TN + 1) + lcol;
+    p[0] = v.x; p[1] = v.y; p[2] = v.z; p[3] = v.w;
+}
+
+template <int TM, int TN, bool FOLD = false>
 __device__ __forceinline__ void g2_epilogue(const GemmArgs& g, f32x16 (&acc)[TM][TN], int64_t m0, int64_t n0, unsigned bz,
-                                            int wm, int wn, int lane) {
+                                            int wm, int wn, int lane, float* park = nullptr) {
     float* C = g.C + (int64_t)bz * g.slab;
     const bool vbias = g.bias != nullptr && (((uintptr_t)g.bias) & 15) == 0;
     const bool vmask = g.mask_act != 0 && (((uintptr_t)g.mask) & 15) == 0 && (g.ldmask & 3) == 0;
@@ -91,7 +103,10 @@
 #pragma unroll
             for (int q = 0; q < 4; ++q) {
                 const int64_t col = n0 + wn * (32 * TN) + j * 32 + 8 * q + 4 * (lane >> 5);
-                if (row >= g.M || col >= g.N) continue;
+                if (row >= g.M || col >= g.N) {
+                    if (FOLD) g2_park<TM, TN>(park, (int)(row - m0), (int)(col - n0), make_float4(0.f, 0.f, 0.f, 0.f));
+                    continue;
+                }
                 float4 v = make_float4(acc[i][j][4 * q], acc[i][j][4 * q + 1], acc[i][j][4 * q + 2], acc[i][j][4 * q + 3]);
                 if (g.bias) {
                     float4 bv;
@@ -120,14 +135,15 @@
                     }
                 }
                 *reinterpret_cast<float4*>(C + row * g.ldc + col) = v;
+                if (FOLD) g2_park<TM, TN>(park, (int)(row - m0), (int)(col - n0), v);
             }
         }
     }
 }
 
-template <int TM, int TN, bool B_KC, int ACT>
+template <int TM, int TN, bool B_KC, int ACT, bool FOLD = false>
 __device__ __forceinline__ void g2_epilogue_full(const GemmArgs& g, f32x16 (&acc)[TM][TN], int64_t m0, int64_t n0, int wm, int wn,
-                                                 int lane) {
+                                                 int lane, float* park = nullptr) {
     float4 bv[TN][4];
     float4 mv[B_KC ? 1 : TM][B_KC ? 1 : TN][4];
     const int64_t row0 = m0 + wm * (32 * TM) + (lane & 31);
@@ -183,6 +199,7 @@
                     }
                 }
                 *reinterpret_cast<float4*>(g.C + (row0 + i * 32) * g.ldc + col0 + j * 32 + 8 * q) = v;
+                if (FOLD) g2_park<TM, TN>(park, (int)(row0 - m0) + i * 32, (int)(col0 - n0) + j * 32 + 8 * q, v);
             }
 }
 
@@ -206,8 +223,43 @@
 #define G2_STAMP(slot)
 #endif
 
-template <bool A_KC, bool B_KC, int TM, int TN>
-__device__ __forceinline__ void gemm2_tile_body(const GemmArgs& g, unsigned bx, unsigned by, unsigned bz, float* lds) {
+template <int TM, int TN>
+__device__ __forceinline__ void g2_fold_thin(const GemmArgs& g, const G2Fold& f, int64_t m0, int64_t n0, unsigned by, float* lds) {
+    constexpr int BM = 64 * TM, BN = 64 * TN, PITCH = BN + 1;
+    constexpr int NG = 256 / BN, KPT = G2_FOLD_KMAX / NG;
+    static_assert(BM * PITCH + BM * G2_FOLD_KMAX <= 2 * 64 * (TM + TN) * G2_BK, "the parked tile and its X0 rows fit the stage LDS");
+    const float* P = lds;
+    float* Xs = lds + BM * PITCH;
+    for (int e = threadIdx.x; e < BM * G2_FOLD_KMAX; e += 256) {
+        const int r = e / G2_FOLD_KMAX, k = e % G2_FOLD_KMAX;
+        const int64_t row = m0 + r;
+        Xs[e] = (k < f.k && row < g.M) ? f.x[row * f.ldx + k] : 0.f;
+    }
+    __syncthreads();
+    const int c = threadIdx.x % BN, kg = threadIdx.x / BN;
+    float a[KPT];
+#pragma unroll
+    for (int j = 0; j < KPT; ++j) a[j] = 0.f;
+    float sum = 0.f;
+#pragma unroll 8
+    for (int r = 0; r < BM; ++r) {
+        const float dz = P[r * PITCH + c];
+        sum += dz;
+#pragma unroll
+        for (int j = 0; j < KPT; ++j) a[j] = fmaf(dz, Xs[r * G2_FOLD_KMAX + kg + j * NG], a[j]);
+    }
+    const int64_t col = n0 + c;
+    if (col >= g.N) return;
+    float* dw = f.dw + ((int64_t)by * g.N + col) * f.k;
+#pragma unroll
+    for (int j = 0; j < KPT; ++j)
+        if (kg + j * NG < f.k) dw[kg + j * NG] = a[j];
+    if (kg == 0 && f.db) f.db[(int64_t)by * g.N + col] = sum;
+}
+
+template <bool A_KC, bool B_KC, int TM, int TN, bool FOLD = false>
+__device__ __forceinline__ void gemm2_tile_body(const GemmArgs& g, unsigned bx, unsigned by, unsigned bz, float* lds,
+                                                const G2Fold* fold = nullptr) {
 #ifdef GEMM2_STAMP
     const unsigned g2_wg = (blockIdx.z * gridDim.y + blockIdx.y) * gridDim.x + blockIdx.x;
 #endif
@@ -331,14 +383,16 @@
         }
     }
     bool fast = A_KC && gridDim.z == 1 && m0 + BM <= g.M && n0 + BN <= (int64_t)g.N && g2_full_ok<B_KC>(g);
+    if (FOLD) __syncthreads();
     if (fast) {
         const int actk = B_KC ? g.act : g.mask_act;
-        if (actk == 1) g2_epilogue_full<TM, TN, B_KC, 1>(g, acc, m0, n0, wm, wn, lane);
-        else if (actk == 2) g2_epilogue_full<TM, TN, B_KC, 2>(g, acc, m0, n0, wm, wn, lane);
-        else g2_epilogue_full<TM, TN, B_KC, 0>(g, acc, m0, n0, wm, wn, lane);
+        if (actk == 1) g2_epilogue_full<TM, TN, B_KC, 1, FOLD>(g, acc, m0, n0, wm, wn, lane, lds);
+        else if (actk == 2) g2_epilogue_full<TM, TN, B_KC, 2, FOLD>(g, acc, m0, n0, wm, wn, lane, lds);
+        else g2_epilogue_full<TM, TN, B_KC, 0, FOLD>(g, acc, m0, n0, wm, wn, lane, lds);
     } else {
-        g2_epilogue<TM, TN>(g, acc, m0, n0, bz, wm, wn, lane);
-    }
+        g2_epilogue<TM, TN, FOLD>(g, acc, m0, n0, bz, wm, wn, lane, lds);
+    }
+    if constexpr (FOLD) g2_fold_thin<TM, TN>(g, *fold, m0, n0, by, lds);
     G2_STAMP(3)
 }
 
@@ -355,6 +409,14 @@
                                         wgid / (gridDim.x * gridDim.y), lds);
 }
 
+template <int TM, int TN>
+__global__ void __launch_bounds__(256) k_gemm2_fold(GemmArgs g, G2Fold f) {
+    __shared__ __attribute__((aligned(1024))) float lds[2 * 64 * (TM + TN) * G2_BK];
+    const unsigned nwg = gridDim.x * gridDim.y;
+    const unsigned wgid = xcd_remap(blockIdx.y * gridDim.x + blockIdx.x, nwg);
+    gemm2_tile_body<true, false, TM, TN, true>(g, wgid % gridDim.x, wgid / gridDim.x, 0, lds, &f);
+}
+
 
 template <bool A_KC, bool B_KC>
 static inline bool gemm2_applies(const GemmArgs& g) {
@@ -380,6 +442,13 @@
     else CDLRM_LAUNCH_EV((k_gemm2<A_KC, B_KC, 1, 1>), grid, dim3(256), dyn, s, g);
 }
 
+static void launch_gemm2_fold(const GemmArgs& g, const G2Fold& f, int tm, int tn, hipStream_t s) {
+    dim3 grid((unsigned)cdiv(g.N, 64 * tn), (unsigned)cdiv(g.M, 64 * tm), 1u);
+    if (tm == 2 && tn == 1) CDLRM_LAUNCH_EV((k_gemm2_fold<2, 1>), grid, dim3(256), 0, s, g, f);
+    else if (tm == 1 && tn == 2) CDLRM_LAUNCH_EV((k_gemm2_fold<1, 2>), grid, dim3(256), 0, s, g, f);
+    else CDLRM_LAUNCH_EV((k_gemm2_fold<1, 1>), grid, dim3(256), 0, s, g, f);
+}
+
 template <bool A_KC, bool B_KC>
 static bool gemm3_try(const GemmArgs& g, int splits, hipStream_t s, const GemmRec* rec);
 
diff --git a/cdlrm_amd/csrc/tape.hip b/cdlrm_amd/csrc/tape.hip
--- a/cdlrm_amd/csrc/tape.hip
+++ b/cdlrm_amd/csrc/tape.hip
@@ -14,7 +14,7 @@
 
 #include "common.h"
 
-#define TAPE_MAX_INT 24
+#define TAPE_MAX_INT 32
 #define TAPE_MAX_FLT 8
 #define TAPE_MAX_LANES 4
 
@@ -85,7 +85,7 @@
         TAPE_FN(cdlrm_window_resolve),
         TAPE_FN(cdlrm_mark_rows), TAPE_FN(cdlrm_interact_fwd), TAPE_FN(cdlrm_interact_bwd), TAPE_FN(cdlrm_gather_interact_fwd),
         TAPE_FN(cdlrm_gather_interact_bwd), TAPE_FN(cdlrm_linear_fwd),
-        TAPE_FN(cdlrm_linear_bwd), TAPE_FN(cdlrm_mlp_wgrad), TAPE_FN(cdlrm_mlp_wgrad_sgd), TAPE_FN(cdlrm_mlp_wgrad_ex),
+        TAPE_FN(cdlrm_linear_bwd), TAPE_FN(cdlrm_linear_bwd_ex), TAPE_FN(cdlrm_mlp_wgrad), TAPE_FN(cdlrm_mlp_wgrad_sgd), TAPE_FN(cdlrm_mlp_wgrad_ex),
         TAPE_FN(cdlrm_mlp_wgrad_sgd_ex), TAPE_FN(cdlrm_bce_fwd_bwd),
         TAPE_FN(cdlrm_loss_fwd_bwd), TAPE_FN(cdlrm_head_fwd_bwd), TAPE_FN(cdlrm_head_finish), TAPE_FN(cdlrm_act_bwd),
         TAPE_FN(cdlrm_sgd_step), TAPE_FN(cdlrm_sgd_step2), TAPE_FN(cdlrm_scale_div),
diff --git a/cdlrm_amd/engine.py b/cdlrm_amd/engine.py
--- a/cdlrm_amd/engine.py
+++ b/cdlrm_amd/engine.py
@@ -686,6 +686,7 @@
         self.fused_head = l_last.out_features == 1 and a_last == 2
         self.wst = self.pref
         self.split_wgrad_min = 2049
+        self.fold_thin_wgrad = True
         self.gather_alone_min = 16384
         self.wide_gemm = True
         self.fuse_once = True
@@ -882,6 +883,17 @@
                                 ops.WgradPlan(xs[nb:], dzs[nb:], gw[nb:], gb[nb:], wk(layers[nb:])))
             b["wgrad_split"][0].set_params([self.W[l] for l in layers[:nb]], [l.bias.data for l in layers[:nb]])
             b["wgrad_split"][1].set_params([self.W[l] for l in layers[nb:]], [l.bias.data for l in layers[nb:]])
+            b["fold"] = None
+            if nb >= 2 and S.is_hip(dev) and self.W[layers[0]].shape[1] <= 16 and self.W[layers[1]].shape[1] % 4 == 0:
+                l0, l1 = layers[0], layers[1]
+                _, fr = ops.linear_bwd_fold_route(b["bot_y"][0], self.W[l1], dzs[1], b["bot_dy"][0], x0, self.gW[l0], self.gb[l0],
+                                                  x_act=self.bot[0][1])
+                if fr is not None:
+                    fold = ops.ThinFold(x0, self.gW[l0], self.gb[l0], dev)
+                    fold.set_params(self.W[l0], l0.bias.data)
+                    rest = ops.WgradPlan(xs[1:nb], dzs[1:nb], gw[1:nb], gb[1:nb], wk(layers[1:nb]))
+                    rest.set_params([self.W[l] for l in layers[1:nb]], [l.bias.data for l in layers[1:nb]])
+                    b["fold"] = (fold, rest)
         self._bufs[B] = b
         return b
 
@@ -1225,13 +1237,23 @@
                               res=(res[0], res[1], res[2], evp), chained_top=chained_top, prepared=chain_sort,
                               sorted_ok=self._next_sorted is not None)
         dY = dfeat[:, 0, :]
+        fold = buf.get("fold") if (split is not None and self.fold_thin_wgrad and self.matmul_precision == "fp32") else None
         for i in reversed(range(1, len(self.bot))):
             l, act = self.bot[i]
             dX = buf["bot_dy"][i - 1]
-            ops.linear_bwd(bot_acts[i], self.W[l], bot_acts[i + 1], dY, dX, None, None, 0,
-                           buf["lin_work"], x_act=self.bot[i - 1][1], **self._mm(l))
+            if i == 1 and fold is not None:
+                fold[0].set_x(X)
+                ops.linear_bwd_fold(bot_acts[i], self.W[l], dY, dX, buf["lin_work"], fold[0], x_act=self.bot[i - 1][1],
+                                    lr=self.lr if sgd_in_wgrad else None)
+            else:
+                ops.linear_bwd(bot_acts[i], self.W[l], bot_acts[i + 1], dY, dX, None, None, 0,
+                               buf["lin_work"], x_act=self.bot[i - 1][1], **self._mm(l))
             dY = dX
-        if split is not None:
+        if fold is not None:
+            ops.mlp_wgrad(fold[1], lr=self.lr if sgd_in_wgrad else None)
+            if not self.defer_top:
+                rec(main.wait_event, ev["wgrad_done"])
+        elif split is not None:
             split[0].set_x(0, X)
             ops.mlp_wgrad(split[0], lr=self.lr if sgd_in_wgrad else None)
             if not self.defer_top:
@@ -1314,7 +1336,7 @@
                self._gslot is not None, self.loss_sync,
                (int(self._pending_resolve["cols"].shape[1]), self._pending_resolve["cols"].stride(0)) if self._mark_this else None,
                self.tape_lanes, self.tape_lanes_below, self.attach_events, self.fuse_gather, self.wide_gemm, self.fuse_once,
-               self.matmul_precision,
+               self.matmul_precision, self.fold_thin_wgrad,
                None if self._cur_sorted is None else self._cur_sorted[3], self._next_sorted is not None,
                self._res[0].stride(0) if (self._res is not None and not hit) else 0,
                self._next_res[0].stride(0) if self._next_res is not None else 0)
diff --git a/cdlrm_amd/ops.py b/cdlrm_amd/ops.py
--- a/cdlrm_amd/ops.py
+++ b/cdlrm_amd/ops.py
@@ -517,8 +517,53 @@
                                       stream_ptr(stream)))
 
 
+class ThinFold:
+
+    def __init__(self, x: torch.Tensor, dW: torch.Tensor, db: Optional[torch.Tensor], device=None):
+        M, k = x.shape
+        assert x.stride(1) == 1 and dW.is_contiguous() and dW.shape[1] == k and (db is None or db.numel() == dW.shape[0])
+        self.M, self.k, self.K = int(M), int(k), int(dW.shape[0])
+        self.x, self.dW, self.db = x, dW, db
+        self.W = self.b = None
+        nbytes = int(_lib.lib().cdlrm_linear_bwd_fold_work_bytes(self.M, self.K, self.k))
+        self.work = torch.empty((nbytes + 255) // 256 * 256, dtype=torch.uint8, device=device if device is not None else dW.device)
+
+    def set_x(self, x: torch.Tensor):
+        assert tuple(x.shape) == (self.M, self.k) and x.stride(1) == 1
+        self.x = x
+
+    def set_params(self, W: torch.Tensor, b: Optional[torch.Tensor]):
+        assert W.is_contiguous() and tuple(W.shape) == (self.K, self.k) and (b is None) == (self.db is None)
+        self.W, self.b = W, b
+
+
+def linear_bwd_fold(X, W, dY, dX, work: torch.Tensor, fold: ThinFold, stream=None, x_act: int = 0, alone: bool = False,
+                    lr: Optional[float] = None):
+    M, K = X.shape
+    N = W.shape[0]
+    assert fold.M == M and fold.K == K and (lr is None or fold.W is not None)
+    check(_lib.lib().cdlrm_linear_bwd_ex(X.data_ptr(), X.stride(0), W.data_ptr(), None, 0, dY.data_ptr(), dY.stride(0),
+                                         dX.data_ptr(), dX.stride(0), None, None, M, N, K, _flags(alone), int(x_act),
+                                         work.data_ptr(), fold.x.data_ptr(), fold.x.stride(0), fold.k, fold.dW.data_ptr(),
+                                         ptr(fold.db), fold.W.data_ptr() if lr is not None else None,
+                                         ptr(fold.b) if lr is not None else None, float(lr or 0.0), fold.work.data_ptr(),
+                                         stream_ptr(stream)))
+
+
+def linear_bwd_fold_route(X, W, dY, dX, x_below, dW_below, db_below, x_act: int = 0, alone: bool = False, n_cu: int = 256,
+                          bf16: bool = False):
+    M, K = X.shape
+    N = W.shape[0]
+    out = (_lib.GemmRoute * 3)()
+    check(_lib.raw().cdlrm_linear_bwd_ex_route(X.data_ptr(), X.stride(0), W.data_ptr(), None, 0, dY.data_ptr(), dY.stride(0),
+                                               dX.data_ptr(), dX.stride(0), None, None, M, N, K, _flags(alone, bf16), int(x_act),
+                                               256, x_below.data_ptr(), x_below.stride(0), x_below.shape[1],
+                                               dW_below.data_ptr(), ptr(db_below), int(n_cu), out))
+    return _route(out[0]), _route(out[2])
+
+
 ROUTE_FAMILIES = {0: None, 1: "smallk_rows", 2: "smallk", 3: "direct", 4: "staged", 5: "gemm2", 6: "gemm3", 7: "gemm",
-                  8: "bf16"}
+                  8: "bf16", 9: "fold"}
 
 
 def _route(r: _lib.GemmRoute) -> Optional[dict]:
diff --git a/include/cdlrm_hip.h b/include/cdlrm_hip.h
--- a/include/cdlrm_hip.h
+++ b/include/cdlrm_hip.h
@@ -249,6 +249,19 @@
                            int64_t M, int32_t N, int32_t K, int32_t act, int32_t x_act, void* work,
                            void* stream, int32_t n_cu, cdlrm_gemm_route* out);
 
+#define CDLRM_ROUTE_FOLD 9
+uint64_t cdlrm_linear_bwd_fold_work_bytes(int64_t M, int32_t K, int32_t k_below);
+int cdlrm_linear_bwd_ex(const float* X, int64_t ld_x, const float* W, const float* Y, int64_t ld_y,
+                        float* dY, int64_t ld_dy, float* dX, int64_t ld_dx, float* dW, float* db,
+                        int64_t M, int32_t N, int32_t K, int32_t act, int32_t x_act, void* work,
+                        const float* x_below, int64_t ld_x_below, int32_t k_below, float* dW_below, float* db_below,
+                        float* P_w, float* P_b, float lr, void* work_below, void* stream);
+int cdlrm_linear_bwd_ex_route(const float* X, int64_t ld_x, const float* W, const float* Y, int64_t ld_y,
+                              float* dY, int64_t ld_dy, float* dX, int64_t ld_dx, float* dW, float* db,
+                              int64_t M, int32_t N, int32_t K, int32_t act, int32_t x_act, void* work,
+                              const float* x_below, int64_t ld_x_below, int32_t k_below, float* dW_below, float* db_below,
+                              int32_t n_cu, cdlrm_gemm_route* out);
+
 uint64_t cdlrm_mlp_wgrad_work_bytes(int32_t n_layers, int64_t M, const int32_t* N, const int32_t* K);
 int cdlrm_mlp_wgrad(int32_t n_layers, const float* const* X, const int64_t* ld_x, const float* const* dZ,
                     const int64_t* ld_dz, float* const* dW, float* const* db, int64_t M, const int32_t* N,
```

Result: no change. 15.41 million (median of 4 runs) (+1.0%).
